# EmanueleCosenza/polyphemus

Measured on AMD Instinct MI355X. Metric: bar-graphs/sec VAE fwd+bwd (+loss +Adam), LMD2 4-track x 32-ts synthetic, higher is better.
Workload: dtype f32 (fp16-pair MFMA products)

## Files before the change

include/polyphemus_hip.h:

```cpp
#ifndef POLYPHEMUS_HIP_H
#define POLYPHEMUS_HIP_H

#include <stdint.h>

#ifdef __cplusplus
extern "C" {
#endif

typedef void* pm_stream_t;

enum {
  PM_OK = 0,
  PM_E_INVALID = -1,
  PM_E_LAUNCH = -2,
  PM_E_UNSUPPORTED = -3
};

enum { PM_N_REL = 6, PM_N_DIST = 32, PM_N_SLOTS = 15, PM_N_PITCH = 131, PM_N_DUR = 99, PM_N_TOK = 230 };

#define PM_ABI_VERSION 9
int pm_abi_version(void);
const char* pm_build_info(void);

int pm_set_deterministic(int32_t on);
// ... 98 lines not shown
int pm_edge_table_bwd(const float* dT , int32_t d, float* d_nn_weight ,
                      float* d_nn_bias , pm_stream_t stream);
int pm_segreduce_fwd(const float* x , const float* T , const int32_t* plan,
                     int32_t N, int32_t E, int32_t G, int32_t d, float dropout_p, uint32_t seed,
                     uint32_t layer_uid, int32_t compact, float* A , pm_stream_t stream);
int pm_segreduce_fwd_planes(const float* x, const float* T, const int32_t* plan, int32_t N, int32_t E, int32_t G,
                            int32_t d, float dropout_p, uint32_t seed, uint32_t layer_uid, int32_t compact,
                            uint16_t* planes, int64_t plane_stride, pm_stream_t stream);
int pm_gcl_forward_fused(const float* x , const float* T , const int32_t* plan, int32_t N,
                         int32_t E, int32_t G, int32_t d, float dropout_p, uint32_t seed, uint32_t layer_uid,
                         const uint16_t* w_frag, const float* bias , int32_t use_classes,
                         float* h , double* col_stats ,
                         uint16_t* planes , int64_t plane_stride, pm_stream_t stream);
int pm_gcl_input_grad_fused(const uint16_t* dh_planes , int64_t plane_stride, const int32_t* plan,
                            int32_t N, int32_t E, int32_t G, int32_t d, const uint16_t* w_frag_t, int32_t use_classes,
                            float* dA , pm_stream_t stream);
typedef struct PmBnBwd {
  const float* h;
  const float* du;
  const float* mean; const float* var; const float* gamma; const float* beta;
  const double* acc3;
  float* dgamma; float* dbeta; float* dbias_pre;
  float eps; int32_t relu;
  int32_t add_residual;
  int32_t reserved;
} PmBnBwd;
int pm_gcl_input_grad_bn(const PmBnBwd* norm, uint16_t* dh_planes , int64_t plane_stride,
                         const int32_t* plan, int32_t N, int32_t E, int32_t G, int32_t d, const uint16_t* w_frag_t,
                         int32_t use_classes, float* dA , pm_stream_t stream);
enum { PM_ABSMAX_SLOTS = 64 };
typedef struct PmH2 {
  const uint32_t* absmax_in; const uint32_t* absmax_aux; float* scale_out; float w_scale; int32_t reserved;
} PmH2;
int pm_absmax(const float* x, int64_t n, uint32_t* out, pm_stream_t stream);
int pm_split_planes_frag_h2(const float* W, int32_t rows, int32_t cols, int32_t kind, int32_t n_mats, int64_t src_stride,
                            int64_t dst_stride, float w_scale, uint16_t* out, pm_stream_t stream);
int pm_gcl_forward_fused_h2(const float* x, const float* T, const int32_t* plan, int32_t N, int32_t E, int32_t G, int32_t d,
                            float dropout_p, uint32_t seed, uint32_t layer_uid, const uint16_t* w_frag, const float* bias,
                            int32_t use_classes, float* h, double* col_stats, uint16_t* planes, int64_t plane_stride,
                            const PmH2* h2, pm_stream_t stream);
int pm_gcl_input_grad_bn_h2(const PmBnBwd* norm, uint16_t* dh_planes, int64_t plane_stride, const int32_t* plan, int32_t N,
                            int32_t E, int32_t G, int32_t d, const uint16_t* w_frag_t, int32_t use_classes, float* dA,
                            const PmH2* h2, pm_stream_t stream);
int pm_bn_bwd_fused_h2(const float* x, const float* dy, int32_t O, int32_t C, const float* mean, const float* var, float eps,
                       const float* gamma, const float* beta, int relu, float* dgamma, float* dbeta, float* dbias_pre,
                       double* acc3, uint16_t* dx_planes, int64_t plane_stride, int32_t sums_ready, const PmH2* h2,
                       pm_stream_t stream);
int pm_gcl_input_grad_fused_h2(const uint16_t* dh_planes, int64_t plane_stride, const int32_t* plan, int32_t N, int32_t E,
                               int32_t G, int32_t d, const uint16_t* w_frag_t, int32_t use_classes, float* dA,
                               const float* dh_scale, float w_scale, pm_stream_t stream);
int pm_gcl_weight_grad_fused_h2(const uint16_t* a_planes, int64_t a_plane_stride, const uint16_t* dh_planes,
                                int64_t dh_plane_stride, const int32_t* plan, int32_t N, int32_t E, int32_t G, int32_t d,
                                int32_t use_classes, float* dW, const float* a_scale, const float* dh_scale,
                                pm_stream_t stream);
int pm_gcl_weight_grad_fused(const uint16_t* a_planes , int64_t a_plane_stride,
                             const uint16_t* dh_planes , int64_t dh_plane_stride, const int32_t* plan,
                             int32_t N, int32_t E, int32_t G, int32_t d, int32_t use_classes, float* dW ,
                             pm_stream_t stream);
int pm_gcl_forward_from_planes(const uint16_t* a_planes , int64_t plane_stride, const int32_t* plan,
                               int32_t N, int32_t E, int32_t G, int32_t d, const uint16_t* w_frag,
                               const float* bias , int32_t use_classes, float* h ,
                               double* col_stats , pm_stream_t stream);
int pm_gcl_forward_from_planes_h2(const uint16_t* a_planes, int64_t plane_stride, const int32_t* plan, int32_t N, int32_t E,
                                  int32_t G, int32_t d, const uint16_t* w_frag, const float* bias, int32_t use_classes,
                                  float* h, double* col_stats, const float* a_scale, float w_scale, pm_stream_t stream);
int pm_rows_times_weight(const float* X, int32_t ldx, int32_t N, int32_t K, const uint16_t* w_frag, int32_t kind,
                         int32_t w_tiles, int32_t Nout, const float* bias , float* C, int32_t ldc,
                         pm_stream_t stream);
int pm_rows_times_weight_longk(const float* X, int32_t ldx, int32_t N, int32_t K, const uint16_t* w_frag, int32_t kind,
                               int32_t w_pitch, int32_t Nout, float* C, int32_t ldc, pm_stream_t stream);
int pm_rows_tn_weight_grad(const float* A, int32_t lda, int32_t M, const float* B, int32_t ldb, int32_t Nn, int32_t K,
                           float* C , int32_t ldc, float* colsum_a , pm_stream_t stream);
typedef struct PmNormSums {
  const float* h;
  const float* mean; const float* var; const float* gamma; const float* beta;
  float eps; int32_t relu;
  double* acc3;
  uint32_t* absmax_out;
} PmNormSums;
int pm_segreduce_bwd_norm(const float* x, const float* T, const float* dA, const float* dres, const int32_t* plan,
                          int32_t N, int32_t E, int32_t G, int32_t d, float dropout_p, uint32_t seed,
                          uint32_t layer_uid, int32_t compact, float* dx, float* dT, const PmNormSums* next_norm,
                          pm_stream_t stream);
int pm_segreduce_bwd(const float* x, const float* T, const float* dA ,
                     const float* dres ,
                     const int32_t* plan, int32_t N, int32_t E, int32_t G, int32_t d, float dropout_p,
                     uint32_t seed, uint32_t layer_uid, int32_t compact, float* dx ,
                     float* dT , pm_stream_t stream);

int pm_bar_aggregate_fwd(const float* x, const float* T, const int32_t* plan, int32_t N, int32_t E, int32_t G, int32_t d,
                         float dropout_p, uint32_t seed, uint32_t layer_uid, uint16_t* planes, int64_t plane_stride,
                         const PmH2* h2 , pm_stream_t stream);
int pm_bar_aggregate_bwd(const float* x, const float* T, const float* dA , const float* dres ,
                         const int32_t* plan, int32_t N, int32_t E, int32_t G, int32_t d, float dropout_p, uint32_t seed,
                         uint32_t layer_uid, float* dx , float* dT ,
                         const PmNormSums* next_norm , pm_stream_t stream);

enum { PM_GEMM_RELU = 1, PM_GEMM_ACCUM = 2,
       PM_GEMM_RELU_ADD = 16 ,
       PM_GEMM_ZEROED = 8 ,
       PM_GEMM_PARTITION = 4  };
int pm_gemm_config(int32_t transA, int32_t M, int32_t N, int32_t K);
int pm_gemm_force_config(int32_t cfg);
int pm_gemm_f32(int transA, int transB, int32_t M, int32_t N, int32_t K, const float* A, int32_t lda,
                const float* B, int32_t ldb, float* C, int32_t ldc, const float* bias, int flags,
                int split_k, const int32_t* rowmap, int32_t rows_per_entry, const int32_t* dyn_entries,
                pm_stream_t stream);
int pm_gemm_f32_grouped(int transA, int transB, int32_t M, int32_t N, int32_t K, const float* A, int32_t lda,
                        const float* B, int32_t ldb, float* C, int32_t ldc, const float* bias, int flags,
                        int split_k, const int32_t* rowmap, int32_t rows_per_entry, const int32_t* dyn_entries,
                        int32_t n_groups, int64_t a_group_stride, int64_t b_group_stride, int64_t c_group_stride,
                        int64_t bias_group_stride, int32_t map_group_stride, int32_t dyn_group_stride,
                        pm_stream_t stream);
int pm_split_planes(const float* src, int64_t n, uint16_t* planes, int64_t plane_stride ,
                    pm_stream_t stream);
typedef struct PmGemmDesc {
  int32_t transA, transB, M, N, K;
  const float* A; int32_t lda;
  const float* B; int32_t ldb;
  float* C; int32_t ldc;
  const float* bias;
  int32_t flags, split_k;
  const int32_t* rowmap; int32_t rows_per_entry;
  const int32_t* dyn_entries;
  int32_t n_groups;
  int64_t a_group_stride, b_group_stride, c_group_stride, bias_group_stride;
  int32_t map_group_stride, dyn_group_stride;
  int32_t b_split_rows; int64_t b_shared_off;
  int32_t c_split_rows; int64_t c_shared_off;
  double* col_stats;
  int32_t operand_planes;
  int64_t a_plane_stride, b_plane_stride;
  const int32_t* class_ptr;
  int32_t class_block;
  const void* b_frag;
  float* a_colsum;
} PmGemmDesc;
int pm_split_planes_frag(const float* W, int32_t rows, int32_t cols, int32_t kind, int32_t n_mats, int64_t src_stride,
                         int64_t dst_stride, uint16_t* out, pm_stream_t stream);
int pm_gemm_f32_desc(const PmGemmDesc* desc, pm_stream_t stream);

int pm_bn_stats(const float* x, int32_t O, int32_t C, int32_t I, float* mean ,
                float* var , float* running_mean ,
                float* running_var, float momentum, double* scratch , pm_stream_t stream);
int pm_bn_apply(const float* x, int32_t O, int32_t C, int32_t I, const float* mean, const float* var,
                float eps, const float* gamma, const float* beta, const float* residual ,
                int relu, float* y, pm_stream_t stream);
int pm_bn_bwd(const float* x, const float* dy, int32_t O, int32_t C, int32_t I, const float* mean,
              const float* var, float eps, const float* gamma, const float* beta, int relu,
              float* dgamma , float* dbeta , float* dbias_pre , float* dx,
              double* scratch , pm_stream_t stream);
#define PM_BN_SCRATCH(C) (256 * 3 * (C) + 4 * (C))
#define PM_BN_SMALL_MAX_ROWS 2048
int pm_bn_small_fwd(const float* x, int32_t O, int32_t C, float eps, const float* gamma, const float* beta,
                    const float* residual , int relu, float* y, float* mean ,
                    float* var , float* running_mean , float* running_var,
                    float momentum, pm_stream_t stream);
int pm_bn_small_bwd(const float* x, const float* dy, int32_t O, int32_t C, const float* mean, const float* var, float eps,
                    const float* gamma, const float* beta, int relu, float* dgamma , float* dbeta ,
                    float* dbias_pre , float* dx, pm_stream_t stream);
int pm_bn_partial_sums(const float* x, const float* dy , int32_t O, int32_t C, int32_t I, const float* mean,
                       const float* var, float eps, const float* gamma, const float* beta, int relu,
                       double* sums , double* scratch , pm_stream_t stream);
int pm_bn_stats_from_sums(const double* sums , double count, int32_t C, float* mean, float* var,
                          float* running_mean , float* running_var, float momentum, pm_stream_t stream);
int pm_bn_bwd_from_sums(const float* x, const float* dy, int32_t O, int32_t C, int32_t I, const float* mean,
// ... 19 lines not shown
                    int32_t sums_ready ,
                    pm_stream_t stream);
int pm_bn_bwd_sums(const float* x, const float* dy, int32_t O, int32_t C, const float* mean, const float* var, float eps,
                   const float* gamma, const float* beta, int relu, double* acc3, pm_stream_t stream);
int pm_bn_fold_weights(const float* W, int32_t rows, int32_t cols, const float* bias, const float* gamma, const float* beta,
                       const float* running_mean, const float* running_var, float eps, float* W_out, float* b_out,
                       pm_stream_t stream);
int pm_bn_counters_update(int64_t* counters , const int64_t* inc , const int64_t* sel ,
                          const int32_t* group_cnt , int32_t n, pm_stream_t stream);
int pm_relu_bwd(const float* dy, const float* y, int64_t n, float* dx, pm_stream_t stream);
int pm_relu_bwd_planes(const float* dy, const float* h, int64_t n, float* dh, uint16_t* planes, int64_t plane_stride,
                       pm_stream_t stream);
int pm_relu_residual_fwd(const float* x, const float* res, int64_t n, float* y, pm_stream_t stream);
int pm_dropout_rows(const float* x, int64_t rows, int32_t cols, float p, uint32_t seed, uint32_t site, float* y,
                    pm_stream_t stream);
int pm_add(const float* a, const float* b, int64_t n, float* out, pm_stream_t stream);
int pm_colsum_acc(const float* x, int32_t M, int32_t C, int32_t ld, float* out , pm_stream_t stream);
int pm_colsum_rows_acc(const float* x, int32_t C, int32_t ld, const int32_t* rowmap, int32_t rows_per_entry,
                       const int32_t* dyn_entries, int32_t max_entries, float* out , pm_stream_t stream);
int pm_reparam_fwd(const float* mu, const float* log_var, const float* eps, int64_t n, float* z, pm_stream_t stream);
int pm_reparam_bwd(const float* dz, const float* log_var, const float* eps, int64_t n, float* dmu ,
                   float* dlog_var , pm_stream_t stream);

int pm_embed_tables(const float* w_pitch_drum , const float* b_pitch_drum,
                    const float* w_pitch_nd, const float* b_pitch_nd, const float* w_dur ,
                    const float* b_dur, const float* bn_drum_g, const float* bn_drum_b,
                    const float* bn_nd_g, const float* bn_nd_b, const float* bn_dur_g, const float* bn_dur_b,
                    float* rm_drum, float* rv_drum, float* rm_nd, float* rv_nd, float* rm_dur, float* rv_dur,
                    const int32_t* tok_hist , int32_t d, int training, float eps, float momentum,
                    float* tables , float* stats ,
                    pm_stream_t stream);
int pm_embed_gather(const float* tables, const int32_t* tokens , const uint8_t* is_drum,
                    int32_t N, int32_t d, int32_t n_slots, float* X , pm_stream_t stream);
int pm_embed_bwd_scatter(const float* dX , const int32_t* tokens, const int32_t* plan, int32_t N,
                         int32_t E, int32_t G, int32_t d, int32_t n_slots,
                         float* S , pm_stream_t stream);
int pm_chord_pad_fwd(const float* tables, const float* chord_w , const float* chord_b,
                     const uint8_t* is_drum, int32_t N, int32_t d, int32_t n_slots, float* cvec ,
                     float* y , pm_stream_t stream);
int pm_chord_pad_bwd(const float* dy , const uint8_t* is_drum, int32_t N, int32_t d, int32_t n_slots,
                     const float* tables, const float* chord_w, float* gsum ,
                     float* d_chord_w , float* S , pm_stream_t stream);
int pm_chord_pad_vec(const float* tables, const float* chord_w, const float* chord_b, int32_t d, int32_t n_slots,
                     float* cvec , pm_stream_t stream);
int pm_chord_tables_fwd(const float* tables , const float* chord_w , int32_t d, int32_t n_slots,
                        float* PT, const float* chord_b , float* cvec ,
                        pm_stream_t stream);
int pm_chord_sum_fwd(const float* PT, const float* cvec, const int32_t* tokens , const uint8_t* is_drum, int32_t N,
                     int32_t d, int32_t n_slots, float* x0 , pm_stream_t stream);
int pm_chord_sum_bwd(const float* dy , const int32_t* tokens, const int32_t* plan, int32_t N, int32_t E, int32_t G,
                     int32_t d , int32_t n_slots, float* Gt, pm_stream_t stream);
int pm_chord_tables_bwd_w(const float* Gt, const float* tables, int32_t d, int32_t n_slots, float* d_chord_w ,
                          float* d_chord_b , pm_stream_t stream);
int pm_chord_tables_bwd_x(const float* Gt, const float* chord_w, int32_t d, int32_t n_slots, float* S , pm_stream_t stream);
int pm_embed_tables_bwd(const float* S, const float* w_pitch_drum, const float* b_pitch_drum,
                        const float* w_pitch_nd, const float* b_pitch_nd, const float* w_dur, const float* b_dur,
                        const float* bn_drum_g, const float* bn_nd_g, const float* bn_dur_g, const float* stats,
                        const int32_t* tok_hist, int32_t d, float eps, float* dw_pitch_drum, float* db_pitch_drum,
                        float* dw_pitch_nd, float* db_pitch_nd, float* dw_dur, float* db_dur, float* dg_drum,
                        float* dbeta_drum, float* dg_nd, float* dbeta_nd, float* dg_dur, float* dbeta_dur,
                        pm_stream_t stream);

int pm_embed_tables_bwd_sync(const float* S, const float* w_pitch_drum, const float* b_pitch_drum, const float* w_pitch_nd,
                             const float* b_pitch_nd, const float* w_dur, const float* b_dur, const float* bn_drum_g,
                             const float* bn_nd_g, const float* bn_dur_g, const float* stats, const int32_t* tok_hist,
                             int32_t d, float eps, float* dw_pitch_drum, float* db_pitch_drum, float* dw_pitch_nd,
                             float* db_pitch_nd, float* dw_dur, float* db_dur, float* dg_drum, float* dbeta_drum,
                             float* dg_nd, float* dbeta_nd, float* dg_dur, float* dbeta_dur, double* sums_out,
                             const double* sums_global, const int32_t* hist_global, pm_stream_t stream);

int pm_gate_fwd(const float* x , const float* w , const float* b , int32_t N,
                int32_t d, float* g , pm_stream_t stream);
int pm_attnpool_fwd(const float* x, const float* g, const float* g_mean, const float* g_var, float eps,
                    const float* bn_g, const float* bn_b, const int32_t* plan, int32_t N, int32_t E, int32_t G,
                    int32_t d, float* alpha , float* out , pm_stream_t stream);
int pm_attnpool_bwd(const float* x, const float* g, const float* g_mean, const float* g_var, float eps,
                    const float* bn_g, const float* alpha, const float* dout , const float* gate_w,
                    const int32_t* plan, int32_t N, int32_t E, int32_t G, int32_t d, float* dx ,
                    float* d_gate_w , float* d_gate_b , float* d_bn_g ,
                    float* d_bn_b , float* scratch ,
                    const float* x_gate ,
                    float* dx_gate ,
                    pm_stream_t stream);
int pm_attnpool_bwd_sums(const float* x, const float* g, const float* g_mean, const float* g_var, float eps,
                         const float* alpha, const float* dout, const int32_t* plan, int32_t N, int32_t E, int32_t G,
                         int32_t d, float* scratch , pm_stream_t stream);
int pm_attnpool_bwd_from_sums(const float* x, const float* g, const float* g_mean, const float* g_var, float eps,
                              const float* bn_g, const float* alpha, const float* dout, const float* gate_w,
                              const int32_t* plan, int32_t N, int32_t E, int32_t G, int32_t d, float* dx, float* d_gate_w,
                              float* d_gate_b, float* d_bn_g, float* d_bn_b, float* scratch, const float* x_gate,
                              float* dx_gate, const double* sums_global , double count_global,
                              pm_stream_t stream);
int pm_bar_broadcast_fwd(const float* bars , const int32_t* plan, int32_t N, int32_t E, int32_t G,
                         int32_t d, float* x , pm_stream_t stream);
int pm_bar_broadcast_bwd(const float* dx , const int32_t* plan, int32_t N, int32_t E, int32_t G,
                         int32_t d, float* dbars , pm_stream_t stream);

int pm_conv3x3_fwd(const float* x, const float* w, const float* b, int32_t G, int32_t Ci, int32_t Co, int32_t H,
                   int32_t W, int up4, float* y, pm_stream_t stream);
int pm_conv3x3_bwd_data(const float* dy, const float* w, int32_t G, int32_t Ci, int32_t Co, int32_t H, int32_t W,
                        int up4, float* dx, pm_stream_t stream);
int pm_conv3x3_bwd_weight(const float* x, const float* dy, int32_t G, int32_t Ci, int32_t Co, int32_t H, int32_t W,
                          int up4, float* dw , float* db , pm_stream_t stream);
int pm_maxpool4_fwd(const float* x, int64_t n_out, float* y, pm_stream_t stream);
int pm_maxpool4_bwd(const float* x, const float* dy, int64_t n_out, float* dx, pm_stream_t stream);
int pm_cnn_enc_fwd(const float* s, const float* w0 , const float* b0, const float* gamma1, const float* beta1,
                   const float* w4 , const float* b4, const float* gamma5, const float* beta5, int32_t G, float eps,
                   float momentum, float* c0, float* a0, float* p0, float* c1, float* a1, float* mean1, float* var1,
                   float* rmean1, float* rvar1, float* mean5, float* var5, float* rmean5, float* rvar5, double* scratch,
                   int64_t scratch_len, pm_stream_t stream);
int pm_cnn_dec_fwd(const float* u2, const float* w1 , const float* b1, const float* gamma2, const float* beta2,
                   const float* w4 , const float* b4, int32_t G, float eps, float momentum, float* c2, float* a2,
                   float* s_logits, float* mean2, float* var2, float* rmean2, float* rvar2, double* scratch, int64_t scratch_len,
                   pm_stream_t stream);
int pm_cnn_enc_bwd(const float* s, const float* c0, const float* a0, const float* p0, const float* c1, const float* da1,
                   const float* mean1, const float* var1, const float* gamma1, const float* beta1, const float* mean5,
                   const float* var5, const float* gamma5, const float* beta5, const float* w4, int32_t G, float eps, float* dw0,
                   float* db0, float* dgamma1, float* dbeta1, float* dw4, float* db4, float* dgamma5, float* dbeta5, float* dc1,
                   float* da0, float* dc0, double* scratch, int64_t scratch_len, pm_stream_t stream);

int pm_content_ce(const float* c_logits , const int32_t* tokens ,
                  const int32_t* tok_hist, const uint8_t* is_drum , int32_t N,
                  int32_t n_slots , float grad_scale,
                  float* d_logits , float* db_pitch_drum ,
                  float* db_pitch_nd , float* db_dur , double* out, pm_stream_t stream);
int pm_content_ce_scaled(const float* c_logits, const int32_t* tokens, const int32_t* tok_hist, const uint8_t* is_drum,
                         int32_t N, int32_t n_slots, float grad_scale, const float* dev_scale ,
                         float* d_logits, float* db_pitch_drum, float* db_pitch_nd, float* db_dur, double* out,
                         pm_stream_t stream);
int64_t pm_unembed_scratch_bytes(int32_t d);
int pm_unembed_ce(const float* H, const float* w_pitch_drum , const float* b_pitch_drum,
                  const float* w_pitch_nd, const float* b_pitch_nd, const float* w_dur , const float* b_dur,
                  const int32_t* tokens, const int32_t* plan, int32_t N, int32_t E, int32_t G, int32_t d, int32_t n_slots,
                  float grad_scale, const float* dev_scale, float* logits , float* d_logits,
                  float* db_pitch_drum, float* db_pitch_nd, float* db_dur, double* out, uint16_t* w_planes ,
                  pm_stream_t stream);
int64_t pm_unembed_dh_scratch_bytes(int32_t d);
int pm_unembed_dh(const float* d_logits, const float* w_pitch_drum , const float* w_pitch_nd,
                  const float* w_dur , const int32_t* plan, int32_t N, int32_t E, int32_t G, int32_t d,
                  int32_t n_slots, float* dH, uint16_t* w_planes, int32_t prepare, pm_stream_t stream);
int64_t pm_unembed_row_counts_len(int32_t N, int32_t n_slots);
int pm_unembed_row_lists(const int32_t* tokens, const int32_t* plan, int32_t N, int32_t E, int32_t G, int32_t d, int32_t n_slots,
                         int32_t* row_lists, int32_t* pad_lists, int32_t* row_counts, float* dH_zero, pm_stream_t stream);
int pm_unembed_ce_rows(const float* H, const float* w_pitch_drum, const float* b_pitch_drum, const float* w_pitch_nd,
                       const float* b_pitch_nd, const float* w_dur, const float* b_dur, const int32_t* tokens, const int32_t* plan,
                       int32_t N, int32_t E, int32_t G, int32_t d, int32_t n_slots, float grad_scale, const float* dev_scale,
                       float* logits, float* d_logits, float* db_pitch_drum, float* db_pitch_nd, float* db_dur, double* out,
                       uint16_t* w_planes, const int32_t* row_lists, const int32_t* row_counts, pm_stream_t stream);
int pm_unembed_dh_rows(const float* d_logits, const float* w_pitch_drum, const float* w_pitch_nd, const float* w_dur,
                       const int32_t* plan, int32_t N, int32_t E, int32_t G, int32_t d, int32_t n_slots, float* dH,
                       uint16_t* w_planes, const int32_t* row_lists, const int32_t* row_counts, pm_stream_t stream);
int pm_unembed_dw(const float* d_logits, const float* H, const int32_t* plan, int32_t N, int32_t E, int32_t G, int32_t d,
                  int32_t n_slots, float* dw_pitch_drum, float* dw_pitch_nd, float* dw_dur, const int32_t* row_lists,
                  const int32_t* row_counts, pm_stream_t stream);
int pm_unembed_bias_grads(const float* d_logits, const uint8_t* is_drum , int32_t N, int32_t S,
                          float* db_pitch_drums , float* db_pitch_non_drums , float* db_dur ,
                          pm_stream_t stream);
int pm_kld(const float* mu, const float* log_var, int32_t B, int32_t d, float beta, float* dmu ,
           float* dlog_var, double* out, pm_stream_t stream);
int pm_bce_logits(const float* logits, const float* target, int64_t n, float grad_scale, float* dlogits ,
                  double* out, pm_stream_t stream);

int pm_content_accuracy(const float* c_logits , const int32_t* tokens ,
                        const uint8_t* is_drum , int32_t N, int64_t* counts , pm_stream_t stream);
int pm_structure_metrics(const float* s_logits, const float* s_target, int64_t n, int64_t* counts ,
                         pm_stream_t stream);
// ... 151 lines not shown
```

polyphemus_amd/_lib.py:

```python
from __future__ import annotations

import ctypes as C
import os
from typing import Optional

import torch

_HERE = os.path.dirname(os.path.abspath(__file__))
LIB_PATH = os.environ.get("PM_LIB_PATH") or os.path.join(_HERE, "libpolyphemus_hip.so")

PROF_NCLASS = 40
PLAN_FIELDS = ["rowptr", "csr_src", "csr_dist", "csr_eid", "colptr", "csc_dst", "csc_reldist", "csc_eid",
               "csc_invcnt", "node_bar", "bar_ptr", "group_list", "group_cnt", "tok_hist", "row_list", "node_trel", "trk_list", "trk_cnt", "scratch"]

_SIGS = {
    "pm_plan_layout": "iiip",
    "pm_gcl_tile_order": "piipi",
    "pm_row_tile_order": "ipi",
    "pm_plan_build": "pppppppiiiiips",
    "pm_edge_attrs_to_ids": "pipps",
    "pm_tokens_from_onehot": "pips",
    "pm_batch_flags": "pppiipps",
    "pm_edge_table": "ppips",
    "pm_edge_table_bwd": "pipps",
# ... 67 lines not shown
    "pm_conv3x3_bwd_weight": "ppiiiiiipps",
    "pm_maxpool4_fwd": "plps",
    "pm_maxpool4_bwd": "pplps",
    "pm_cnn_enc_fwd": "pppppppppiffppppppppppppppls",
    "pm_cnn_dec_fwd": "pppppppiffppppppppls",
    "pm_cnn_enc_bwd": "pppppppppppppppifppppppppppppls",
    "pm_content_ce": "ppppiifppppps",
    "pm_content_ce_scaled": "ppppiifpppppps",
    "pm_unembed_ce": "pppppppppiiiiifpppppppps",
    "pm_unembed_dh": "pppppiiiiippis",
    "pm_unembed_dh_scratch_bytes": "i",
    "pm_unembed_row_counts_len": "ii",
    "pm_unembed_dw": "pppiiiiippppps",
    "pm_unembed_row_lists": "ppiiiiipppps",
    "pm_unembed_ce_rows": "pppppppppiiiiifpppppppppps",
    "pm_unembed_dh_rows": "pppppiiiiipppps",
    "pm_unembed_scratch_bytes": "i",
    "pm_kld": "ppiifppps",
    "pm_unembed_bias_grads": "ppiippps",
    "pm_bce_logits": "pplfpps",
    "pm_content_accuracy": "pppips",
    "pm_structure_metrics": "pplps",
    "pm_adam_step": "pppplffffifs",
    "pm_comm_unique_id": "p",
    "pm_comm_init": "piip",
    "pm_comm_destroy": "p",
    "pm_allreduce": "plps",
    "pm_prof_configure": "li",
    "pm_prof_begin": "i",
    "pm_prof_end": "ppp",
    "pm_vae_step_workspace_bytes": "piiiii",
    "pm_vae_step_forward": "pppppppfuufiplpps",
    "pm_vae_step_info": "pp",
    "pm_vae_step_outputs": "ppppps".replace(" ", ""),
    "pm_vae_step_set_output_grads": "ppppps",
    "pm_vae_step_saved": "piiipp",
    "pm_vae_step_output_views": "ppp",
    "pm_bn_relu_decisions": "pppppflips",
    "pm_vae_step_backward_decoder": "ps",
    "pm_vae_step_backward_encoder": "ps",
    "pm_vae_step_backward_encoder_tail": "ps",
    "pm_vae_step_join_decoder_grads": "ps",
    "pm_vae_step_backward_encoder_heads": "ps",
    "pm_vae_step_reload_switches": "",
    "pm_relu_bwd_planes": "pplppls",
    "pm_absmax": "plps",
    "pm_split_planes_frag_h2": "piiiillfps",
    "pm_gcl_forward_fused_h2": "pppiiiifuuppippplps",
    "pm_gcl_input_grad_bn_h2": "pplpiiiipipps",
    "pm_gcl_weight_grad_fused_h2": "plplpiiiiippps",
    "pm_bn_bwd_fused_h2": "ppiippfppippppplips",
    "pm_gcl_input_grad_fused_h2": "plpiiiipippfs",
    "pm_bn_apply_fused_absmax": "piipfpppipppppfps",
    "pm_bar_aggregate_fwd": "pppiiiifuuplps",
    "pm_bar_aggregate_bwd": "pppppiiiifuuppps",
    "pm_gcl_forward_from_planes_h2": "plpiiiippipppfs",
    "pm_set_deterministic": "i",
    "pm_get_deterministic": "",
    "pm_deterministic_faults": "",
    "pm_h2_clamp_events": "i",
    "pm_h2_clamp_init": "",
    "pm_overflow_snapshot": "ps",
    "pm_overflow_poison": "pps",
    "pm_grad_nonfinite_check": "plpppfffis",
    "pm_adam_step_guarded": "pppplffffps",
    "pm_adam_bias_scalars": "plfffps",
    "pm_vae_step_set_metrics": "pp",
    "pm_unembed_ce_metrics": "pppppppppiiiiifppppppppppps",
    "pm_unembed_ce_rows_metrics": "pppppppppiiiiifppppppppppppps",
    "pm_content_accuracy_slots": "pppiipps",
    "pm_train_metric_counts": "pppiipplps",
    "pm_grad_sumsq": "plps",
    "pm_grad_nonfinite_check_sumsq": "plpppfffips",
    "pm_grad_clip_finish": "pffps",
    "pm_adam_step_clipped": "pppplffffipps",
    "pm_adam_step_ema": "ppppplffffiffpps",
    "pm_buffer_swap": "ppls",
    "pm_sample_tokens": "plfifups",
    "pm_mtp_from_tokens": "ppilppps",
    "pm_sample_chords": "pplpupps",
    "pm_node_tracks": "pilppps",
    "pm_sample_structure": "pipuppps",
    "pm_notes_from_tokens": "ppiilppppplpps",
}
_CT = {"p": C.c_void_p, "i": C.c_int32, "l": C.c_int64, "f": C.c_float, "u": C.c_uint32, "s": C.c_void_p, "D": C.c_double}
_RET64 = {"pm_vae_step_workspace_bytes", "pm_vae_layout_bytes", "pm_vae_step_state_bytes", "pm_unembed_scratch_bytes",
          "pm_unembed_dh_scratch_bytes", "pm_unembed_row_counts_len"}
ABI_VERSION = 9
EXPORTED = sorted(list(_SIGS) + ["pm_abi_version", "pm_build_info", "pm_dropout_hash", "pm_sample_hash",
                                 "pm_vae_layout_bytes", "pm_vae_step_state_bytes"])



class PmChordRules(C.Structure):
    _fields_ = [("temperature", C.c_float * 2), ("top_k", C.c_int32), ("top_p", C.c_float), ("min_notes", C.c_int32 * 4),
                ("max_notes", C.c_int32 * 4), ("pitch_mask", (C.c_uint32 * 4) * 4)]


class PmStructureRules(C.Structure):
    _fields_ = [("temperature", C.c_float), ("bias", C.c_float * 4), ("min_active", C.c_int32 * 4),
                ("max_active", C.c_int32 * 4), ("step_mask", C.c_uint32 * 4)]


_lib: Optional[C.CDLL] = None


class HipExtensionError(RuntimeError):
    pass


def lib() -> C.CDLL:
    global _lib
    if _lib is None:
        if not os.path.exists(LIB_PATH):
            raise HipExtensionError(
                f"{LIB_PATH} is missing: build it with `python -m polyphemus_amd.build` "
                "(__graft_entry__.build()).  There is no CPU fallback for the HIP path.")
        L = C.CDLL(LIB_PATH)
        for name, sig in _SIGS.items():
            fn = getattr(L, name)
            fn.argtypes = [_CT[c] for c in sig]
            fn.restype = C.c_int64 if name in _RET64 else C.c_int
        L.pm_vae_layout_bytes.restype = C.c_int64
        L.pm_vae_step_state_bytes.restype = C.c_int64
        L.pm_abi_version.restype = C.c_int
        if L.pm_abi_version() != ABI_VERSION:
            raise HipExtensionError(f"{LIB_PATH} has ABI version {L.pm_abi_version()}, this binding expects {ABI_VERSION}: "
                                    "rebuild it (`python -m polyphemus_amd.build --force`)")
        L.pm_build_info.restype = C.c_char_p
        L.pm_dropout_hash.argtypes = [C.c_uint32] * 4
        L.pm_dropout_hash.restype = C.c_uint32
        L.pm_sample_hash.argtypes = [C.c_uint32] * 4
        L.pm_sample_hash.restype = C.c_uint32
        _lib = L
    return _lib


def ptr(t: Optional[torch.Tensor]):
    return None if t is None else t.data_ptr()


def stream() -> int:
    return torch.cuda.current_stream().cuda_stream


_ERR = {-1: "PM_E_INVALID (bad argument)", -2: "PM_E_LAUNCH (kernel launch failed)", -3: "PM_E_UNSUPPORTED"}


def call(name: str, *args) -> None:
    rc = getattr(lib(), name)(*args)
    if rc != 0:
        raise HipExtensionError(f"{name} failed: {_ERR.get(rc, rc)}")


def plan_layout(N: int, E: int, G: int):
    off = (C.c_int64 * (len(PLAN_FIELDS) + 1))()
    rc = lib().pm_plan_layout(N, E, G, C.cast(off, C.c_void_p))
    if rc != 0:
        raise HipExtensionError(f"pm_plan_layout({N},{E},{G}) failed: {_ERR.get(rc, rc)}")
    return list(off)


def gcl_tile_order(trk_cnt, use_classes: bool, N: int):
    tc = (C.c_int32 * 32)(*[int(v) for v in list(trk_cnt)[:32]])
    grid = lib().pm_gcl_tile_order(C.cast(tc, C.c_void_p), int(bool(use_classes)), int(N), None, 0)
    if grid < 0:
# ... 40 lines not shown
```

polyphemus_amd/csrc/common.h:

```cpp
#pragma once
#include <hip/hip_runtime.h>
#include <stdint.h>
#include "../../include/polyphemus_hip.h"

#define PM_WAVE 64

static inline int pm_check_launch() {
  hipError_t e = hipGetLastError();
  return e == hipSuccess ? PM_OK : PM_E_LAUNCH;
}

static inline int pm_device_slot() {
  int d = 0;
  if (hipGetDevice(&d) != hipSuccess || d < 0 || d >= 16) d = 0;
  return d;
}

static inline int64_t pm_cdiv(int64_t a, int64_t b) { return (a + b - 1) / b; }
static inline int64_t pm_align4(int64_t x) { return (x + 3) & ~int64_t(3); }

struct PmPlanView {
  const int32_t* rowptr; const int32_t* csr_src; const int32_t* csr_dist; const int32_t* csr_eid;
  const int32_t* colptr; const int32_t* csc_dst; const int32_t* csc_reldist; const int32_t* csc_eid;
  const float* csc_invcnt; const int32_t* node_bar; const int32_t* bar_ptr; const int32_t* group_list;
// ... 98 lines not shown
  return v;
}
__device__ static inline double pm_wave_sum_d(double v) {
#pragma unroll
  for (int o = 32; o > 0; o >>= 1) v += __shfl_xor(v, o, 64);
  return v;
}
typedef __bf16 pm_bf16x2 __attribute__((ext_vector_type(2)));
typedef float pm_f32x2 __attribute__((ext_vector_type(2)));
typedef unsigned int pm_u32x2 __attribute__((ext_vector_type(2)));
__device__ static inline unsigned pm_pk_bf16(float a, float b) {
  pm_f32x2 v = {a, b};
  return __builtin_bit_cast(unsigned, __builtin_convertvector(v, pm_bf16x2));
}
__device__ static inline void pm_split3_pair(float a, float b, unsigned& h1, unsigned& h2, unsigned& h3) {
  h1 = pm_pk_bf16(a, b);
  a -= __uint_as_float(h1 << 16); b -= __uint_as_float(h1 & 0xffff0000u);
  h2 = pm_pk_bf16(a, b);
  a -= __uint_as_float(h2 << 16); b -= __uint_as_float(h2 & 0xffff0000u);
  h3 = pm_pk_bf16(a, b);
}
typedef _Float16 pm_f16x2 __attribute__((ext_vector_type(2)));
__device__ static inline unsigned pm_pk_f16(float a, float b) {
  pm_f32x2 v = {a, b};
  return __builtin_bit_cast(unsigned, __builtin_convertvector(v, pm_f16x2));
}
__device__ static inline void pm_split2h_pair(float a, float b, unsigned& h1, unsigned& h2) {
  h1 = pm_pk_f16(a, b);
  const pm_f16x2 hv = __builtin_bit_cast(pm_f16x2, h1);
  a -= (float)hv.x; b -= (float)hv.y;
  h2 = pm_pk_f16(a, b);
}
__device__ static inline float pm_pow2_scale(float bound, int target) {
  if (!(bound > 0.f) || !(bound < 3.0e38f)) return 1.f;
  const int e = (int)((__float_as_uint(bound) >> 23) & 0xff) - 126;
  int k = target - e;
  k = k < -120 ? -120 : (k > 120 ? 120 : k);
  return __uint_as_float((unsigned)(k + 127) << 23);
}
__device__ static inline float pm_clamp_f16(float v) { return fminf(fmaxf(v, -65504.f), 65504.f); }
__device__ static inline float pm_clamp_f16(float v, bool& cut) {
  const float c = fminf(fmaxf(v, -65504.f), 65504.f);
  cut = cut || (c != v);
  return c;
}
__device__ static inline float pm_absmax_read(const unsigned* __restrict__ p) {
  static_assert(PM_ABSMAX_SLOTS == 64, "one slot per lane");
  float v = __uint_as_float(p[__lane_id()]);
#pragma unroll
  for (int o = 32; o > 0; o >>= 1) v = fmaxf(v, __shfl_xor(v, o, 64));
  return v;
}
__device__ static inline void pm_absmax_block(unsigned* __restrict__ out, float v, unsigned* sm) {
  v = fabsf(v);
#pragma unroll
  for (int o = 32; o > 0; o >>= 1) v = fmaxf(v, __shfl_xor(v, o, 64));
  if ((threadIdx.x & 63) == 0) atomicMax(sm, __float_as_uint(v));
  __syncthreads();
  if (threadIdx.x == 0) atomicMax(out + (blockIdx.x % PM_ABSMAX_SLOTS), *sm);
}
__device__ static inline void pm_store_planes4(uint16_t* __restrict__ planes, int64_t plane_stride, int64_t idx, float x0,
                                               float x1, float x2, float x3) {
  unsigned l1, l2, l3, u1, u2, u3;
  pm_split3_pair(x0, x1, l1, l2, l3);
  pm_split3_pair(x2, x3, u1, u2, u3);
  const pm_u32x2 p1 = {l1, u1}, p2 = {l2, u2}, p3 = {l3, u3};
  *reinterpret_cast<pm_u32x2*>(planes + idx) = p1;
  *reinterpret_cast<pm_u32x2*>(planes + plane_stride + idx) = p2;
  *reinterpret_cast<pm_u32x2*>(planes + 2 * plane_stride + idx) = p3;
}
__device__ static inline double pm_repl_sum(const double* __restrict__ acc, int nacc, int C, int a, int c) {
  double t = 0;
#pragma unroll
  for (int r = 0; r < PM_BN_REPL; ++r) t += acc[((int64_t)r * nacc + a) * C + c];
  return t;
}
__device__ static inline float pm_bn_bwd_elem(float x, float dy, float mean, float rstd, float ga, float be, float m0,
                                              float m1, int relu) {
  const float xh = (x - mean) * rstd;
  float du = dy;
  if (relu && !(xh * ga + be > 0.f)) du = 0.f;
  return ga * rstd * (du - m0 - xh * m1);
}
__device__ static inline float pm_wave_max(float v) {
#pragma unroll
  for (int o = 32; o > 0; o >>= 1) v = fmaxf(v, __shfl_xor(v, o, 64));
  return v;
}
#endif
```

polyphemus_amd/csrc/linear.hip:

```cpp
#include "gcl_tiles.h"
#include <type_traits>
#include <stdlib.h>
#include "prof.h"
#include "wide.h"

#ifndef ROWS_NMW
#define ROWS_NMW 4
#endif
template <int D> constexpr int rows_nmw() { return D == 256 ? ROWS_NMW : 4; }
template <int D> constexpr int rows_threads() { return (rows_nmw<D>() + 4) * 64; }
template <int D, int BKIND>
__global__ void __launch_bounds__(rows_threads<D>()) __attribute__((amdgpu_waves_per_eu((rows_nmw<D>() + 4) / 4, (rows_nmw<D>() + 4) / 4)))
k_rows_w(const float* __restrict__ X, int ldx, int N, const char* __restrict__ wfrag, int wtiles, int nblk,
         const float* __restrict__ bias, float* __restrict__ C, int ldc) {
  constexpr int NMW = rows_nmw<D>(), WC = D / NMW, TN = WC / 32, KS = D / 16, RB = D * 2, PL = BM * RB;
  extern __shared__ __attribute__((aligned(16))) char smem[];
  float* const sC = reinterpret_cast<float*>(smem + 3 * PL);
  int m0 = 0, rows = BM;
  if (!pm_row_tile(N, blockIdx.x, m0, rows)) return;
  const bool full = rows > BM / 2;
  N = min(N, m0 + rows);
  const int tid = threadIdx.x, lane = tid & 63, wave = tid >> 6, li = lane & 31, lh = lane >> 5;
  if (wave >= NMW) {
    constexpr int LPR = D / 4, RPW = 64 / LPR, NR = BM / (4 * RPW);
    const int st = tid - NMW * 64, c4 = st % LPR, r0 = st / LPR;
    const __amdgpu_buffer_rsrc_t crs = __builtin_amdgcn_make_buffer_rsrc(C, 0, GCL_OOB, 0x00020000);
    __syncthreads();
#pragma unroll 1
    for (int qb = 0; qb < nblk; ++qb) {
      __syncthreads();
      __syncthreads();
      float4 bv = make_float4(0.f, 0.f, 0.f, 0.f);
      if (bias) bv = *reinterpret_cast<const float4*>(bias + qb * D + c4 * 4);
#pragma unroll
      for (int k = 0; k < NR; ++k) {
        const int rr = r0 + k * 4 * RPW, row = m0 + rr;
        float4 v = *reinterpret_cast<const float4*>(sC + rr * D + c4 * 4);
        v.x += bv.x; v.y += bv.y; v.z += bv.z; v.w += bv.w;
        __builtin_amdgcn_raw_buffer_store_b128(__builtin_bit_cast(u32x4, v), crs,
            row < N ? (int)(((int64_t)row * ldc + qb * D + c4 * 4) * 4) : GCL_OOB, 0, 0);
      }
    }
    return;
  }
  {
    const __amdgpu_buffer_rsrc_t rs = __builtin_amdgcn_make_buffer_rsrc(const_cast<float*>(X), 0, GCL_OOB, 0x00020000);
    constexpr int CPR = D / 8, NST = NMW * 64, NCHK = BM * CPR / NST;
    u32x4 v[NCHK][2];
#pragma unroll
    for (int k = 0; k < NCHK; ++k) {
      const int ci = tid + k * NST, rr = ci / CPR, ch = ci % CPR, row = m0 + rr;
#pragma unroll
      for (int h = 0; h < 2; ++h)
        v[k][h] = __builtin_amdgcn_raw_buffer_load_b128(rs, row < N ? (int)(((int64_t)row * ldx + ch * 8 + h * 4) * 4) : GCL_OOB, 0, 0);
    }
#pragma unroll
    for (int k = 0; k < NCHK; ++k) {
      const int ci = tid + k * NST, rr = ci / CPR, ch = ci % CPR;
      unsigned p1[4], p2[4], p3[4];
#pragma unroll
      for (int h = 0; h < 2; ++h) {
        pm_split3_pair(__uint_as_float(v[k][h][0]), __uint_as_float(v[k][h][1]), p1[2 * h], p2[2 * h], p3[2 * h]);
        pm_split3_pair(__uint_as_float(v[k][h][2]), __uint_as_float(v[k][h][3]), p1[2 * h + 1], p2[2 * h + 1], p3[2 * h + 1]);
      }
      char* dst = smem + rr * RB + ((ch ^ (rr & 15)) << 4);
      *reinterpret_cast<u32x4*>(dst) = u32x4{p1[0], p1[1], p1[2], p1[3]};
      *reinterpret_cast<u32x4*>(dst + PL) = u32x4{p2[0], p2[1], p2[2], p2[3]};
      *reinterpret_cast<u32x4*>(dst + 2 * PL) = u32x4{p3[0], p3[1], p3[2], p3[3]};
    }
  }
  const __amdgpu_buffer_rsrc_t brs = __builtin_amdgcn_make_buffer_rsrc(const_cast<char*>(wfrag), 0, GCL_OOB, 0x00020000);
  auto bload = [&](bf16x8 (&dst)[3][TN], int gs) {
    const int qb = min(gs / KS, nblk - 1), ks = gs % KS;
    const int n0 = qb * D + wave * WC;
    const int soff = __builtin_amdgcn_readfirstlane(BKIND == 0 ? ((n0 >> 5) * KS + ks) * 3072 : (ks * wtiles + (n0 >> 5)) * 3072);
#pragma unroll
    for (int j = 0; j < TN; ++j)
#pragma unroll
      for (int p = 0; p < 3; ++p)
        dst[p][j] = __builtin_bit_cast(bf16x8, __builtin_amdgcn_raw_buffer_load_b128(brs, lane * 16, soff + j * (BKIND == 0 ? KS : 1) * 3072 + p * 1024, 0));
  };
  bf16x8 bq[GCL_BDEPTH][3][TN];
#pragma unroll
  for (int s2 = 0; s2 < GCL_BDEPTH; ++s2) bload(bq[s2], s2);
  __syncthreads();
// ... 2 lines not shown
    for (int p = 0; p < 3; ++p)
#pragma unroll
      for (int i = 0; i < 2; ++i) {
        const int rr = i * 32 + li;
        a[p][i] = *reinterpret_cast<const bf16x8*>(smem + p * PL + rr * RB + (((ks * 2 + lh) ^ (rr & 15)) << 4));
      }
  };
  bf16x8 af[2][3][2];
  aload(af[0], 0);
  auto blocks = [&](auto ni_tag) {
  constexpr int NI = decltype(ni_tag)::value;
#pragma unroll 1
  for (int qb = 0; qb < nblk; ++qb) {
    f32x16 acc[2][TN];
#pragma unroll
    for (int i = 0; i < 2; ++i)
#pragma unroll
      for (int j = 0; j < TN; ++j)
#pragma unroll
        for (int r = 0; r < 16; ++r) acc[i][j][r] = 0.f;
#pragma unroll
    for (int ks = 0; ks < KS; ++ks) {
      aload(af[(ks + 1) & 1], (ks + 1) % KS);
      constexpr int PA[6] = {2, 1, 0, 1, 0, 0}, PB[6] = {0, 1, 2, 0, 1, 0};
#pragma unroll
      for (int t6 = 0; t6 < 6; ++t6)
#pragma unroll
        for (int i = 0; i < NI; ++i)
#pragma unroll
          for (int j = 0; j < TN; ++j)
            acc[i][j] = __builtin_amdgcn_mfma_f32_32x32x16_bf16(af[ks & 1][PA[t6]][i], bq[ks % GCL_BDEPTH][PB[t6]][j], acc[i][j], 0, 0, 0);
      bload(bq[ks % GCL_BDEPTH], qb * KS + ks + GCL_BDEPTH);
      __builtin_amdgcn_sched_barrier(0);
    }
    __syncthreads();
#pragma unroll
    for (int i = 0; i < 2; ++i)
#pragma unroll
      for (int r = 0; r < 16; ++r)
#pragma unroll
        for (int j = 0; j < TN; ++j)
          sC[(i * 32 + (r & 3) + 8 * (r >> 2) + 4 * lh) * D + wave * WC + j * 32 + li] = acc[i][j][r];
    __syncthreads();
  }
  };
  if (full) blocks(std::integral_constant<int, 2>{});
  else blocks(std::integral_constant<int, 1>{});
}

extern "C" int pm_rows_times_weight(const float* X, int32_t ldx, int32_t N, int32_t K, const uint16_t* w_frag, int32_t kind,
                                    int32_t w_tiles, int32_t Nout, const float* bias, float* C, int32_t ldc,
                                    pm_stream_t stream) {
  if (!X || !w_frag || !C || N <= 0 || (K != 128 && K != 256 && K != 512) || Nout <= 0 || (Nout % K) || (kind != 0 && kind != 1) ||
      ldx < K || ldc < Nout || (ldx & 3) || (ldc & 3) || ((uintptr_t)X % 16) || ((uintptr_t)C % 16) ||
      ((uintptr_t)w_frag % 16) || (bias && ((uintptr_t)bias % 16)) || (int64_t)N * ldx * 4 >= 0x7fffffffLL ||
      (int64_t)N * ldc * 4 >= 0x7fffffffLL || (kind == 1 && w_tiles * 32 < Nout))
    return PM_E_INVALID;
  if (K == 512)
    return pm_wide_rows_times_weight(X, ldx, N, w_frag, kind, w_tiles, Nout, bias, C, ldc, (hipStream_t)stream);
  hipStream_t st = (hipStream_t)stream;
  const dim3 grid(pm_row_grid(N));
  const size_t lds = (size_t)3 * BM * K * 2 + (size_t)BM * K * 4;
  const int pe = pm_prof_open(st, PM_PROF_ROWS_W, 2.0 * N * (double)K * Nout);
#define LAUNCH(DD, KD)                                                                                                 \
  do {                                                                                                                 \
    static bool once_dev[16] = {}; bool& once = once_dev[pm_device_slot()];                                                                                          \
    if (!once) {                                                                                                       \
      hipFuncSetAttribute((const void*)k_rows_w<DD, KD>, hipFuncAttributeMaxDynamicSharedMemorySize, 160 * 1024);      \
      once = true;                                                                                                     \
    }                                                                                                                  \
    hipLaunchKernelGGL((k_rows_w<DD, KD>), grid, dim3(rows_threads<DD>()), lds, st, X, ldx, N, reinterpret_cast<const char*>(w_frag), \
                       w_tiles, Nout / K, bias, C, ldc);                                                               \
  } while (0)
  if (K == 256) { if (kind == 0) LAUNCH(256, 0); else LAUNCH(256, 1); }
  else { if (kind == 0) LAUNCH(128, 0); else LAUNCH(128, 1); }
#undef LAUNCH
  pm_prof_close(st, pe);
  return pm_check_launch();
}

template <int D, int BKIND>
__global__ void __launch_bounds__(rows_threads<D>()) __attribute__((amdgpu_waves_per_eu((rows_nmw<D>() + 4) / 4, (rows_nmw<D>() + 4) / 4)))
k_rows_wk(const float* __restrict__ X, int ldx, int N, int K, const char* __restrict__ wfrag, int wpitch,
          float* __restrict__ C, int ldc) {
  constexpr int NMW = rows_nmw<D>(), WC = D / NMW, TN = WC / 32, HS = D + 8, NTHR = rows_threads<D>();
  extern __shared__ __attribute__((aligned(16))) char smem[];
  float* const sH = reinterpret_cast<float*>(smem);
  const int nchunk = K / CH;
  int m0 = 0, rows = BM;
  if (!pm_row_tile(N, blockIdx.x, m0, rows)) return;
  const bool full = rows > BM / 2;
  N = min(N, m0 + rows);
  const int tid = threadIdx.x, lane = tid & 63, wave = tid >> 6;
  if (wave >= NMW) {
    const int pt = tid - NMW * 64, q = pt & 31, prow = pt >> 5;
    const __amdgpu_buffer_rsrc_t xrs = __builtin_amdgcn_make_buffer_rsrc(const_cast<float*>(X), 0, GCL_OOB, 0x00020000);
    auto issue = [&](float4 (&xs)[8], int c) {
#pragma unroll
      for (int ps = 0; ps < 8; ++ps) {
        const int row = m0 + ps * 8 + prow;
        xs[ps] = __builtin_bit_cast(float4, __builtin_amdgcn_raw_buffer_load_b128(
            xrs, (row < N && c < nchunk) ? (int)(((int64_t)row * ldx + c * CH + q * 4) * 4) : GCL_OOB, 0, 0));
      }
    };
    auto put = [&](const float4 (&xs)[8], int c) {
      char* img = smem + (c & 1) * IMG;
#pragma unroll
      for (int ps = 0; ps < 8; ++ps) {
        const int rr = ps * 8 + prow;
        unsigned l1, l2, l3, u1, u2, u3;
        pm_split3_pair(xs[ps].x, xs[ps].y, l1, l2, l3);
        pm_split3_pair(xs[ps].z, xs[ps].w, u1, u2, u3);
        const pm_u32x2 p1 = {l1, u1}, p2 = {l2, u2}, p3 = {l3, u3};
        char* dst = img + rr * ROWB + (((q >> 1) ^ (rr & 15)) << 4) + ((q & 1) << 3);
        *reinterpret_cast<pm_u32x2*>(dst) = p1;
        *reinterpret_cast<pm_u32x2*>(dst + PLANE) = p2;
        *reinterpret_cast<pm_u32x2*>(dst + 2 * PLANE) = p3;
      }
    };
    float4 xa[8], xb[8];
    issue(xa, 0);
    issue(xb, 1);
    __builtin_amdgcn_sched_barrier(0);
    put(xa, 0);
    __syncthreads();
#pragma unroll 1
    for (int c = 0; c < nchunk; c += 2) {
      issue(xa, c + 2);
      __builtin_amdgcn_sched_barrier(0);
      put(xb, c + 1);
      __syncthreads();
      if (c + 1 >= nchunk) break;
      issue(xb, c + 3);
      __builtin_amdgcn_sched_barrier(0);
      put(xa, c + 2);
      __syncthreads();
    }
  } else {
    const int li = lane & 31, lh = lane >> 5;
    f32x16 acc[2][TN];
#pragma unroll
    for (int i = 0; i < 2; ++i)
#pragma unroll
      for (int j = 0; j < TN; ++j)
#pragma unroll
        for (int r = 0; r < 16; ++r) acc[i][j][r] = 0.f;
    const __amdgpu_buffer_rsrc_t brs = __builtin_amdgcn_make_buffer_rsrc(const_cast<char*>(wfrag), 0, GCL_OOB, 0x00020000);
    const int n0 = wave * WC;
    auto bload = [&](bf16x8 (&dst)[3][TN], int gs) {
      const int kk = min(gs, nchunk * 8 - 1);
      const int soff = __builtin_amdgcn_readfirstlane(BKIND == 0 ? ((n0 >> 5) * wpitch + kk) * 3072 : (kk * (D / 32) + (n0 >> 5)) * 3072);
#pragma unroll
      for (int j = 0; j < TN; ++j)
#pragma unroll
        for (int p = 0; p < 3; ++p)
          dst[p][j] = __builtin_bit_cast(bf16x8, __builtin_amdgcn_raw_buffer_load_b128(brs, lane * 16, soff + j * (BKIND == 0 ? wpitch : 1) * 3072 + p * 1024, 0));
    };
    bf16x8 bq[GCL_BDEPTH][3][TN];
#pragma unroll
    for (int s2 = 0; s2 < GCL_BDEPTH; ++s2) bload(bq[s2], s2);
    __syncthreads();
    auto chunks = [&](auto ni_tag) {
      constexpr int NI = decltype(ni_tag)::value;
#pragma unroll 1
      for (int c = 0; c < nchunk; ++c) {
        const char* img = smem + (c & 1) * IMG;
#pragma unroll
        for (int ks = 0; ks < 8; ++ks) {
          bf16x8 a[3][NI];
#pragma unroll
          for (int p = 0; p < 3; ++p)
#pragma unroll
            for (int i = 0; i < NI; ++i) {
              const int rr = i * 32 + li;
              a[p][i] = *reinterpret_cast<const bf16x8*>(img + p * PLANE + rr * ROWB + (((ks * 2 + lh) ^ (rr & 15)) << 4));
            }
          constexpr int PA[6] = {2, 1, 0, 1, 0, 0}, PB[6] = {0, 1, 2, 0, 1, 0};
#pragma unroll
          for (int t6 = 0; t6 < 6; ++t6)
#pragma unroll
            for (int i = 0; i < NI; ++i)
#pragma unroll
              for (int j = 0; j < TN; ++j)
                acc[i][j] = __builtin_amdgcn_mfma_f32_32x32x16_bf16(a[PA[t6]][i], bq[ks % GCL_BDEPTH][PB[t6]][j], acc[i][j], 0, 0, 0);
          bload(bq[ks % GCL_BDEPTH], c * 8 + ks + GCL_BDEPTH);
          __builtin_amdgcn_sched_barrier(0);
        }
        __syncthreads();
      }
    };
    if (full) chunks(std::integral_constant<int, 2>{});
    else chunks(std::integral_constant<int, 1>{});
#pragma unroll
    for (int j = 0; j < TN; ++j)
#pragma unroll
      for (int i = 0; i < 2; ++i)
#pragma unroll
        for (int r = 0; r < 16; ++r)
          sH[(i * 32 + (r & 3) + 8 * (r >> 2) + 4 * lh) * HS + n0 + j * 32 + li] = acc[i][j][r];
  }
  __syncthreads();
  constexpr int NG = 512 / D, RG = BM / NG;
  static_assert(NTHR >= 512, "row groups");
  const int col = tid % D, rg = tid / D;
  const __amdgpu_buffer_rsrc_t crs = __builtin_amdgcn_make_buffer_rsrc(C, 0, GCL_OOB, 0x00020000);
  if (tid >= 512) return;
#pragma unroll 8
  for (int k = 0; k < RG; ++k) {
    const int rr = rg * RG + k, row = m0 + rr;
    __builtin_amdgcn_raw_buffer_store_b32(__float_as_uint(sH[rr * HS + col]), crs, row < N ? (int)(((int64_t)row * ldc + col) * 4) : GCL_OOB, 0, 0);
  }
}

extern "C" int pm_rows_times_weight_longk(const float* X, int32_t ldx, int32_t N, int32_t K, const uint16_t* w_frag,
                                          int32_t kind, int32_t w_pitch, int32_t Nout, float* C, int32_t ldc,
                                          pm_stream_t stream) {
  if (!X || !w_frag || !C || N <= 0 || K <= 0 || (K % CH) || (Nout != 128 && Nout != 256 && Nout != 512) || (kind != 0 && kind != 1) ||
      ldx < K || ldc < Nout || (ldx & 3) || ((uintptr_t)X % 16) || ((uintptr_t)w_frag % 16) ||
      (int64_t)N * ldx * 4 >= 0x7fffffffLL || (int64_t)N * ldc * 4 >= 0x7fffffffLL || (kind == 0 && w_pitch * 16 < K))
    return PM_E_INVALID;
  if (Nout == 512)
    return pm_wide_rows_times_weight_longk(X, ldx, N, K, w_frag, kind, w_pitch, C, ldc, (hipStream_t)stream);
  hipStream_t st = (hipStream_t)stream;
  const dim3 grid(pm_row_grid(N));
  const size_t lds = 2 * IMG;
  const int pe = pm_prof_open(st, PM_PROF_ROWS_W, 2.0 * N * (double)K * Nout);
#define LAUNCH(DD, KD)                                                                                                 \
  do {                                                                                                                 \
    static bool once_dev[16] = {}; bool& once = once_dev[pm_device_slot()];                                                                                          \
    if (!once) {                                                                                                       \
      hipFuncSetAttribute((const void*)k_rows_wk<DD, KD>, hipFuncAttributeMaxDynamicSharedMemorySize, 160 * 1024);     \
      once = true;                                                                                                     \
    }                                                                                                                  \
    hipLaunchKernelGGL((k_rows_wk<DD, KD>), grid, dim3(rows_threads<DD>()), lds, st, X, ldx, N, K, reinterpret_cast<const char*>(w_frag), \
                       w_pitch, C, ldc);                                                                               \
  } while (0)
  if (Nout == 256) { if (kind == 0) LAUNCH(256, 0); else LAUNCH(256, 1); }
  else { if (kind == 0) LAUNCH(128, 0); else LAUNCH(128, 1); }
#undef LAUNCH
  pm_prof_close(st, pe);
  return pm_check_launch();
}


__global__ void __launch_bounds__(512) __attribute__((amdgpu_waves_per_eu(2, 2)))
k_rows_tn(const float* __restrict__ A, int lda, const float* __restrict__ B, int ldb, int K, int ntn, int nsplit,
          float* __restrict__ C, int ldc, float* __restrict__ colsum_a, unsigned* gate) {
  extern __shared__ __attribute__((aligned(16))) char smem[];
  const int ntile = gridDim.x / nsplit;
  int L = blockIdx.x;
  {
    const int total = gridDim.x, q = total >> 3, r = total & 7, xcd = L & 7, idx = L >> 3;
    L = (xcd < r ? xcd * (q + 1) : r * (q + 1) + (xcd - r) * q) + idx;
  }
  const int zs = L / ntile, within = L % ntile, ft = within / ntn, ct = within % ntn;
  const int kper = (((K + nsplit - 1) / nsplit + DW_KT - 1) / DW_KT) * DW_KT;
  const int kbeg = zs * kper, kend = min(kbeg + kper, K);
  if (kbeg >= kend) { pm_turn_skip_block(gate, 8); return; }
  const int nt = (kend - kbeg + DW_KT - 1) / DW_KT;
  const int tid = threadIdx.x, lane = tid & 63, wave = tid >> 6;
  const unsigned my_turn = blockIdx.x * 8 + wave;
  if (wave >= 4) {
    const int lt = tid - 256, c4 = lt & 31, r0 = lt >> 5;
    const __amdgpu_buffer_rsrc_t ars = __builtin_amdgcn_make_buffer_rsrc(const_cast<float*>(A), 0, GCL_OOB, 0x00020000);
    const __amdgpu_buffer_rsrc_t brs = __builtin_amdgcn_make_buffer_rsrc(const_cast<float*>(B), 0, GCL_OOB, 0x00020000);
    const int acol = (ft * DW_T + c4 * 4) * 4, bcol = (ct * DW_T + c4 * 4) * 4;
    float4 cs = make_float4(0.f, 0.f, 0.f, 0.f);
    const bool want_cs = colsum_a != nullptr && ct == 0;
    auto issue = [&](float4 (&v)[4][2], int t) {
#pragma unroll
      for (int j = 0; j < 4; ++j) {
        const int row = kbeg + t * DW_KT + r0 + j * 8;
        const bool ok = t < nt && row < kend;
        v[j][0] = __builtin_bit_cast(float4, __builtin_amdgcn_raw_buffer_load_b128(ars, ok ? (int)((int64_t)row * lda * 4) + acol : GCL_OOB, 0, 0));
        v[j][1] = __builtin_bit_cast(float4, __builtin_amdgcn_raw_buffer_load_b128(brs, ok ? (int)((int64_t)row * ldb * 4) + bcol : GCL_OOB, 0, 0));
      }
    };
    auto put = [&](const float4 (&v)[4][2], int t) {
      char* st = smem + (t & 1) * DW_STAGE;
#pragma unroll
      for (int j = 0; j < 4; ++j) {
        if (want_cs) { cs.x += v[j][0].x; cs.y += v[j][0].y; cs.z += v[j][0].z; cs.w += v[j][0].w; }
#pragma unroll
        for (int o = 0; o < 2; ++o) {
          unsigned l1, l2, l3, u1, u2, u3;
          pm_split3_pair(v[j][o].x, v[j][o].y, l1, l2, l3);
          pm_split3_pair(v[j][o].z, v[j][o].w, u1, u2, u3);
          const pm_u32x2 p1 = {l1, u1}, p2 = {l2, u2}, p3 = {l3, u3};
          char* dst = st + o * 3 * DW_PLANE + (r0 + j * 8) * DW_PITCH + c4 * 8;
          *reinterpret_cast<pm_u32x2*>(dst) = p1;
          *reinterpret_cast<pm_u32x2*>(dst + DW_PLANE) = p2;
          *reinterpret_cast<pm_u32x2*>(dst + 2 * DW_PLANE) = p3;
        }
      }
    };
    float4 va[4][2], vb[4][2];
    issue(va, 0);
    issue(vb, 1);
    __builtin_amdgcn_sched_barrier(0);
    put(va, 0);
    __syncthreads();
#pragma unroll 1
    for (int t = 0; t < nt; t += 2) {
      issue(va, t + 2);
      __builtin_amdgcn_sched_barrier(0);
      put(vb, t + 1);
      __syncthreads();
      if (t + 1 >= nt) break;
      issue(vb, t + 3);
      __builtin_amdgcn_sched_barrier(0);
      put(va, t + 2);
      __syncthreads();
    }
    pm_turn_enter(gate, my_turn);
    if (want_cs) {
      cs.x += __shfl_xor(cs.x, 32, 64); cs.y += __shfl_xor(cs.y, 32, 64);
      cs.z += __shfl_xor(cs.z, 32, 64); cs.w += __shfl_xor(cs.w, 32, 64);
      float* dst = colsum_a + ft * DW_T + c4 * 4;
      if (lane < 32) { atomicAdd(dst, cs.x); atomicAdd(dst + 1, cs.y); atomicAdd(dst + 2, cs.z); atomicAdd(dst + 3, cs.w); }
    }
    pm_turn_leave(gate, my_turn);
    return;
  }
  const int li = lane & 31, lh = lane >> 5, wr = wave >> 1, wc = wave & 1;
// ... 70 lines not shown
```

polyphemus_amd/csrc/norm.hip:

```cpp
#include "common.h"
#include <stdlib.h>

#define BN_MAX_CHUNKS 256
#define BN_NACC 3

struct BnCtx {
  const float* mean; const float* var; const float* gamma; const float* beta; float eps; int relu;
};
template <int MODE>
__device__ static inline void bn_acc(float xv, float dyv, float m, float rstd, float ga, float be, int relu,
                                     double& a, double& b, double& c) {
  if (MODE == 0) { a += (double)xv; b += (double)xv * (double)xv; }
  else {
    const float xh = (xv - m) * rstd;
    float du = dyv;
    if (relu && !(xh * ga + be > 0.f)) du = 0.f;
    a += (double)du; b += (double)du * (double)xh; c += (double)xh;
  }
}

template <int MODE>
__global__ void __launch_bounds__(256) k_colreduce_rows(const float* __restrict__ x, const float* __restrict__ dy,
                                                        int O, int C, BnCtx ctx, int rows_per_chunk,
                                                        double* __restrict__ partial) {
  __shared__ double sh[4][64][12];
  const int lane = threadIdx.x & 63, wave = threadIdx.x >> 6;
  const int c = (blockIdx.x * 64 + lane) * 4;
  const bool ok = c < C;
  double acc[12] = {0, 0, 0, 0, 0, 0, 0, 0, 0, 0, 0, 0};
  float m[4] = {0, 0, 0, 0}, rs[4] = {1, 1, 1, 1}, ga[4] = {1, 1, 1, 1}, be[4] = {0, 0, 0, 0};
  if (MODE == 1 && ok) {
#pragma unroll
    for (int j = 0; j < 4; ++j) {
      m[j] = ctx.mean[c + j]; rs[j] = rsqrtf(ctx.var[c + j] + ctx.eps);
      ga[j] = ctx.gamma[c + j]; be[j] = ctx.beta[c + j];
    }
  }
  const int r0 = blockIdx.y * rows_per_chunk;
  int r1 = r0 + rows_per_chunk;
  if (r1 > O) r1 = O;
  if (ok) {
    for (int r = r0 + wave; r < r1; r += 4) {
      const float4 xv = *reinterpret_cast<const float4*>(x + (int64_t)r * C + c);
      float4 dv = make_float4(0.f, 0.f, 0.f, 0.f);
      if (MODE == 1) dv = *reinterpret_cast<const float4*>(dy + (int64_t)r * C + c);
      bn_acc<MODE>(xv.x, dv.x, m[0], rs[0], ga[0], be[0], ctx.relu, acc[0], acc[4], acc[8]);
      bn_acc<MODE>(xv.y, dv.y, m[1], rs[1], ga[1], be[1], ctx.relu, acc[1], acc[5], acc[9]);
      bn_acc<MODE>(xv.z, dv.z, m[2], rs[2], ga[2], be[2], ctx.relu, acc[2], acc[6], acc[10]);
      bn_acc<MODE>(xv.w, dv.w, m[3], rs[3], ga[3], be[3], ctx.relu, acc[3], acc[7], acc[11]);
    }
  }
  constexpr int NA = MODE == 0 ? 8 : 12;
#pragma unroll
  for (int j = 0; j < NA; ++j) sh[wave][lane][j] = acc[j];
  __syncthreads();
  if (wave == 0 && ok) {
#pragma unroll
    for (int j = 0; j < NA; ++j) {
      const double s = sh[0][lane][j] + sh[1][lane][j] + sh[2][lane][j] + sh[3][lane][j];
      partial[((int64_t)blockIdx.y * BN_NACC + (j >> 2)) * C + c + (j & 3)] = s;
    }
  }
}

template <int MODE>
__global__ void __launch_bounds__(256) k_colreduce_chan(const float* __restrict__ x, const float* __restrict__ dy,
                                                        int O, int C, int I, BnCtx ctx, int64_t per_chunk,
                                                        double* __restrict__ partial) {
  __shared__ double sh[3][4];
  const int c = blockIdx.x;
  float m = 0.f, rs = 1.f, ga = 1.f, be = 0.f;
  if (MODE == 1) { m = ctx.mean[c]; rs = rsqrtf(ctx.var[c] + ctx.eps); ga = ctx.gamma[c]; be = ctx.beta[c]; }
  double a = 0, b = 0, cc = 0;
  const int64_t total = (int64_t)O * I;
  const int64_t j0 = (int64_t)blockIdx.y * per_chunk;
  int64_t j1 = j0 + per_chunk;
  if (j1 > total) j1 = total;
  for (int64_t j = j0 + threadIdx.x; j < j1; j += blockDim.x) {
    const int64_t idx = ((j / I) * C + c) * I + (j % I);
    bn_acc<MODE>(x[idx], MODE == 1 ? dy[idx] : 0.f, m, rs, ga, be, ctx.relu, a, b, cc);
  }
  a = pm_wave_sum_d(a); b = pm_wave_sum_d(b); cc = pm_wave_sum_d(cc);
  if ((threadIdx.x & 63) == 0) { sh[0][threadIdx.x >> 6] = a; sh[1][threadIdx.x >> 6] = b; sh[2][threadIdx.x >> 6] = cc; }
  __syncthreads();
  if (threadIdx.x < 3)
    partial[((int64_t)blockIdx.y * BN_NACC + threadIdx.x) * C + c] =
        sh[threadIdx.x][0] + sh[threadIdx.x][1] + sh[threadIdx.x][2] + sh[threadIdx.x][3];
}

#define BN_FIN_WAVES 16
__device__ static inline void sum_chunks(const double* __restrict__ partial, int nchunk, int C, int c, int nacc,
                                         double (*sh)[64][BN_NACC], double* out) {
  const int lane = threadIdx.x & 63, wave = threadIdx.x >> 6;
  double s[BN_NACC] = {0, 0, 0};
  if (c < C)
    for (int k = wave; k < nchunk; k += BN_FIN_WAVES)
      for (int a = 0; a < nacc; ++a) s[a] += partial[((int64_t)k * BN_NACC + a) * C + c];
  for (int a = 0; a < BN_NACC; ++a) sh[wave][lane][a] = s[a];
  __syncthreads();
  for (int a = 0; a < BN_NACC; ++a) {
    double t = 0;
// ... 791 lines not shown
```

polyphemus_amd/csrc/pool.hip:

```cpp
#include "common.h"

__global__ void __launch_bounds__(256) k_gate_fwd(const float* __restrict__ x, const float* __restrict__ w,
                                                  const float* __restrict__ b, int N, int d, float* __restrict__ g) {
  const int n = blockIdx.x * 4 + (threadIdx.x >> 6);
  if (n >= N) return;
  const int lane = threadIdx.x & 63;
  float s = 0.f;
  for (int c = lane * 4; c < d; c += 256) {
    const float4 xv = *reinterpret_cast<const float4*>(x + (int64_t)n * d + c);
    const float4 wv = *reinterpret_cast<const float4*>(w + c);
    s += xv.x * wv.x + xv.y * wv.y + xv.z * wv.z + xv.w * wv.w;
  }
  s = pm_wave_sum(s);
  if (lane == 0) g[n] = s + b[0];
}
extern "C" int pm_gate_fwd(const float* x, const float* w, const float* b, int32_t N, int32_t d, float* g,
                           pm_stream_t stream) {
  if (!x || !w || !b || !g || N <= 0 || d <= 0 || (d & 3)) return PM_E_INVALID;
  hipLaunchKernelGGL(k_gate_fwd, dim3(pm_cdiv(N, 4)), dim3(256), 0, (hipStream_t)stream, x, w, b, N, d, g);
  return pm_check_launch();
}

__device__ static inline float block_max(float v, float* sh) {
  v = pm_wave_max(v);
  if ((threadIdx.x & 63) == 0) sh[threadIdx.x >> 6] = v;
  __syncthreads();
  const float r = fmaxf(fmaxf(sh[0], sh[1]), fmaxf(sh[2], sh[3]));
  __syncthreads();
  return r;
}
__device__ static inline float block_sum(float v, float* sh) {
  v = pm_wave_sum(v);
  if ((threadIdx.x & 63) == 0) sh[threadIdx.x >> 6] = v;
  __syncthreads();
  const float r = sh[0] + sh[1] + sh[2] + sh[3];
  __syncthreads();
  return r;
}

__global__ void __launch_bounds__(256) k_attnpool_fwd(const float* __restrict__ x, const float* __restrict__ g,
                                                      const float* __restrict__ gm, const float* __restrict__ gv,
                                                      float eps, const float* __restrict__ bg,
                                                      const float* __restrict__ bb, const int* __restrict__ bar_ptr,
                                                      int d, float* __restrict__ alpha, float* __restrict__ out) {
  __shared__ float sh[4];
  const int b = blockIdx.x;
  const int beg = bar_ptr[b], end = bar_ptr[b + 1];
  const float mean = gm[0], rstd = rsqrtf(gv[0] + eps), ga = bg[0], be = bb[0];
  float mx = -INFINITY;
  for (int i = beg + threadIdx.x; i < end; i += blockDim.x) mx = fmaxf(mx, (g[i] - mean) * rstd * ga + be);
  mx = block_max(mx, sh);
  float s = 0.f;
  for (int i = beg + threadIdx.x; i < end; i += blockDim.x) s += expf(((g[i] - mean) * rstd * ga + be) - mx);
  s = block_sum(s, sh);
  const float inv = 1.0f / (s + 1e-16f);
  for (int i = beg + threadIdx.x; i < end; i += blockDim.x)
    alpha[i] = expf(((g[i] - mean) * rstd * ga + be) - mx) * inv;
  __syncthreads();
  for (int c = threadIdx.x; c < d; c += blockDim.x) {
    float acc = 0.f;
    for (int i = beg; i < end; ++i) acc += alpha[i] * x[(int64_t)i * d + c];
    out[(int64_t)b * d + c] = acc;
  }
}
extern "C" int pm_attnpool_fwd(const float* x, const float* g, const float* g_mean, const float* g_var, float eps,
                               const float* bn_g, const float* bn_b, const int32_t* plan, int32_t N, int32_t E,
                               int32_t G, int32_t d, float* alpha, float* out, pm_stream_t stream) {
  if (!x || !g || !g_mean || !g_var || !bn_g || !bn_b || !plan || !alpha || !out || N <= 0 || G <= 0 || d <= 0)
    return PM_E_INVALID;
  PmPlanView pv = pm_plan_view(plan, N, E, G);
  hipLaunchKernelGGL(k_attnpool_fwd, dim3(G), dim3(256), 0, (hipStream_t)stream, x, g, g_mean, g_var, eps, bn_g, bn_b,
                     pv.bar_ptr, d, alpha, out);
  return pm_check_launch();
}

__global__ void __launch_bounds__(256) k_attnpool_bwd1(const float* __restrict__ x, const float* __restrict__ g,
                                                       const float* __restrict__ gm, const float* __restrict__ gv,
                                                       float eps, const float* __restrict__ alpha,
                                                       const float* __restrict__ dout, const int* __restrict__ bar_ptr,
                                                       int d, float* __restrict__ dgn, double* __restrict__ sums,
                                                       unsigned* gate) {
  __shared__ float sh[4];
  const int b = blockIdx.x;
  const int beg = bar_ptr[b], end = bar_ptr[b + 1];
  const int lane = threadIdx.x & 63, wave = threadIdx.x >> 6;
  for (int i = beg + wave; i < end; i += 4) {
    float s = 0.f;
    for (int c = lane * 4; c < d; c += 256) {
      const float4 xv = *reinterpret_cast<const float4*>(x + (int64_t)i * d + c);
      const float4 dv = *reinterpret_cast<const float4*>(dout + (int64_t)b * d + c);
      s += xv.x * dv.x + xv.y * dv.y + xv.z * dv.z + xv.w * dv.w;
    }
    s = pm_wave_sum(s);
    if (lane == 0) dgn[i] = s;
  }
  __syncthreads();
  float t = 0.f;
  for (int i = beg + threadIdx.x; i < end; i += blockDim.x) t += alpha[i] * dgn[i];
  t = block_sum(t, sh);
  const float mean = gm[0], rstd = rsqrtf(gv[0] + eps);
  float s0 = 0.f, s1 = 0.f;
  for (int i = beg + threadIdx.x; i < end; i += blockDim.x) {
    const float v = alpha[i] * (dgn[i] - t);
    dgn[i] = v;
    s0 += v;
    s1 += v * ((g[i] - mean) * rstd);
  }
  s0 = block_sum(s0, sh);
  s1 = block_sum(s1, sh);
  pm_turn_enter_block(gate);
  if (threadIdx.x == 0) { atomicAdd(&sums[0], (double)s0); atomicAdd(&sums[1], (double)s1); }
  pm_turn_leave_block(gate);
}
__global__ void __launch_bounds__(256) k_attnpool_bwd2(const float* __restrict__ x, const float* __restrict__ g,
                                                       const float* __restrict__ gm, const float* __restrict__ gv,
                                                       float eps, const float* __restrict__ bg,
                                                       const float* __restrict__ alpha, const float* __restrict__ dout,
                                                       const float* __restrict__ w, const int* __restrict__ node_bar,
                                                       const float* __restrict__ dgn, const double* __restrict__ sums,
                                                       int N, int d, float* __restrict__ dx, float* dW, float* db,
                                                       float* dbn_g, float* dbn_b, const float* __restrict__ xg,
                                                       float* __restrict__ dxg, const double* __restrict__ gsums,
                                                       double gcount, unsigned* gate) {
  extern __shared__ __attribute__((aligned(16))) float sW[];
  for (int i = threadIdx.x; i <= d; i += blockDim.x) sW[i] = 0.f;
  __syncthreads();
  const int lane = threadIdx.x & 63, wave = threadIdx.x >> 6;
  const float mean = gm[0], rstd = rsqrtf(gv[0] + eps), ga = bg[0];
  const float m0 = gsums ? (float)(gsums[0] / gcount) : (float)(sums[0] / N);
  const float m1 = gsums ? (float)(gsums[1] / gcount) : (float)(sums[1] / N);
  if (blockIdx.x == 0 && threadIdx.x == 0) { dbn_b[0] += (float)sums[0]; dbn_g[0] += (float)sums[1]; }
  float4 wacc[4];
#pragma unroll
  for (int k = 0; k < 4; ++k) wacc[k] = make_float4(0.f, 0.f, 0.f, 0.f);
  float bacc = 0.f;
  for (int n = blockIdx.x * 4 + wave; n < N; n += gridDim.x * 4) {
    const float gh = (g[n] - mean) * rstd;
    const float dg = ga * rstd * (dgn[n] - m0 - gh * m1);
    const float a = alpha[n];
    const int b = node_bar[n];
#pragma unroll
    for (int k = 0; k < 4; ++k) {
      const int c = lane * 4 + k * 256;
      if (c >= d) continue;
      const float4 xv = *reinterpret_cast<const float4*>(xg + (int64_t)n * d + c);
      const float4 dv = *reinterpret_cast<const float4*>(dout + (int64_t)b * d + c);
      const float4 wv = *reinterpret_cast<const float4*>(w + c);
      if (dxg) {
        *reinterpret_cast<float4*>(dx + (int64_t)n * d + c) = make_float4(a * dv.x, a * dv.y, a * dv.z, a * dv.w);
        *reinterpret_cast<float4*>(dxg + (int64_t)n * d + c) = make_float4(dg * wv.x, dg * wv.y, dg * wv.z, dg * wv.w);
      } else
      *reinterpret_cast<float4*>(dx + (int64_t)n * d + c) =
          make_float4(a * dv.x + dg * wv.x, a * dv.y + dg * wv.y, a * dv.z + dg * wv.z, a * dv.w + dg * wv.w);
      wacc[k].x += dg * xv.x; wacc[k].y += dg * xv.y; wacc[k].z += dg * xv.z; wacc[k].w += dg * xv.w;
    }
    bacc += dg;
  }
  for (int w = 0; w < (gate ? 4 : 1); ++w) {
    if (!gate || wave == w) {
#pragma unroll
      for (int k = 0; k < 4; ++k) {
        const int c = lane * 4 + k * 256;
        if (c >= d) continue;
        atomicAdd(&sW[c + 0], wacc[k].x); atomicAdd(&sW[c + 1], wacc[k].y);
        atomicAdd(&sW[c + 2], wacc[k].z); atomicAdd(&sW[c + 3], wacc[k].w);
      }
      if (lane == 0) atomicAdd(&sW[d], bacc);
    }
    if (gate) __syncthreads();
  }
  __syncthreads();
  pm_turn_enter_block(gate);
  for (int i = threadIdx.x; i < d; i += blockDim.x) atomicAdd(&dW[i], sW[i]);
  if (threadIdx.x == 0) atomicAdd(&db[0], sW[d]);
  pm_turn_leave_block(gate);
}
static int attnpool_bwd_impl(const float* x, const float* g, const float* g_mean, const float* g_var, float eps,
                             const float* bn_g, const float* alpha, const float* dout, const float* gate_w,
                             const int32_t* plan, int32_t N, int32_t E, int32_t G, int32_t d, float* dx, float* d_gate_w,
                             float* d_gate_b, float* d_bn_g, float* d_bn_b, float* scratch, const float* x_gate,
                             float* dx_gate, int phase, const double* gsums, double gcount, pm_stream_t stream) {
  if ((x_gate == nullptr) != (dx_gate == nullptr)) return PM_E_INVALID;
  if (!x || !g || !g_mean || !g_var || !alpha || !dout || !plan || !scratch || N <= 0 || G <= 0 || d <= 0 || (d & 3) ||
      d > 1024 || ((uintptr_t)scratch & 7))
    return PM_E_INVALID;
  if (phase != 1 && (!bn_g || !gate_w || !dx || !d_gate_w || !d_gate_b || !d_bn_g || !d_bn_b)) return PM_E_INVALID;
  hipStream_t st = (hipStream_t)stream;
  PmPlanView pv = pm_plan_view(plan, N, E, G);
  double* sums = reinterpret_cast<double*>(scratch);
  float* dgn = scratch + 4;
  if (phase != 2) {
    hipMemsetAsync(sums, 0, 2 * sizeof(double), st);
    hipLaunchKernelGGL(k_attnpool_bwd1, dim3(G), dim3(256), 0, st, x, g, g_mean, g_var, eps, alpha, dout, pv.bar_ptr, d,
                       dgn, sums, pm_det_gate(st));
  }
  if (phase != 1) {
    int nb = (int)pm_cdiv(N, 4);
    if (nb > 256) nb = 256;
    hipLaunchKernelGGL(k_attnpool_bwd2, dim3(nb), dim3(256), sizeof(float) * (d + 1), st, x, g, g_mean, g_var, eps, bn_g,
                       alpha, dout, gate_w, pv.node_bar, dgn, sums, N, d, dx, d_gate_w, d_gate_b, d_bn_g, d_bn_b,
                       x_gate ? x_gate : x, dx_gate, gsums, gcount, pm_det_gate(st));
  }
  return pm_check_launch();
}
extern "C" int pm_attnpool_bwd(const float* x, const float* g, const float* g_mean, const float* g_var, float eps,
                               const float* bn_g, const float* alpha, const float* dout, const float* gate_w,
                               const int32_t* plan, int32_t N, int32_t E, int32_t G, int32_t d, float* dx,
                               float* d_gate_w, float* d_gate_b, float* d_bn_g, float* d_bn_b, float* scratch,
                               const float* x_gate, float* dx_gate, pm_stream_t stream) {
  return attnpool_bwd_impl(x, g, g_mean, g_var, eps, bn_g, alpha, dout, gate_w, plan, N, E, G, d, dx, d_gate_w, d_gate_b,
                           d_bn_g, d_bn_b, scratch, x_gate, dx_gate, 0, nullptr, 0.0, stream);
}
extern "C" int pm_attnpool_bwd_sums(const float* x, const float* g, const float* g_mean, const float* g_var, float eps,
                                    const float* alpha, const float* dout, const int32_t* plan, int32_t N, int32_t E,
                                    int32_t G, int32_t d, float* scratch, pm_stream_t stream) {
  return attnpool_bwd_impl(x, g, g_mean, g_var, eps, nullptr, alpha, dout, nullptr, plan, N, E, G, d, nullptr, nullptr,
                           nullptr, nullptr, nullptr, scratch, nullptr, nullptr, 1, nullptr, 0.0, stream);
}
extern "C" int pm_attnpool_bwd_from_sums(const float* x, const float* g, const float* g_mean, const float* g_var, float eps,
                                         const float* bn_g, const float* alpha, const float* dout, const float* gate_w,
                                         const int32_t* plan, int32_t N, int32_t E, int32_t G, int32_t d, float* dx,
                                         float* d_gate_w, float* d_gate_b, float* d_bn_g, float* d_bn_b, float* scratch,
                                         const float* x_gate, float* dx_gate, const double* sums_global,
                                         double count_global, pm_stream_t stream) {
  if (!sums_global || !(count_global > 0)) return PM_E_INVALID;
  return attnpool_bwd_impl(x, g, g_mean, g_var, eps, bn_g, alpha, dout, gate_w, plan, N, E, G, d, dx, d_gate_w, d_gate_b,
                           d_bn_g, d_bn_b, scratch, x_gate, dx_gate, 2, sums_global, count_global, stream);
}

__global__ void __launch_bounds__(256) k_bar_bcast_fwd(const float* __restrict__ bars, const int* __restrict__ node_bar,
                                                       int N, int d, float* __restrict__ x) {
  const int n = blockIdx.x * 4 + (threadIdx.x >> 6);
  if (n >= N) return;
  const int b = node_bar[n];
  for (int c = (threadIdx.x & 63) * 4; c < d; c += 256)
    *reinterpret_cast<float4*>(x + (int64_t)n * d + c) = *reinterpret_cast<const float4*>(bars + (int64_t)b * d + c);
}
__global__ void __launch_bounds__(256) k_bar_bcast_bwd(const float* __restrict__ dx, const int* __restrict__ bar_ptr,
                                                       int d, float* __restrict__ dbars) {
  const int b = blockIdx.x;
  const int beg = bar_ptr[b], end = bar_ptr[b + 1];
  for (int c = threadIdx.x; c < d; c += blockDim.x) {
    float acc = 0.f;
    for (int i = beg; i < end; ++i) acc += dx[(int64_t)i * d + c];
    dbars[(int64_t)b * d + c] = acc;
  }
}
extern "C" int pm_bar_broadcast_fwd(const float* bars, const int32_t* plan, int32_t N, int32_t E, int32_t G, int32_t d,
                                    float* x, pm_stream_t stream) {
  if (!bars || !plan || !x || N <= 0 || G <= 0 || d <= 0 || (d & 3)) return PM_E_INVALID;
  PmPlanView pv = pm_plan_view(plan, N, E, G);
  hipLaunchKernelGGL(k_bar_bcast_fwd, dim3(pm_cdiv(N, 4)), dim3(256), 0, (hipStream_t)stream, bars, pv.node_bar, N, d, x);
  return pm_check_launch();
}
extern "C" int pm_bar_broadcast_bwd(const float* dx, const int32_t* plan, int32_t N, int32_t E, int32_t G, int32_t d,
                                    float* dbars, pm_stream_t stream) {
  if (!dx || !plan || !dbars || N <= 0 || G <= 0 || d <= 0) return PM_E_INVALID;
  PmPlanView pv = pm_plan_view(plan, N, E, G);
  hipLaunchKernelGGL(k_bar_bcast_bwd, dim3(G), dim3(256), 0, (hipStream_t)stream, dx, pv.bar_ptr, d, dbars);
  return pm_check_launch();
}
```

polyphemus_amd/csrc/segreduce.hip:

```cpp
#include "common.h"
#include <string.h>
#include <stdlib.h>
#include "prof.h"

extern "C" uint32_t pm_dropout_hash(uint32_t seed, uint32_t layer_uid, uint32_t eid, uint32_t channel) {
  return pm_elem_hash(pm_edge_key(seed, layer_uid, eid), channel) >> 8;
}

__global__ void k_edge_table(const float* __restrict__ w, const float* __restrict__ b, int d, float* T) {
  const int i = blockIdx.x * blockDim.x + threadIdx.x;
  if (i >= PM_N_DIST * d) return;
  const int dist = i / d, c = i % d;
  T[i] = w[c * PM_N_DIST + dist] + b[c];
}
__global__ void k_edge_table_bwd(const float* __restrict__ dT, int d, float* dw, float* db) {
  const int c = blockIdx.x * blockDim.x + threadIdx.x;
  if (c >= d) return;
  float s = 0.f;
  for (int dist = 0; dist < PM_N_DIST; ++dist) {
    const float g = dT[dist * d + c];
    dw[c * PM_N_DIST + dist] += g;
    s += g;
  }
  db[c] += s;
// ... 65 lines not shown
    const float inv = 1.0f / (float)(cnt > 1 ? cnt : 1);
#pragma unroll
    for (int v = 0; v < NV; ++v) {
      if (!ok[v]) continue;
      float4 o = make_float4(acc[v].x * inv, acc[v].y * inv, acc[v].z * inv, acc[v].w * inv);
      if (planes) pm_store_planes4(planes, plane_stride, arow + (int64_t)blk * d + c[v], o.x, o.y, o.z, o.w);
      else *reinterpret_cast<float4*>(A + arow + (int64_t)blk * d + c[v]) = o;
    }
    beg = end;
  }
#pragma unroll
  for (int v = 0; v < NV; ++v) {
    if (!ok[v]) continue;
    const float4 xs = *reinterpret_cast<const float4*>(x + (int64_t)n * d + c[v]);
    if (planes) pm_store_planes4(planes, plane_stride, arow + (int64_t)(nblk - 1) * d + c[v], xs.x, xs.y, xs.z, xs.w);
    else *reinterpret_cast<float4*>(A + arow + (int64_t)(nblk - 1) * d + c[v]) = xs;
  }
}

static bool seg_xcd_aware() {
  constexpr bool on = true;
  return on;
}

static int segreduce_fwd_impl(const float* x, const float* T, const int32_t* plan, int32_t N, int32_t E, int32_t G,
                              int32_t d, float dropout_p, uint32_t seed, uint32_t layer_uid, int32_t compact, float* A,
                              uint16_t* planes, int64_t plane_stride, pm_stream_t stream) {
  if (!x || !T || !plan || (!A && !planes) || N <= 0 || d <= 0 || (d & 3) || d > 1024 || dropout_p < 0.f ||
      dropout_p >= 1.f)
    return PM_E_INVALID;
  if (planes && (plane_stride < (int64_t)N * (compact ? 4 : 7) * d || (plane_stride & 3) || ((uintptr_t)planes % 8)))
    return PM_E_INVALID;
  PmPlanView pv = pm_plan_view(plan, N, E, G);
  const int* trel = compact ? pv.node_trel : nullptr;
  hipStream_t st = (hipStream_t)stream;
  int nwg = (int)pm_cdiv(N, 4), xcd_chunk = 0;
  if (seg_xcd_aware() && nwg >= 64) { xcd_chunk = (int)pm_cdiv(nwg, 8); nwg = xcd_chunk * 8; }
  const dim3 grid(nwg), block(256);
  const bool drop = dropout_p > 0.f;
  const uint32_t thresh = pm_keep_threshold(dropout_p);
  const float scale = drop ? 1.0f / (1.0f - dropout_p) : 1.0f;
#define LAUNCH(NV, DR)                                                                                              \
  hipLaunchKernelGGL((k_segreduce_fwd<NV, DR>), grid, block, 0, st, x, T, pv.rowptr, pv.csr_src, pv.csr_dist,       \
                     pv.csr_eid, N, d, seed, layer_uid, thresh, scale, trel, A, planes, plane_stride, xcd_chunk)
  const int nv = (int)pm_cdiv(d, 256);
  const double bytes_out = (planes ? 6.0 : 4.0) * d * (double)N * (compact ? 4 : 7);
  const int pe = pm_prof_open(st, PM_PROF_SEGREDUCE_FWD, 4.0 * d * (double)N + bytes_out + 12.0 * E);
  if (nv == 1) { if (drop) LAUNCH(1, true); else LAUNCH(1, false); }
  else if (nv == 2) { if (drop) LAUNCH(2, true); else LAUNCH(2, false); }
  else { if (drop) LAUNCH(4, true); else LAUNCH(4, false); }
#undef LAUNCH
  pm_prof_close(st, pe);
  return pm_check_launch();
}
extern "C" int pm_segreduce_fwd(const float* x, const float* T, const int32_t* plan, int32_t N, int32_t E, int32_t G,
                                int32_t d, float dropout_p, uint32_t seed, uint32_t layer_uid, int32_t compact, float* A,
                                pm_stream_t stream) {
  if (!A) return PM_E_INVALID;
  return segreduce_fwd_impl(x, T, plan, N, E, G, d, dropout_p, seed, layer_uid, compact, A, nullptr, 0, stream);
}
extern "C" int pm_segreduce_fwd_planes(const float* x, const float* T, const int32_t* plan, int32_t N, int32_t E,
                                       int32_t G, int32_t d, float dropout_p, uint32_t seed, uint32_t layer_uid,
                                       int32_t compact, uint16_t* planes, int64_t plane_stride, pm_stream_t stream) {
  if (!planes) return PM_E_INVALID;
  return segreduce_fwd_impl(x, T, plan, N, E, G, d, dropout_p, seed, layer_uid, compact, nullptr, planes, plane_stride,
                            stream);
}

#ifndef SEG_KEEP
#define SEG_KEEP 1
#endif
#ifndef SEG_EPT
#define SEG_EPT 4
#endif
template <int NV, bool DROP, bool FUSE, bool RL>
__global__ void __launch_bounds__(1024) k_segreduce_bwd(const float* __restrict__ x, const float* __restrict__ T,
                                                       const float* __restrict__ dA, const float* __restrict__ dres,
                                                       const int* __restrict__ colptr, const int* __restrict__ csc_dst,
                                                       const int* __restrict__ csc_reldist,
                                                       const int* __restrict__ csc_eid,
                                                       const float* __restrict__ csc_invcnt, int N, int d,
                                                       uint32_t seed, uint32_t layer_uid, uint32_t thresh, float scale,
                                                       int compact, float* __restrict__ dx, float* __restrict__ dT,
                                                       PmNormSums nn, int xcd_nodes, int pr, unsigned* gate) {
  constexpr int EPT = NV == 1 ? SEG_EPT : 2;
  extern __shared__ __attribute__((aligned(16))) float sT[];
  const int nwv0 = blockDim.x >> 6;
  for (int i = threadIdx.x; i < (PM_N_DIST + nwv0 * pr) * d + 1; i += blockDim.x) sT[i] = 0.f;
  __syncthreads();
  const int lane = threadIdx.x & 63;
  const int wave = threadIdx.x >> 6;
  float* const sP = sT + PM_N_DIST * d + wave * pr * d;
  const int nblk = compact ? 4 : 7;
  const int dq = d >> 2;
  int c[NV];
  bool ok[NV];
#pragma unroll
  for (int v = 0; v < NV; ++v) { c[v] = (lane + v * 64) * 4; ok[v] = c[v] < d; }
  const int nwv = blockDim.x >> 6;
  constexpr bool KEEP = NV == 1 && SEG_KEEP;
  float nm[NV][4], nrs[NV][4], nga[NV][4], nbe[NV][4];
  double ns0[NV][4], ns1[NV][4], ns2[NV][4];
  if (FUSE) {
#pragma unroll
    for (int v = 0; v < NV; ++v)
#pragma unroll
      for (int j = 0; j < 4; ++j) {
        const int col = ok[v] ? c[v] + j : 0;
        if (KEEP) {
          nm[v][j] = nn.mean[col]; nrs[v][j] = rsqrtf(nn.var[col] + nn.eps); nga[v][j] = nn.gamma[col]; nbe[v][j] = nn.beta[col];
        }
        ns0[v][j] = 0; ns1[v][j] = 0; ns2[v][j] = 0;
      }
  }
  float z0[NV][4];
#pragma unroll
  for (int v = 0; v < NV; ++v)
#pragma unroll
    for (int j = 0; j < 4; ++j) z0[v][j] = 0.f;
  float amax = 0.f;
  unsigned* const sMax = reinterpret_cast<unsigned*>(sT + (PM_N_DIST + nwv0 * pr) * d);
  int n_lo = blockIdx.x * nwv, n_hi = N, n_step = gridDim.x * nwv;
  if (xcd_nodes > 0) {
    n_lo = (blockIdx.x & 7) * xcd_nodes + (blockIdx.x >> 3) * nwv;
    n_hi = min(N, ((int)(blockIdx.x & 7) + 1) * xcd_nodes);
    n_step = (gridDim.x >> 3) * nwv;
  }
  float run[NV][4];
#pragma unroll
  for (int v = 0; v < NV; ++v)
#pragma unroll
    for (int j = 0; j < 4; ++j) run[v][j] = 0.f;
  int cur = -1;
  auto flush_run = [&](int v, int dist_r) {
    if (dist_r < 0) return;
    {
      if (dist_r == 0) {
#pragma unroll
        for (int j = 0; j < 4; ++j) z0[v][j] += run[v][j];
      } else if (dist_r <= pr) {
        float4* pp = reinterpret_cast<float4*>(sP + (dist_r - 1) * d + c[v]);
        float4 t = *pp;
        t.x += run[v][0]; t.y += run[v][1]; t.z += run[v][2]; t.w += run[v][3];
        *pp = t;
      } else {
        float* row = sT + dist_r * d + (c[v] >> 2);
#pragma unroll
        for (int j = 0; j < 4; ++j)
          if (run[v][j] != 0.f) atomicAdd(row + j * dq, run[v][j]);
      }
#pragma unroll
      for (int j = 0; j < 4; ++j) run[v][j] = 0.f;
    }
  };
  for (int n0 = n_lo; n0 < n_hi; n0 += n_step) {
    const int n = __builtin_amdgcn_readfirstlane(n0 + wave);
    if (n >= n_hi) continue;
    float4 xv[NV], acc[NV];
    int beg, end;
    {
#pragma unroll
    for (int v = 0; v < NV; ++v) {
      if (!ok[v]) continue;
      xv[v] = *reinterpret_cast<const float4*>(x + (int64_t)n * d + c[v]);
      acc[v] = *reinterpret_cast<const float4*>(dA + ((int64_t)n * nblk + (nblk - 1)) * d + c[v]);
      if (dres) {
        const float4 rv = *reinterpret_cast<const float4*>(dres + (int64_t)n * d + c[v]);
        acc[v].x += rv.x; acc[v].y += rv.y; acc[v].z += rv.z; acc[v].w += rv.w;
      }
    }
    beg = colptr[n]; end = colptr[n + 1];
    }
    struct Meta { int dst[EPT], dist[EPT], blk[EPT]; float w[EPT]; uint32_t key[EPT]; };
    auto load_meta = [&](Meta& m, int p) __attribute__((always_inline)) {
#pragma unroll
      for (int u = 0; u < EPT; ++u) {
        const bool live = p + u < end;
        const int q = live ? p + u : end - 1;
        m.dst[u] = csc_dst[q];
        const int rd = csc_reldist[q];
        const int r = rd & 0xff;
        m.dist[u] = rd >> 8;
        m.blk[u] = compact ? (r < 4 ? 0 : r - 3) : r;
        m.w[u] = live ? csc_invcnt[q] * scale : 0.f;
        m.key[u] = DROP ? pm_edge_key(seed, layer_uid, (uint32_t)csc_eid[q]) : 0u;
      }
    };
    Meta mt;
    for (int p = beg; p < end; p += EPT) {
      load_meta(mt, p);
      const int (&dst)[EPT] = mt.dst, (&dist)[EPT] = mt.dist, (&blk)[EPT] = mt.blk;
      const float (&w)[EPT] = mt.w;
      const uint32_t (&key)[EPT] = mt.key;
      int prev[EPT];
      prev[0] = cur;
#pragma unroll
      for (int u = 1; u < EPT; ++u) prev[u] = dist[u - 1];
#pragma unroll
      for (int v = 0; v < NV; ++v) {
        if (!ok[v]) continue;
        float4 g4[EPT], tv[EPT];
#pragma unroll
        for (int u = 0; u < EPT; ++u) {
          g4[u] = *reinterpret_cast<const float4*>(dA + ((int64_t)dst[u] * nblk + blk[u]) * d + c[v]);
          tv[u] = *reinterpret_cast<const float4*>(T + dist[u] * d + c[v]);
        }
        const float xs[4] = {xv[v].x, xv[v].y, xv[v].z, xv[v].w};
        float* ap = reinterpret_cast<float*>(&acc[v]);
#pragma unroll
        for (int u = 0; u < EPT; ++u) {
          const float g[4] = {g4[u].x * w[u], g4[u].y * w[u], g4[u].z * w[u], g4[u].w * w[u]};
          const float ts[4] = {tv[u].x, tv[u].y, tv[u].z, tv[u].w};
          float gt[4];
          const uint32_t gh = DROP ? pm_group_hash(key[u], c[v] >> 2) : 0u;
#pragma unroll
          for (int j = 0; j < 4; ++j) {
            bool on = xs[j] * ts[j] > 0.f;
            if (DROP) on = on && ((pm_lane_hash(gh, j) >> 8) >= thresh);
            const float gg = on ? g[j] : 0.f;
            ap[j] += gg * ts[j];
            gt[j] = gg * xs[j];
          }
          if (RL) {
            if (dist[u] != prev[u]) flush_run(v, prev[u]);
#pragma unroll
            for (int j = 0; j < 4; ++j) run[v][j] += gt[j];
          } else {
#pragma unroll
            for (int j = 0; j < 4; ++j) run[v][j] = gt[j];
            flush_run(v, dist[u]);
          }
        }
      }
      cur = dist[EPT - 1];
    }
    if (RL) {
#pragma unroll
      for (int v = 0; v < NV; ++v)
        if (ok[v]) flush_run(v, cur);
    }
    cur = -1;
#pragma unroll
    for (int v = 0; v < NV; ++v) {
      if (!ok[v]) continue;
      *reinterpret_cast<float4*>(dx + (int64_t)n * d + c[v]) = acc[v];
      if (FUSE) {
        if constexpr (NV == 1)
          amax = fmaxf(fmaxf(amax, fmaxf(fabsf(acc[v].x), fabsf(acc[v].y))), fmaxf(fabsf(acc[v].z), fabsf(acc[v].w)));
        const float4 hv = *reinterpret_cast<const float4*>(nn.h + (int64_t)n * d + c[v]);
        const float hs[4] = {hv.x, hv.y, hv.z, hv.w};
        const float ds[4] = {acc[v].x, acc[v].y, acc[v].z, acc[v].w};
        float m4[4], r4[4], g4n[4], b4[4];
        if (KEEP) {
#pragma unroll
          for (int j = 0; j < 4; ++j) { m4[j] = nm[v][j]; r4[j] = nrs[v][j]; g4n[j] = nga[v][j]; b4[j] = nbe[v][j]; }
        } else {
          const float4 mv = *reinterpret_cast<const float4*>(nn.mean + c[v]), vv = *reinterpret_cast<const float4*>(nn.var + c[v]);
          const float4 gv = *reinterpret_cast<const float4*>(nn.gamma + c[v]), bv = *reinterpret_cast<const float4*>(nn.beta + c[v]);
          m4[0] = mv.x; m4[1] = mv.y; m4[2] = mv.z; m4[3] = mv.w;
          r4[0] = rsqrtf(vv.x + nn.eps); r4[1] = rsqrtf(vv.y + nn.eps); r4[2] = rsqrtf(vv.z + nn.eps); r4[3] = rsqrtf(vv.w + nn.eps);
          g4n[0] = gv.x; g4n[1] = gv.y; g4n[2] = gv.z; g4n[3] = gv.w;
          b4[0] = bv.x; b4[1] = bv.y; b4[2] = bv.z; b4[3] = bv.w;
        }
#pragma unroll
        for (int j = 0; j < 4; ++j) {
          const float xh = (hs[j] - m4[j]) * r4[j];
          float du = ds[j];
          if (nn.relu && !(xh * g4n[j] + b4[j] > 0.f)) du = 0.f;
          ns0[v][j] += (double)du; ns1[v][j] += (double)du * (double)xh; ns2[v][j] += (double)xh;
        }
      }
    }
  }
#pragma unroll
  for (int v = 0; v < NV; ++v) {
    if (!ok[v]) continue;
#pragma unroll
    for (int j = 0; j < 4; ++j)
      if (z0[v][j] != 0.f) atomicAdd(&sT[j * dq + (c[v] >> 2)], z0[v][j]);
  }
  if (FUSE && NV == 1 && nn.absmax_out) {
    amax = pm_wave_max(amax);
    if (lane == 0) atomicMax(sMax, __float_as_uint(amax));
  }
  __syncthreads();
  if (FUSE && NV == 1 && nn.absmax_out && threadIdx.x == 0) atomicMax(nn.absmax_out + (blockIdx.x % PM_ABSMAX_SLOTS), *sMax);
  for (int i = threadIdx.x; i < pr * d; i += blockDim.x) {
    const int r = i / d, col = i - r * d;
    float t = 0.f;
    for (int w = 0; w < nwv0; ++w) t += sT[PM_N_DIST * d + (w * pr + r) * d + col];
    sT[(r + 1) * d + (col & 3) * dq + (col >> 2)] += t;
  }
  __syncthreads();
  pm_turn_enter_block(gate);
  for (int i = threadIdx.x; i < PM_N_DIST * d; i += blockDim.x) {
    const int col = i % d;
    const float v = sT[i - col + (col & 3) * dq + (col >> 2)];
    if (v != 0.f) atomicAdd(&dT[i], v);
  }
  if (FUSE) {
    __syncthreads();
    double* sd = reinterpret_cast<double*>(sT);
    for (int r = 0; r * 4 < nwv; ++r) {
      if ((wave >> 2) == r) {
        double* slot = sd + (int64_t)(wave & 3) * 3 * d;
#pragma unroll
        for (int v = 0; v < NV; ++v) {
          if (!ok[v]) continue;
#pragma unroll
          for (int j = 0; j < 4; ++j) {
            const int col = c[v] + j;
            if (r == 0) { slot[col] = ns0[v][j]; slot[d + col] = ns1[v][j]; slot[2 * d + col] = ns2[v][j]; }
            else { slot[col] += ns0[v][j]; slot[d + col] += ns1[v][j]; slot[2 * d + col] += ns2[v][j]; }
          }
        }
      }
      __syncthreads();
    }
    const int nslot = nwv < 4 ? nwv : 4;
    double* dst = nn.acc3 + (int64_t)(blockIdx.x % PM_BN_REPL) * 3 * d;
    for (int i = threadIdx.x; i < 3 * d; i += blockDim.x) {
      double t = 0;
      for (int q = 0; q < nslot; ++q) t += sd[(int64_t)q * 3 * d + i];
      atomicAdd(&dst[i], t);
    }
  }
  pm_turn_leave_block(gate);
}

template <int NV, bool DR, bool FU, bool RL>
static void seg_bwd_lds_attr(size_t lds) {
  static size_t granted_dev[16] = {};
  size_t& granted = granted_dev[pm_device_slot()];
  if (granted == 0) granted = 64 * 1024;
  if (lds > granted) {
    hipFuncSetAttribute(reinterpret_cast<const void*>(&k_segreduce_bwd<NV, DR, FU, RL>),
                        hipFuncAttributeMaxDynamicSharedMemorySize, (int)lds);
    granted = lds;
  }
}

static int segreduce_bwd_impl(const float* x, const float* T, const float* dA, const float* dres, const int32_t* plan,
                              int32_t N, int32_t E, int32_t G, int32_t d, float dropout_p, uint32_t seed,
                              uint32_t layer_uid, int32_t compact, float* dx, float* dT, const PmNormSums* nn,
                              pm_stream_t stream) {
  if (!x || !T || !dA || !plan || !dx || !dT || N <= 0 || d <= 0 || (d & 3) || d > 1024 || dropout_p < 0.f ||
      dropout_p >= 1.f)
    return PM_E_INVALID;
  if (nn && (!nn->h || !nn->mean || !nn->var || !nn->gamma || !nn->beta || !nn->acc3)) return PM_E_INVALID;
  PmPlanView pv = pm_plan_view(plan, N, E, G);
  hipStream_t st = (hipStream_t)stream;
  unsigned* const gate = pm_det_gate(st);
  constexpr int dev_waves = 0;
  constexpr int dev_blocks = 0;
  const int threads = gate ? 64 : (N >= 4096 ? (dev_waves > 0 && dev_waves <= 16 ? dev_waves * 64 : 1024) : 256);
  int nblk = (int)pm_cdiv(N, threads / 64);
  const int cap = gate ? 512 : (dev_blocks > 0 ? dev_blocks : 256);
  if (nblk > cap) nblk = cap;
  const dim3 grid(nblk), block(threads);
  int xcd_nodes = 0;
  if (seg_xcd_aware() && nblk >= 16 && (nblk & 7) == 0) xcd_nodes = (int)pm_cdiv(pm_cdiv(N, 8), threads / 64) * (threads / 64);
  constexpr int pr_cap = 4;
  int pr = (int)((144 * 1024 / sizeof(float) / d - PM_N_DIST) / (threads / 64));
  if (pr > pr_cap) pr = pr_cap;
  if (pr < 0) pr = 0;
  const size_t lds = sizeof(float) * ((PM_N_DIST + (size_t)(threads / 64) * pr) * d + 4);
  const bool drop = dropout_p > 0.f;
  const uint32_t thresh = pm_keep_threshold(dropout_p);
  const float scale = drop ? 1.0f / (1.0f - dropout_p) : 1.0f;
  PmNormSums none;
  memset(&none, 0, sizeof(none));
  const PmNormSums nv_ = nn ? *nn : none;
#define LAUNCH(NV, DR, FU, RL)                                                                                       \
  do { seg_bwd_lds_attr<NV, DR, FU, RL>(lds);                                                                     \
  hipLaunchKernelGGL((k_segreduce_bwd<NV, DR, FU, RL>), grid, block, lds, st, x, T, dA, dres, pv.colptr, pv.csc_dst,  \
                     pv.csc_reldist, pv.csc_eid, pv.csc_invcnt, N, d, seed, layer_uid, thresh, scale, compact, dx, dT, nv_, xcd_nodes, pr, gate); } while (0)
  const bool rl = d <= 256 || (int64_t)E >= 16 * (int64_t)N;
#define LAUNCH2(NV, DR) do { if (nn) { if (rl) LAUNCH(NV, DR, true, true); else LAUNCH(NV, DR, true, false); }       \
                             else { if (rl) LAUNCH(NV, DR, false, true); else LAUNCH(NV, DR, false, false); } } while (0)
  const int nv = (int)pm_cdiv(d, 256);
  const int pe = pm_prof_open(st, PM_PROF_SEGREDUCE_BWD, 4.0 * d * (double)N * ((compact ? 4 : PM_N_REL + 1) + 1 + (dres ? 1 : 0) + (nn ? 1 : 0)) + 12.0 * E + 128.0 * d);
  if (nv == 1) { if (drop) LAUNCH2(1, true); else LAUNCH2(1, false); }
  else if (nv == 2) { if (drop) LAUNCH2(2, true); else LAUNCH2(2, false); }
  else { if (drop) LAUNCH2(4, true); else LAUNCH2(4, false); }
#undef LAUNCH2
#undef LAUNCH
  pm_prof_close(st, pe);
  return pm_check_launch();
}
extern "C" int pm_segreduce_bwd(const float* x, const float* T, const float* dA, const float* dres, const int32_t* plan,
                                int32_t N, int32_t E, int32_t G, int32_t d, float dropout_p, uint32_t seed,
                                uint32_t layer_uid, int32_t compact, float* dx, float* dT, pm_stream_t stream) {
  return segreduce_bwd_impl(x, T, dA, dres, plan, N, E, G, d, dropout_p, seed, layer_uid, compact, dx, dT, nullptr, stream);
}
extern "C" int pm_segreduce_bwd_norm(const float* x, const float* T, const float* dA, const float* dres,
                                     const int32_t* plan, int32_t N, int32_t E, int32_t G, int32_t d, float dropout_p,
                                     uint32_t seed, uint32_t layer_uid, int32_t compact, float* dx, float* dT,
                                     const PmNormSums* next_norm, pm_stream_t stream) {
  if (!next_norm) return PM_E_INVALID;
  return segreduce_bwd_impl(x, T, dA, dres, plan, N, E, G, d, dropout_p, seed, layer_uid, compact, dx, dT, next_norm, stream);
}
```

polyphemus_amd/csrc/vae_step.hip:

```cpp
#include "common.h"
#include <stdio.h>
#include <string.h>
#include <mutex>

int pm_plan_build_marked(const int64_t* edge_index, const int32_t* edge_type, const int32_t* edge_dist, const int64_t* bars,
                         const int64_t* batch, const uint8_t* is_drum, const int32_t* tokens, int32_t n_bars, int32_t n_slots,
                         int32_t N, int32_t E, int32_t G, int32_t* plan, hipStream_t stream, hipEvent_t after_count);
extern "C" int pm_kld_acc(const float* mu, const float* log_var, int32_t B, int32_t d, float beta, float* dmu, float* dlog_var,
                          double* out, pm_stream_t stream);
extern "C" int pm_chord_sum_fwd_absmax(const float* PT, const float* cvec, const int32_t* tokens, const uint8_t* is_drum, int32_t N, int32_t d,
                                       int32_t n_slots, float* x0, uint32_t* absmax, pm_stream_t stream);
extern "C" int pm_bn_bwd_sums_absmax(const float* x, const float* dy, int32_t O, int32_t C, const float* mean, const float* var, float eps,
                                     const float* gamma, const float* beta, int relu, double* acc3, uint32_t* absmax_dy,
                                     pm_stream_t stream);
extern "C" int pm_bce_logits_acc(const float* logits, const float* target, int64_t n, float grad_scale, float* dlogits, double* out,
                                 pm_stream_t stream);
namespace {

struct StepCfg {
  bool gcl_fused, no_dw, no_rows_w, no_classes, fused_ce, debug;
  int side_stream;
  int side_delay_us;
  bool dagg_bn;
  bool dagg_res;
  bool chord_tables;
  bool plan_side;
  bool h2;
  bool senc_first;
  bool unembed_dw;
  bool pad_skip;
  bool cnn_fused;
  bool bar_route;
  int64_t offset_limit;
};
static StepCfg read_cfg() {
  auto flag = [](const char* n, bool dflt) { const char* v = getenv(n); return v ? atoi(v) != 0 : dflt; };
  StepCfg k;
  k.gcl_fused = flag("PM_GCL_FUSED", true);
  k.no_dw = flag("PM_GCL_NO_DW", false);
  k.no_rows_w = flag("PM_NO_ROWS_W", false);
  k.no_classes = getenv("PM_GCL_NO_CLASSES") != nullptr;
  k.fused_ce = flag("PM_FUSED_CE", true);
  k.debug = getenv("PM_DEBUG") != nullptr;
  k.side_stream = getenv("PM_SIDE_STREAM") ? atoi(getenv("PM_SIDE_STREAM")) : 0xffff;
  k.dagg_bn = flag("PM_DAGG_BN", true);
  k.plan_side = flag("PM_PLAN_SIDE", true);
  k.chord_tables = flag("PM_CHORD_TABLES", true);
  k.dagg_res = flag("PM_DAGG_RES", true);
  k.h2 = flag("PM_H2", true);
  k.side_delay_us = getenv("PM_SIDE_DELAY_US") ? atoi(getenv("PM_SIDE_DELAY_US")) : 0;
  k.bar_route = flag("PM_BAR_ROUTE", true);
  k.pad_skip = flag("PM_PAD_SKIP", true);
  k.unembed_dw = flag("PM_UNEMBED_DW", true);
  k.senc_first = flag("PM_SENC_FIRST", true);
  k.cnn_fused = flag("PM_CNN_FUSED", true);
  k.offset_limit = getenv("PM_GCL_OFFSET_LIMIT") ? atoll(getenv("PM_GCL_OFFSET_LIMIT")) : 0x7fffffffLL;
  return k;
}
static StepCfg g_cfg = read_cfg();
static const StepCfg& cfg() { return g_cfg; }

struct Arena {
  char* base; size_t cap, used; bool overflow;
  size_t zcap, zused;
  void* take(size_t bytes) {
    const size_t a = (used + 255) & ~size_t(255);
    used = a + bytes;
    if (!base) return nullptr;
    if (zcap + used > cap) { overflow = true; return base + zcap; }
    return base + zcap + a;
  }
  void* z(size_t bytes) {
    const size_t a = (zused + 255) & ~size_t(255);
    zused = a + bytes;
    if (!base) return nullptr;
    if (zused > zcap) { overflow = true; return base; }
    return base + a;
  }
  bool zeroed(const void* p) const { return base && (const char*)p >= base && (const char*)p < base + zcap; }
  float* f(size_t n) { return (float*)take(n * sizeof(float)); }
  double* dbl(size_t n) { return (double*)take(n * sizeof(double)); }
  float* zf(size_t n) { return (float*)z(n * sizeof(float)); }
  double* zdbl(size_t n) { return (double*)z(n * sizeof(double)); }
};

constexpr int kDenseDeg = 16;
struct GcnRoute {
  enum Agg { AGG_IN_PRODUCT, AGG_BAR, AGG_SEG_PLANES, AGG_SEG_F32 } agg;
  enum Mul { MUL_FUSED, MUL_FROM_PLANES, MUL_GROUPED, MUL_SEVEN } mul;
  bool h2;
  bool x_tracked;
  bool plain_w_planes;
  enum Norm { NORM_IN_DAGG, NORM_PASS, NORM_NONE } norm;
  bool res_in_dagg;
  enum Dagg { DAGG_BN, DAGG_TILES, DAGG_GROUPED, DAGG_SEVEN } dagg;
  enum Dw { DW_TILES, DW_GROUPED, DW_SEVEN } dw;
  enum Bagg { BAGG_SEG_DROPPED, BAGG_BAR, BAGG_SEG } bagg;
  bool bagg_sums;
  bool bagg_absmax;
  bool frag;
  int classes;
};
struct HeadRoute {
  enum Chord { CHORD_TABLES, CHORD_FULL, CHORD_FRAG, CHORD_TILES } chord;
  bool chord_dw_tn;
  bool dec_rows;
  bool dec_dw_tn;
  enum Ue { UE_KERNEL, UE_PRODUCTS } ue_fwd, ue_dh, ue_dw;
  bool ue_rows;
  bool keep_logits;
  bool logits_only;
  bool cnn_fused;
  bool metrics;
  bool plan_side, prep_main, senc_first;
  bool sw_fused_ce, sw_gcl_fused, sw_dagg_bn; int side_mask;
};

struct GcnSaved {
  GcnRoute rt;
  float* T; float* x[PM_MAX_LAYERS + 1]; float* A[PM_MAX_LAYERS]; float* h[PM_MAX_LAYERS];
  const float* xin[PM_MAX_LAYERS];
  uint32_t site0;
  float* mean[PM_MAX_LAYERS]; float* var[PM_MAX_LAYERS];
  uint16_t* Ap[PM_MAX_LAYERS];
  uint16_t* Wp; int64_t wp_stride; int64_t wp_base;
  uint16_t* Wfn; uint16_t* Wft; int64_t wf_stride;
  double* pool;
  uint32_t seed, uid0; float p;
  uint32_t* mx; uint32_t* mdu; float* sA; float* sdh;
  bool x0_maxed;
  const float* x0_src; int64_t x0_src_n;
};
constexpr float kH2WScale = 16.f;

struct StepState {
  uint64_t magic;
  PmVaeLayout lay;
  const float* P; float* Bf; float* G;
  PmBatch bt; const int32_t* plan; const float* eps;
  Arena ar;
  double* bn_scratch; double* bn_scratch_side; double* losses;
  float beta; int fix_structure;
  float *c0, *a0, *m0, *v0, *p0, *c1, *a1, *m1, *v1, *h1, *h2, *zcat;
  float *emb_stats, *X, *x0, *tables, *cvec; GcnSaved eg; float *g, *gm, *gv, *alpha, *pooled;
  float *m, *mm, *mv, *zg, *mu, *lv, *z;
  float *zd, *dm, *dv, *zr, *sb, *u1, *u2, *c2, *a2, *m2, *v2, *s_logits, *cb; GcnSaved dg; float *H, *c_logits;
  float *dc_logits, *ds_logits, *dmu, *dlv, *dz;
  HeadRoute head;
  int32_t* ue_lists; int32_t* ue_counts; float* dH;
  float* dc_logits_own;
  float* PT;
  uint16_t *wf_enc, *wf_enc_t, *wf_dec, *wf_dec_t, *w_unembed_dh;
  const float *a1d, *h1d, *x0d, *xLg, *zcat_d, *zg_d, *zr_d, *sbd, *u1d, *H_d;
  struct { float *a1, *h1, *x0, *xLg, *zcat, *zg, *zr, *sb, *u1; } dbuf;
  uint32_t seed_enc, seed_dec;
  float *bk_dx0, *bk_dzcat;
  float *bk_dxL;
  int rc;
  unsigned br_open;
  int ext_loss;
  int64_t* metrics;
  uint8_t* verdict;
};
constexpr uint64_t kMagic = 0x504d5354455031ULL;

struct Ctx {
  StepState* s; hipStream_t st; int rc;
  double* bn_scratch;
  int N, E, Gn, B, d, nb, L, S;
  bool bn;
  float pdrop;
  int compact;
  int planes;
  const float* P; float* G; float* Bf;
  void chk(int r, int line = __builtin_LINE()) {
    if (r != PM_OK && rc == PM_OK) {
      rc = r;
      if (cfg().debug) fprintf(stderr, "[polyphemus_hip] vae_step.hip:%d returned %d\n", line, r);
    }
  }
};

// ... 90 lines not shown
  w.a_colsum = want_bias ? c.G + l.b : nullptr;
  if (defer && defer->n < 8) defer->q[defer->n++] = w;
  else RUN(pm_gemm_f32_desc(&w, c.st));
  if (dx) RUN(pm_gemm_f32(0, 0, M, Kin, Nout, dy, lddy, c.P + l.w, Kin, dx, lddx ? lddx : Kin, nullptr,
                            c.s->ar.zeroed(dx) ? PM_GEMM_ZEROED : 0, 1, nullptr, 0, nullptr, c.st));
}
void bn_fwd(Ctx& c, const float* x, int O, int C, int I, PmBn bn, bool relu, const float* res, float* y, float* mean,
            float* var) {
  if (I == 1 && O <= PM_BN_SMALL_MAX_ROWS) {
    RUN(pm_bn_small_fwd(x, O, C, 1e-5f, c.P + bn.w, c.P + bn.b, res, relu ? 1 : 0, y, mean, var, c.Bf + bn.rm, c.Bf + bn.rv,
                          0.1f, c.st));
    return;
  }
  RUN(pm_bn_stats(x, O, C, I, mean, var, c.Bf + bn.rm, c.Bf + bn.rv, 0.1f, c.bn_scratch, c.st));
  RUN(pm_bn_apply(x, O, C, I, mean, var, 1e-5f, c.P + bn.w, c.P + bn.b, res, relu ? 1 : 0, y, c.st));
}
void bn_bwd(Ctx& c, const float* x, const float* dy, int O, int C, int I, PmBn bn, const float* mean, const float* var,
            bool relu, float* dx, float* dbias_pre = nullptr) {
  if (I == 1 && O <= PM_BN_SMALL_MAX_ROWS) {
    RUN(pm_bn_small_bwd(x, dy, O, C, mean, var, 1e-5f, c.P + bn.w, c.P + bn.b, relu ? 1 : 0, c.G + bn.w, c.G + bn.b,
                          dbias_pre, dx, c.st));
    return;
  }
  RUN(pm_bn_bwd(x, dy, O, C, I, mean, var, 1e-5f, c.P + bn.w, c.P + bn.b, relu ? 1 : 0, c.G + bn.w, c.G + bn.b,
                  dbias_pre, dx, c.bn_scratch, c.st));
}

enum { SITE_ENC_CNN_IN = 2001, SITE_ENC_CNN_MID, SITE_ENC_CHORD, SITE_ENC_GATE, SITE_ENC_MERGE_IN, SITE_ENC_MERGE_OUT, SITE_DEC_IN,
       SITE_DEC_CNN_IN, SITE_DEC_CNN_MID, SITE_DEC_CHORD, SITE_ENC_GCN = 2100, SITE_DEC_GCN = 2200 };
const float* drop(Ctx& c, const float* x, int64_t rows, int cols, uint32_t site, uint32_t seed, float* y) {
  if (!(c.pdrop > 0.f)) return x;
  RUN(pm_dropout_rows(x, rows, cols, c.pdrop, seed, site, y, c.st));
  return y;
}
static bool rows_tn_pays(int d) { return d >= 512 && d % 128 == 0; }
static bool gcl_width(int d) { return d == 128 || d == 256 || d == 512; }
static bool gcl_fits(int N, int d, int S) {
  const int64_t lim = cfg().offset_limit;
  return (int64_t)N * 4 * d * 6 < lim && (int64_t)N * 4 * d * 4 < lim && (int64_t)N * S * d * 4 < lim;
}
static bool rows_w_ok(const Ctx& c) { return gcl_width(c.d) && cfg().gcl_fused && gcl_fits(c.N, c.d, c.S) && !cfg().no_rows_w; }
static bool chord_tab_ok(const Ctx& c) { return cfg().chord_tables && c.d % 32 == 0 && c.d <= 512 && (int64_t)c.N * c.d * 4 < 0x7fffffffLL; }
static bool enc_frag_ok(const Ctx& c) { return rows_w_ok(c) && c.S < PM_N_SLOTS && !chord_tab_ok(c); }
static bool fused_ce_on() { return cfg().fused_ce; }
static bool unembed_dh_ok(const Ctx& c) {
  const int dh = c.d / 2;
  return cfg().fused_ce && (dh == 64 || dh == 128 || dh == 256) && (int64_t)c.N * c.S * (c.d > PM_N_TOK ? c.d : PM_N_TOK) * 4 < ((int64_t)1 << 31);
}
PmGemmDesc gcl_desc(const PmPlanView& pv, int N, int d, int classes) {
  PmGemmDesc q;
  memset(&q, 0, sizeof(q));
  q.flags = PM_GEMM_PARTITION; q.split_k = 1; q.rowmap = pv.trk_list; q.rows_per_entry = 1; q.dyn_entries = pv.trk_cnt;
  if (classes) { q.class_ptr = pv.trk_cnt + 8; q.class_block = d; }
  q.n_groups = 4; q.map_group_stride = N; q.dyn_group_stride = 1;
  return q;
}

GcnRoute gcn_route(const Ctx& c, const GcnSaved& sv) {
  const StepCfg& k = cfg();
  const int d = c.d;
  const bool dropping = c.pdrop > 0.f;
  GcnRoute r;
  r.frag = sv.Wfn && sv.Wft;
  r.classes = k.no_classes ? 0 : 1;
  const bool tiles = c.planes && c.compact && k.gcl_fused && gcl_fits(c.N, d, 1);
  const bool gcl_kernels = tiles && r.frag && gcl_width(d);
  const bool dense = (int64_t)c.E >= (int64_t)kDenseDeg * c.N;
  const bool bar = dense && c.compact && c.planes && (d % 128) == 0 && k.bar_route && !pm_det_on();
  const bool fused = gcl_kernels && !dense;
  const bool from_planes = gcl_kernels && dense && d == 512;
  r.agg = fused ? GcnRoute::AGG_IN_PRODUCT : bar ? GcnRoute::AGG_BAR : c.planes ? GcnRoute::AGG_SEG_PLANES : GcnRoute::AGG_SEG_F32;
  r.mul = fused ? GcnRoute::MUL_FUSED : from_planes ? GcnRoute::MUL_FROM_PLANES : c.compact ? GcnRoute::MUL_GROUPED : GcnRoute::MUL_SEVEN;
  r.plain_w_planes = c.planes && r.mul == GcnRoute::MUL_GROUPED;
  r.h2 = k.h2 && gcl_kernels && (!dense || (bar && d == 512)) && c.bn && (((d == 128 || d == 256) && k.dagg_bn) || d == 512) && !k.no_dw;
  r.x_tracked = r.h2 && !dropping;
  const bool in_dagg = c.bn && tiles && r.frag && (d == 128 || d == 256) && k.dagg_bn;
  r.norm = in_dagg ? GcnRoute::NORM_IN_DAGG : c.bn ? GcnRoute::NORM_PASS : GcnRoute::NORM_NONE;
  r.res_in_dagg = in_dagg && !dropping && k.dagg_res;
  r.dagg = !c.compact ? GcnRoute::DAGG_SEVEN : in_dagg ? GcnRoute::DAGG_BN : gcl_kernels ? GcnRoute::DAGG_TILES : GcnRoute::DAGG_GROUPED;
  r.dw = !c.compact ? GcnRoute::DW_SEVEN : (tiles && gcl_width(d) && !k.no_dw) ? GcnRoute::DW_TILES : GcnRoute::DW_GROUPED;
  r.bagg = dropping ? GcnRoute::BAGG_SEG_DROPPED : bar ? GcnRoute::BAGG_BAR : GcnRoute::BAGG_SEG;
  r.bagg_sums = d <= 512 && c.bn && !dropping;
  r.bagg_absmax = r.h2 && (d <= 256 || bar);
  return r;
}
HeadRoute head_route(const Ctx& c) {
  const StepCfg& k = cfg();
  const StepState& s = *c.s;
  const int d = c.d, dh = d / 2;
  const int64_t R = (int64_t)c.N * c.S;
  HeadRoute r;
  r.chord = chord_tab_ok(c) ? HeadRoute::CHORD_TABLES : c.S == PM_N_SLOTS ? HeadRoute::CHORD_FULL
          : enc_frag_ok(c) ? HeadRoute::CHORD_FRAG : HeadRoute::CHORD_TILES;
  r.chord_dw_tn = r.chord == HeadRoute::CHORD_FRAG && rows_tn_pays(d);
  r.dec_rows = rows_w_ok(c);
  r.dec_dw_tn = r.dec_rows && rows_tn_pays(d);
  r.keep_logits = (s.bt.flags & 4) != 0;
  r.logits_only = (s.bt.flags & 8) != 0;
  r.metrics = !r.logits_only && s.metrics != nullptr;
  r.plan_side = k.plan_side;
  r.prep_main = r.chord == HeadRoute::CHORD_TABLES && r.plan_side;
  r.senc_first = k.senc_first;
  r.cnn_fused = k.cnn_fused && c.bn;
  r.ue_fwd = (fused_ce_on() && !r.logits_only) ? HeadRoute::UE_KERNEL : HeadRoute::UE_PRODUCTS;
  r.ue_dh = unembed_dh_ok(c) ? HeadRoute::UE_KERNEL : HeadRoute::UE_PRODUCTS;
  r.ue_rows = k.pad_skip && fused_ce_on() && r.plan_side && unembed_dh_ok(c) && !r.logits_only;
  r.ue_dw = (k.unembed_dw && dh % 128 == 0 && !pm_det_on() && R * PM_N_TOK * 4 < ((int64_t)1 << 31) && R * (int64_t)d * 4 < ((int64_t)1 << 31))
                ? HeadRoute::UE_KERNEL : HeadRoute::UE_PRODUCTS;
  r.sw_fused_ce = k.fused_ce; r.sw_gcl_fused = k.gcl_fused; r.sw_dagg_bn = k.dagg_bn;
  r.side_mask = k.side_stream;
  return r;
}
void head_route_gradient_in_any_row(HeadRoute& r) { r.ue_rows = false; }
void gcn_prepare(Ctx& c, const PmGcn& g, GcnSaved& sv) {
  Arena& ar = c.s->ar;
  const int d = c.d;
  const int64_t dd = (int64_t)d * d;
  sv.T = ar.f((size_t)PM_N_DIST * d);
  if (ar.base) RUN(pm_edge_table(c.P + g.nn_w, c.P + g.nn_b, d, sv.T, c.st));
  sv.pool = ar.zdbl((size_t)c.L * 5 * d * PM_BN_REPL);
  {
    constexpr int SL = PM_ABSMAX_SLOTS;
    uint32_t* w = (uint32_t*)ar.z(sizeof(uint32_t) * (size_t)((2 * c.L + 1) * SL + 2 * c.L));
    sv.mx = w; sv.mdu = w ? w + (c.L + 1) * SL : nullptr; sv.sA = w ? (float*)(w + (2 * c.L + 1) * SL) : nullptr;
    sv.sdh = w ? sv.sA + c.L : nullptr;
  }
  const int64_t lstride = c.L > 2 ? g.weight[2] - g.weight[1] : 7 * dd;
  sv.Wfn = sv.Wft = nullptr; sv.wf_stride = 7 * dd * 3;
  if (c.planes) {
    sv.wp_base = g.weight[0];
    sv.wp_stride = (g.weight[c.L - 1] + 7 * dd - g.weight[0] + 7) & ~(int64_t)7;
    for (int i = 0; i < c.L; ++i)
      if (g.weight[i] < sv.wp_base || ((g.weight[i] - sv.wp_base) & 7)) RUN(PM_E_INVALID);
    sv.Wp = (uint16_t*)ar.take((size_t)sv.wp_stride * 6);
    bool even = (d % 32) == 0 && c.compact && (lstride % 4) == 0;
    for (int i = 2; i < c.L; ++i) even = even && (g.weight[i] - g.weight[i - 1] == lstride);
    if (even) {
      sv.Wfn = (uint16_t*)ar.take((size_t)sv.wf_stride * 2 * c.L);
      sv.Wft = (uint16_t*)ar.take((size_t)sv.wf_stride * 2 * c.L);
    }
  }
  const GcnRoute& r = sv.rt = gcn_route(c, sv);
  if (r.frag) {
    auto split = [&](const float* W, int n_mats, int64_t src_stride, int kind, uint16_t* dst) {
      if (r.h2) RUN(pm_split_planes_frag_h2(W, 7 * d, d, kind, n_mats, src_stride, sv.wf_stride, kH2WScale, dst, c.st));
      else RUN(pm_split_planes_frag(W, 7 * d, d, kind, n_mats, src_stride, sv.wf_stride, dst, c.st));
    };
    for (int kind = 0; kind < 2; ++kind) {
      uint16_t* dst = kind ? sv.Wfn : sv.Wft;
      split(c.P + g.weight[0], 1, 7 * dd, kind, dst);
      if (c.L > 1) split(c.P + g.weight[1], c.L - 1, lstride, kind, dst + sv.wf_stride);
    }
    if (r.h2) RUN(pm_absmax(sv.T, (int64_t)PM_N_DIST * d, sv.mx + c.L * PM_ABSMAX_SLOTS, c.st));
  }
  if (r.plain_w_planes)
    RUN(pm_split_planes(c.P + sv.wp_base, sv.wp_stride & ~(int64_t)3, sv.Wp, sv.wp_stride, c.st));
}

float* gcn_forward(Ctx& c, float* x0, const PmGcn& g, GcnSaved& sv, uint32_t seed, uint32_t uid0, float p) {
  Arena& ar = c.s->ar;
  const int N = c.N, d = c.d, nb = c.compact ? 4 : 7;
  const int64_t dd = (int64_t)d * d;
  sv.seed = seed; sv.uid0 = uid0; sv.p = p;
  PmPlanView pv;
  if (ar.base) pv = pm_plan_view(c.s->plan, N, c.E, c.Gn);
  sv.x[0] = x0;
// ... 2 lines not shown
  const bool dropping = c.pdrop > 0.f;
  sv.site0 = uid0 == 0 ? SITE_ENC_GCN : SITE_DEC_GCN;
  for (int i = 0; i < c.L; ++i) {
    if (c.planes) { sv.Ap[i] = (uint16_t*)ar.take((size_t)aps * 6); sv.A[i] = nullptr; }
    else sv.A[i] = ar.f((size_t)N * nb * d);
    sv.h[i] = ar.f((size_t)N * d); sv.x[i + 1] = ar.f((size_t)N * d);
    sv.mean[i] = ar.f(d); sv.var[i] = ar.f(d);
    float* xdrop = dropping ? ar.f((size_t)N * d) : nullptr;
    if (!ar.base) continue;
    sv.xin[i] = drop(c, sv.x[i], N, d, sv.site0 + i, seed, xdrop);
    const float* W = c.P + g.weight[i];
    const float* bias = c.P + g.bias[i];
    const uint16_t* Wf = r.frag ? sv.Wfn + (int64_t)i * sv.wf_stride : nullptr;
    double* sums = c.bn ? sv.pool + (size_t)i * 5 * d * PM_BN_REPL : nullptr;
    PmH2 h2;
    if (r.h2) {
      if (!(r.x_tracked && i > 0)) {
        if (i == 0 && sv.x0_maxed && !dropping) {}
        else if (i == 0 && sv.x0_src && !dropping) RUN(pm_absmax(sv.x0_src, sv.x0_src_n, sv.mx, c.st));
        else RUN(pm_absmax(sv.xin[i], (int64_t)N * d, sv.mx + i * PM_ABSMAX_SLOTS, c.st));
      }
      h2.absmax_in = sv.mx + i * PM_ABSMAX_SLOTS; h2.absmax_aux = sv.mx + c.L * PM_ABSMAX_SLOTS; h2.scale_out = sv.sA + i;
      h2.w_scale = kH2WScale; h2.reserved = 0;
    }
    switch (r.agg) {
      case GcnRoute::AGG_IN_PRODUCT:
        if (r.h2)
          RUN(pm_gcl_forward_fused_h2(sv.xin[i], sv.T, c.s->plan, N, c.E, c.Gn, d, p, seed, uid0 + i, Wf, bias, r.classes,
                                        sv.h[i], sums, sv.Ap[i], aps, &h2, c.st));
        else
          RUN(pm_gcl_forward_fused(sv.xin[i], sv.T, c.s->plan, N, c.E, c.Gn, d, p, seed, uid0 + i, Wf, bias, r.classes,
                                     sv.h[i], sums, sv.Ap[i], aps, c.st));
        break;
      case GcnRoute::AGG_BAR:
        RUN(pm_bar_aggregate_fwd(sv.xin[i], sv.T, c.s->plan, N, c.E, c.Gn, d, p, seed, uid0 + i, sv.Ap[i], aps, r.h2 ? &h2 : nullptr, c.st)); break;
      case GcnRoute::AGG_SEG_PLANES:
        RUN(pm_segreduce_fwd_planes(sv.xin[i], sv.T, c.s->plan, N, c.E, c.Gn, d, p, seed, uid0 + i, 1, sv.Ap[i], aps, c.st)); break;
      case GcnRoute::AGG_SEG_F32:
        RUN(pm_segreduce_fwd(sv.xin[i], sv.T, c.s->plan, N, c.E, c.Gn, d, p, seed, uid0 + i, c.compact, sv.A[i], c.st)); break;
    }
    switch (r.mul) {
      case GcnRoute::MUL_FUSED: break;
      case GcnRoute::MUL_FROM_PLANES:
        if (r.h2)
          RUN(pm_gcl_forward_from_planes_h2(sv.Ap[i], aps, c.s->plan, N, c.E, c.Gn, d, Wf, bias, r.classes, sv.h[i], sums,
                                              sv.sA + i, kH2WScale, c.st));
        else
          RUN(pm_gcl_forward_from_planes(sv.Ap[i], aps, c.s->plan, N, c.E, c.Gn, d, Wf, bias, r.classes, sv.h[i], sums, c.st));
        break;
      case GcnRoute::MUL_SEVEN: {
        PmGemmDesc q;
        memset(&q, 0, sizeof(q));
        q.M = N; q.N = d; q.K = 7 * d; q.split_k = 1; q.n_groups = 1;
        q.A = sv.A[i]; q.lda = 7 * d; q.B = W; q.ldb = d; q.C = sv.h[i]; q.ldc = d; q.bias = bias;
        q.col_stats = sums;
        RUN(pm_gemm_f32_desc(&q, c.st));
        break;
      }
      case GcnRoute::MUL_GROUPED: {
        PmGemmDesc q = gcl_desc(pv, N, d, r.classes);
        q.M = N; q.N = d; q.K = 4 * d;
        q.A = sv.A[i]; q.lda = 4 * d; q.B = W; q.ldb = d; q.C = sv.h[i]; q.ldc = d; q.bias = bias;
        q.b_group_stride = dd; q.b_split_rows = d; q.b_shared_off = 3 * dd;
        q.col_stats = sums;
        if (c.planes) {
          q.operand_planes = 1; q.A = (const float*)sv.Ap[i]; q.a_plane_stride = aps;
          q.B = (const float*)(sv.Wp + (g.weight[i] - sv.wp_base)); q.b_plane_stride = sv.wp_stride;
          q.b_frag = Wf;
        }
        RUN(pm_gemm_f32_desc(&q, c.st));
        break;
      }
    }
    const PmBn& bn = g.norm[i];
    if (c.bn)
      RUN(pm_bn_apply_fused_absmax(sv.h[i], N, d, sums, 1e-5f, c.P + bn.w, c.P + bn.b, sv.x[i], 1, sv.x[i + 1], sv.mean[i],
                                     sv.var[i], c.Bf + bn.rm, c.Bf + bn.rv, 0.1f,
                                     (r.x_tracked && i + 1 < c.L) ? sv.mx + (i + 1) * PM_ABSMAX_SLOTS : nullptr, c.st));
    else
      RUN(pm_relu_residual_fwd(sv.h[i], sv.x[i], (int64_t)N * d, sv.x[i + 1], c.st));
  }
  return sv.x[c.L];
}
float* gcn_backward(Ctx& c, float* dx, const PmGcn& g, GcnSaved& sv) {
  Arena& ar = c.s->ar;
  const int N = c.N, d = c.d, nb = c.compact ? 4 : 7;
  const int64_t dd = (int64_t)d * d;
  float* dT = ar.zf((size_t)PM_N_DIST * d);
  float* dh = ar.f((size_t)N * d);
  float* dA = ar.f((size_t)N * nb * d);
  const int64_t aps = (int64_t)N * nb * d, dps = (int64_t)N * d;
  uint16_t* const dhp = c.planes ? (uint16_t*)ar.take((size_t)dps * 6) : nullptr;
  float* dxa = ar.f((size_t)N * d);
  float* dxb = ar.f((size_t)N * d);
  PmPlanView pv = pm_plan_view(c.s->plan, N, c.E, c.Gn);
  float* dxin = c.pdrop > 0.f ? ar.f((size_t)N * d) : nullptr;
  const GcnRoute& r = sv.rt;
  for (int i = c.L - 1; i >= 0; --i) {
    const float* W = c.P + g.weight[i];
    float* dW = c.G + g.weight[i];
    const PmBn& bn = g.norm[i];
    const uint16_t* Wf = r.frag ? sv.Wft + (int64_t)i * sv.wf_stride : nullptr;
    double* const acc3 = sv.pool + ((size_t)i * 5 + 2) * d * PM_BN_REPL;
    const bool sums_ready = i < c.L - 1 && r.bagg_sums;
    const bool du_tracked = sums_ready && r.bagg_absmax, du_from_sums = r.norm == GcnRoute::NORM_IN_DAGG && !sums_ready;
    PmH2 h2 = {};
    if (r.h2) { h2.absmax_in = sv.mdu + i * PM_ABSMAX_SLOTS; h2.scale_out = sv.sdh + i; h2.w_scale = kH2WScale; }
    switch (r.norm) {
      case GcnRoute::NORM_IN_DAGG:
        if (!sums_ready)
          RUN(pm_bn_bwd_sums_absmax(sv.h[i], dx, N, d, sv.mean[i], sv.var[i], 1e-5f, c.P + bn.w, c.P + bn.b, 1, acc3,
                                      (r.h2 && du_from_sums) ? sv.mdu + i * PM_ABSMAX_SLOTS : nullptr, c.st));
        break;
      case GcnRoute::NORM_PASS:
        if (r.h2) {
          if (!du_tracked) RUN(pm_absmax(dx, (int64_t)N * d, sv.mdu + i * PM_ABSMAX_SLOTS, c.st));
          RUN(pm_bn_bwd_fused_h2(sv.h[i], dx, N, d, sv.mean[i], sv.var[i], 1e-5f, c.P + bn.w, c.P + bn.b, 1, c.G + bn.w, c.G + bn.b,
                                   c.G + g.bias[i], acc3, dhp, dps, sums_ready ? 1 : 0, &h2, c.st));
        } else
          RUN(pm_bn_bwd_fused(sv.h[i], dx, N, d, sv.mean[i], sv.var[i], 1e-5f, c.P + bn.w, c.P + bn.b, 1, c.G + bn.w,
                                c.G + bn.b, c.G + g.bias[i], c.planes ? nullptr : dh, acc3, dhp, dps, sums_ready ? 1 : 0, c.st));
        break;
      case GcnRoute::NORM_NONE:
        RUN(pm_relu_bwd_planes(dx, sv.h[i], (int64_t)N * d, dh, c.planes ? dhp : nullptr, dps, c.st));
        RUN(pm_colsum_acc(dh, N, d, d, c.G + g.bias[i], c.st));
        break;
    }
    switch (r.dagg) {
      case GcnRoute::DAGG_SEVEN:
        RUN(pm_gemm_f32(0, 1, N, 7 * d, d, dh, d, W, d, dA, 7 * d, nullptr, 0, 1, nullptr, 0, nullptr, c.st)); break;
      case GcnRoute::DAGG_BN: {
        PmBnBwd nb;
        nb.h = sv.h[i]; nb.du = dx; nb.mean = sv.mean[i]; nb.var = sv.var[i]; nb.gamma = c.P + bn.w; nb.beta = c.P + bn.b;
        nb.acc3 = acc3; nb.dgamma = c.G + bn.w; nb.dbeta = c.G + bn.b; nb.dbias_pre = c.G + g.bias[i]; nb.eps = 1e-5f; nb.relu = 1;
        nb.add_residual = r.res_in_dagg ? 1 : 0; nb.reserved = 0;
        if (r.h2) {
          if (!du_tracked && !du_from_sums) RUN(pm_absmax(dx, (int64_t)N * d, sv.mdu + i * PM_ABSMAX_SLOTS, c.st));
          RUN(pm_gcl_input_grad_bn_h2(&nb, dhp, dps, c.s->plan, N, c.E, c.Gn, d, Wf, r.classes, dA, &h2, c.st));
        } else
          RUN(pm_gcl_input_grad_bn(&nb, dhp, dps, c.s->plan, N, c.E, c.Gn, d, Wf, r.classes, dA, c.st));
        break;
      }
      case GcnRoute::DAGG_TILES:
        if (r.h2)
          RUN(pm_gcl_input_grad_fused_h2(dhp, dps, c.s->plan, N, c.E, c.Gn, d, Wf, r.classes, dA, sv.sdh + i, kH2WScale, c.st));
        else
          RUN(pm_gcl_input_grad_fused(dhp, dps, c.s->plan, N, c.E, c.Gn, d, Wf, r.classes, dA, c.st));
        break;
      case GcnRoute::DAGG_GROUPED: {
        PmGemmDesc q = gcl_desc(pv, N, d, r.classes);
        q.transB = 1; q.M = N; q.N = 4 * d; q.K = d;
        q.A = dh; q.lda = d; q.B = W; q.ldb = d; q.C = dA; q.ldc = 4 * d;
        q.b_group_stride = dd; q.b_split_rows = d; q.b_shared_off = 3 * dd;
        if (c.planes) {
          q.operand_planes = 1; q.A = (const float*)dhp; q.a_plane_stride = dps;
          q.B = (const float*)(sv.Wp + (g.weight[i] - sv.wp_base)); q.b_plane_stride = sv.wp_stride;
          q.b_frag = Wf;
        }
        RUN(pm_gemm_f32_desc(&q, c.st));
        break;
      }
    }
    switch (r.dw) {
      case GcnRoute::DW_SEVEN:
        RUN(pm_gemm_f32(1, 0, 7 * d, d, N, sv.A[i], 7 * d, dh, d, dW, d, nullptr, PM_GEMM_ACCUM, 0, nullptr, 0, nullptr, c.st)); break;
      case GcnRoute::DW_TILES:
        if (r.h2)
          RUN(pm_gcl_weight_grad_fused_h2(sv.Ap[i], aps, dhp, dps, c.s->plan, N, c.E, c.Gn, d, r.classes, dW, sv.sA + i, sv.sdh + i, c.st));
        else
          RUN(pm_gcl_weight_grad_fused(sv.Ap[i], aps, dhp, dps, c.s->plan, N, c.E, c.Gn, d, r.classes, dW, c.st));
        break;
      case GcnRoute::DW_GROUPED: {
        PmGemmDesc w = gcl_desc(pv, N, d, r.classes);
        w.transA = 1; w.M = 4 * d; w.N = d; w.K = N; w.flags = PM_GEMM_ACCUM | PM_GEMM_PARTITION; w.split_k = 0;
        w.A = sv.A[i]; w.lda = 4 * d; w.B = dh; w.ldb = d; w.C = dW; w.ldc = d;
        w.c_group_stride = dd; w.c_split_rows = d; w.c_shared_off = 3 * dd;
        if (c.planes) {
          w.operand_planes = 1; w.A = (const float*)sv.Ap[i]; w.a_plane_stride = aps;
          w.B = (const float*)dhp; w.b_plane_stride = dps;
        }
        RUN(pm_gemm_f32_desc(&w, c.st));
        break;
      }
    }
    float* out = (dx == dxa) ? dxb : dxa;
    const float* res = r.res_in_dagg ? nullptr : dx;
    PmNormSums nn;
    const bool carry = i > 0 && r.bagg_sums;
    if (carry) {
      const PmBn& pb = g.norm[i - 1];
      nn.h = sv.h[i - 1]; nn.mean = sv.mean[i - 1]; nn.var = sv.var[i - 1]; nn.gamma = c.P + pb.w; nn.beta = c.P + pb.b;
      nn.eps = 1e-5f; nn.relu = 1; nn.acc3 = sv.pool + ((size_t)(i - 1) * 5 + 2) * d * PM_BN_REPL;
      nn.absmax_out = r.bagg_absmax ? sv.mdu + (i - 1) * PM_ABSMAX_SLOTS : nullptr;
    }
    switch (r.bagg) {
      case GcnRoute::BAGG_SEG_DROPPED:
        RUN(pm_segreduce_bwd(sv.xin[i], sv.T, dA, nullptr, c.s->plan, N, c.E, c.Gn, d, sv.p, sv.seed, sv.uid0 + i, c.compact, dxin,
                               dT, c.st));
        drop(c, dxin, N, d, sv.site0 + i, sv.seed, dxin);
        RUN(pm_add(dx, dxin, (int64_t)N * d, out, c.st));
        break;
      case GcnRoute::BAGG_BAR:
        RUN(pm_bar_aggregate_bwd(sv.x[i], sv.T, dA, res, c.s->plan, N, c.E, c.Gn, d, sv.p, sv.seed, sv.uid0 + i, out, dT,
                                   carry ? &nn : nullptr, c.st));
        break;
      case GcnRoute::BAGG_SEG:
        if (carry)
          RUN(pm_segreduce_bwd_norm(sv.x[i], sv.T, dA, res, c.s->plan, N, c.E, c.Gn, d, sv.p, sv.seed, sv.uid0 + i, c.compact, out,
                                      dT, &nn, c.st));
        else
          RUN(pm_segreduce_bwd(sv.x[i], sv.T, dA, res, c.s->plan, N, c.E, c.Gn, d, sv.p, sv.seed, sv.uid0 + i, c.compact, out, dT, c.st));
        break;
    }
    dx = out;
  }
  RUN(pm_edge_table_bwd(dT, d, c.G + g.nn_w, c.G + g.nn_b, c.st));
  return dx;
}

Ctx make_ctx(StepState* s, hipStream_t st) {
  Ctx c;
  c.s = s; c.st = st; c.rc = PM_OK; c.bn_scratch = s->bn_scratch;
  c.N = s->bt.N; c.E = s->bt.E; c.Gn = s->bt.G; c.B = s->bt.B;
  c.d = s->lay.d; c.nb = s->lay.n_bars; c.L = s->lay.n_layers;
  c.S = s->bt.n_slots;
  c.compact = (s->bt.flags & 1) ? 1 : 0;
  c.planes = (c.compact && (s->bt.flags & 2) && (s->lay.d % 8) == 0) ? 1 : 0;
  c.P = s->P; c.G = s->G; c.Bf = s->Bf;
  c.bn = !(s->lay.flags & 1); c.pdrop = s->lay.dropout;
  return c;
}


void cnn_act_fwd(Ctx& c, const float* x, int O, int C, int I, PmBn bn, float* y, float* mean, float* var) {
  if (c.bn) bn_fwd(c, x, O, C, I, bn, true, nullptr, y, mean, var);
  else RUN(pm_relu_residual_fwd(x, nullptr, (int64_t)O * C * I, y, c.st));
}
int64_t bn_scratch_len(const Ctx& c) { return (int64_t)PM_BN_SCRATCH(2 * c.d > 16 ? 2 * c.d : 16); }
void cnn_act_bwd(Ctx& c, const float* x, const float* dy, int O, int C, int I, PmBn bn, const float* mean, const float* var, float* dx) {
  if (c.bn) bn_bwd(c, x, dy, O, C, I, bn, mean, var, true, dx);
  else RUN(pm_relu_bwd(dy, x, (int64_t)O * C * I, dx, c.st));
}
#define EMB_PARAMS(base)                                                                                                       \
  base + Y.enc_pitch_d.w, base + Y.enc_pitch_d.b, base + Y.enc_pitch_nd.w, base + Y.enc_pitch_nd.b, base + Y.enc_dur.w,        \
  base + Y.enc_dur.b, base + Y.enc_bn_d.w, base + Y.enc_bn_d.b, base + Y.enc_bn_nd.w, base + Y.enc_bn_nd.b,                    \
  base + Y.enc_bn_dur.w, base + Y.enc_bn_dur.b
enum UeDir { UE_LOGITS, UE_DH, UE_DW };
void unembed_products(Ctx& c, UeDir dir, bool lists, float* dH) {
  StepState& s = *c.s;
  if (!s.ar.base) return;
  const PmVaeLayout& Y = s.lay;
  const int N = c.N, d = c.d, dh = d / 2;
  const int64_t R = (int64_t)N * c.S;
  const PmPlanView pv = pm_plan_view(s.plan, N, c.E, c.Gn);
  const PmLin head[3] = {Y.dec_dur, Y.dec_pitch_d, Y.dec_pitch_nd};
  for (int g = 0; g < 3; ++g) {
    const int n_out = g ? PM_N_PITCH : PM_N_DUR, col = g ? 0 : PM_N_PITCH, hoff = g ? 0 : dh;
    const int32_t* lst = g ? pv.row_list + (g == 2 ? (int64_t)N * PM_N_SLOTS : 0) : nullptr;
    const int32_t* cnt = g ? pv.group_cnt + 1 + g : nullptr;
    if (lists) { lst = s.ue_lists + (g + 2) % 3 * R; cnt = s.ue_counts + (g + 2) % 3; }
    const PmLin& w = head[g];
    switch (dir) {
      case UE_LOGITS:
        RUN(pm_gemm_f32(0, 1, (int)R, n_out, dh, s.H + hoff, d, c.P + w.w, dh, s.c_logits + col, PM_N_TOK, c.P + w.b, 0, 1, lst,
                          lst ? 1 : 0, cnt, c.st));
        break;
      case UE_DH:
        RUN(pm_gemm_f32(0, 0, (int)R, dh, n_out, s.dc_logits + col, PM_N_TOK, c.P + w.w, dh, dH + hoff, d, nullptr, 0, 1, lst,
                          lst ? 1 : 0, cnt, c.st));
        break;
      case UE_DW:
        RUN(pm_gemm_f32(1, 0, n_out, dh, (int)R, s.dc_logits + col, PM_N_TOK, s.H + hoff, d, c.G + w.w, dh, nullptr, PM_GEMM_ACCUM, 0,
                          lst, lst ? 1 : 0, cnt, c.st));
        break;
    }
  }
}

void carve_structure_encoder(Ctx& c) {
  StepState& s = *c.s; Arena& ar = s.ar;
  const int Gn = c.Gn, d = c.d;
  const bool dropping = c.pdrop > 0.f;
  s.zcat = ar.zf((size_t)c.B * 2 * d);
  s.c0 = ar.f((size_t)Gn * 8 * 128); s.a0 = ar.f((size_t)Gn * 8 * 128); s.m0 = ar.f(8); s.v0 = ar.f(8);
  s.p0 = ar.f((size_t)Gn * 8 * 32); s.c1 = ar.f((size_t)Gn * 16 * 32); s.a1 = ar.f((size_t)Gn * 512);
  s.m1 = ar.f(16); s.v1 = ar.f(16); s.h1 = ar.f((size_t)Gn * d); s.h2 = ar.zf((size_t)Gn * d);
  s.dbuf.a1 = dropping ? ar.f((size_t)Gn * 512) : nullptr;
  s.dbuf.h1 = dropping ? ar.f((size_t)Gn * d) : nullptr;
}
void chord_encoder_planes(Ctx& c, int kind) {
  StepState& s = *c.s;
  const int d = c.d;
// ... 272 lines not shown
  float* xd0 = decoder_trunk(c);
  if (run) branch_join(c, BR_WPREP_DEC);
  if (run) branch_join(c, BR_ENC_FWD);
  s.dg.x0_src = s.cb; s.dg.x0_src_n = (int64_t)c.Gn * c.d;
  float* xdL = gcn_forward(c, xd0, Y.dec_gcn, s.dg, seed_dec, 1000, msg_p);
  structure_decoder(c);
  decoder_head(c, xdL);
}

void structure_decoder_backward(Ctx& c, float* dzr) {
  StepState& s = *c.s; Arena& ar = s.ar; const PmVaeLayout& Y = s.lay;
  const int Gn = c.Gn, d = c.d;
  BranchScope br(c, BR_DEC_BWD);
  float* da2 = ar.f((size_t)Gn * 8 * 128); float* dc2 = ar.f((size_t)Gn * 8 * 128);
  float* du2 = ar.f((size_t)Gn * 512); float* du1 = ar.zf((size_t)Gn * d); float* dsb = ar.zf((size_t)Gn * d);
  RUN(pm_conv3x3_bwd_weight(s.a2, s.ds_logits, Gn, 8, 1, 4, 32, 0, c.G + Y.dec_conv4.w, c.G + Y.dec_conv4.b, c.st));
  RUN(pm_conv3x3_bwd_data(s.ds_logits, c.P + Y.dec_conv4.w, Gn, 8, 1, 4, 32, 0, da2, c.st));
  cnn_act_bwd(c, s.c2, da2, Gn, 8, 128, Y.dec_bn2, s.m2, s.v2, dc2);
  RUN(pm_conv3x3_bwd_weight(s.u2, dc2, Gn, 16, 8, 4, 32, 1, c.G + Y.dec_conv1.w, c.G + Y.dec_conv1.b, c.st));
  RUN(pm_conv3x3_bwd_data(dc2, c.P + Y.dec_conv1.w, Gn, 16, 8, 4, 32, 1, du2, c.st));
  RUN(pm_relu_bwd(du2, s.u2, (int64_t)Gn * 512, du2, c.st));
  lin_bwd(c, du2, s.u1d, Y.dec_s_lin4, Gn, 512, d, du1);
  drop(c, du1, Gn, d, SITE_DEC_CNN_MID, s.seed_dec, du1);
  RUN(pm_relu_bwd(du1, s.u1, (int64_t)Gn * d, du1, c.st));
  lin_bwd(c, du1, s.sbd, Y.dec_s_lin1, Gn, d, d, dsb);
  drop(c, dsb, Gn, d, SITE_DEC_CNN_IN, s.seed_dec, dsb);
  lin_bwd(c, dsb, s.zr_d, Y.dec_s_bars, c.B, c.nb * d, d, dzr, 0, 2 * d, 2 * d);
}
void unembed_input_grad(Ctx& c) {
  StepState& s = *c.s; const PmVaeLayout& Y = s.lay;
  const HeadRoute& rt = s.head;
  const int N = c.N, d = c.d, S = c.S;
  if (rt.ue_dh == HeadRoute::UE_PRODUCTS) unembed_products(c, UE_DH, false, s.dH);
  else if (rt.ue_rows)
    RUN(pm_unembed_dh_rows(s.dc_logits, c.P + Y.dec_pitch_d.w, c.P + Y.dec_pitch_nd.w, c.P + Y.dec_dur.w, s.plan, N, c.E, c.Gn, d, S,
                             s.dH, s.w_unembed_dh, s.ue_lists, s.ue_counts, c.st));
  else
    RUN(pm_unembed_dh(s.dc_logits, c.P + Y.dec_pitch_d.w, c.P + Y.dec_pitch_nd.w, c.P + Y.dec_dur.w, s.plan, N, c.E, c.Gn, d, S,
                        s.dH, s.w_unembed_dh, 0, c.st));
  drop(c, s.dH, N, S * d, SITE_DEC_CHORD, s.seed_dec, s.dH);
}
void decoder_weight_grads(Ctx& c) {
  StepState& s = *c.s; const PmVaeLayout& Y = s.lay;
  const HeadRoute& rt = s.head;
  const int N = c.N, d = c.d, S = c.S;
  BranchScope br(c, BR_DEC_WGRAD);
  if (rt.ue_dw == HeadRoute::UE_KERNEL)
    RUN(pm_unembed_dw(s.dc_logits, s.H, s.plan, N, c.E, c.Gn, d, S, c.G + Y.dec_pitch_d.w, c.G + Y.dec_pitch_nd.w, c.G + Y.dec_dur.w,
                        rt.ue_rows ? s.ue_lists : nullptr, rt.ue_rows ? s.ue_counts : nullptr, c.st));
  else unembed_products(c, UE_DW, rt.ue_rows, nullptr);
  if (s.ext_loss) {
    RUN(pm_unembed_bias_grads(s.dc_logits, s.bt.is_drum, N, S, c.G + Y.dec_pitch_d.b, c.G + Y.dec_pitch_nd.b, c.G + Y.dec_dur.b, c.st));
  }
  if (rt.dec_dw_tn)
    RUN(pm_rows_tn_weight_grad(s.dH, S * d, S * d, s.dg.x[c.L], d, d, N, c.G + Y.dec_chord.w, d, c.G + Y.dec_chord.b, c.st));
  else if (rt.dec_rows) lin_bwd(c, s.dH, s.dg.x[c.L], Y.dec_chord, N, S * d, d, nullptr);
}
void decoder_trunk_backward(Ctx& c, float* dx0, float* dzr) {
  StepState& s = *c.s; Arena& ar = s.ar; const PmVaeLayout& Y = s.lay;
  const int N = c.N, Gn = c.Gn, B = c.B, d = c.d;
  float* dcb = ar.f((size_t)Gn * d);
  RUN(pm_bar_broadcast_bwd(dx0, s.plan, N, c.E, Gn, d, dcb, c.st));
  Deferred df;
  float* dzd = ar.zf((size_t)B * 2 * d);
  s.dz = ar.zf((size_t)B * d);
  lin_bwd(c, dcb, s.zr_d + d, Y.dec_c_bars, B, c.nb * d, d, dzr + d, 0, 2 * d, 2 * d, true, &df);
  branch_join(c, BR_DEC_BWD);
  drop(c, dzr, B, 2 * d, SITE_DEC_IN, s.seed_dec, dzr);
  bn_bwd(c, s.zd, dzr, B, 2 * d, 1, Y.dec_bn, s.dm, s.dv, true, dzd);
  lin_bwd(c, dzd, s.z, Y.dec_lin, B, 2 * d, d, s.dz, 0, 0, 0, true, &df);
  RUN(pm_reparam_bwd(s.dz, s.lv, s.eps, (int64_t)B * d, s.dmu, s.dlv, c.st));
  if (df.n) {
    BranchScope br(c, BR_DEC_WGRAD);
    flush_deferred(c, df);
  }
}
void backward_decoder(Ctx& c) {
  StepState& s = *c.s; const PmVaeLayout& Y = s.lay;
  const int N = c.N, d = c.d, S = c.S;
  float* dzr = s.ar.zf((size_t)c.B * 2 * d);
  if (s.fix_structure) structure_decoder_backward(c, dzr);
  unembed_input_grad(c);
  float* dxL = s.ar.f((size_t)N * d);
  if (s.head.dec_rows)
    RUN(pm_rows_times_weight_longk(s.dH, S * d, N, S * d, s.wf_dec_t, 1, 0, d, dxL, d, c.st));
  else
    lin_bwd(c, s.dH, s.dg.x[c.L], Y.dec_chord, N, S * d, d, dxL);
  float* dx0 = gcn_backward(c, dxL, Y.dec_gcn, s.dg);
  decoder_weight_grads(c);
  decoder_trunk_backward(c, dx0, dzr);
}

void backward_encoder_heads(Ctx& c) {
  StepState& s = *c.s;
  Arena& ar = s.ar;
  const PmVaeLayout& Y = s.lay;
  const int N = c.N, Gn = c.Gn, B = c.B, d = c.d, nb = c.nb, dh = d / 2;
  float* dzg = ar.zf((size_t)B * d); float* dzg2 = ar.zf((size_t)B * d);
  Deferred df;
  float* dm = ar.f((size_t)B * d);
  float* dzcat = ar.zf((size_t)B * 2 * d);
  float* dpooled = ar.zf((size_t)Gn * d);
  if (d % 64 == 0 && d >= 128) {
    lin_bwd(c, s.dmu, s.zg_d, Y.enc_mu, B, d, d, nullptr, 0, 0, 0, true, &df);
    lin_bwd(c, s.dlv, s.zg_d, Y.enc_lv, B, d, d, nullptr, 0, 0, 0, true, &df);
    RUN(pm_gemm_f32_grouped(0, 0, B, d, d, s.dmu, d, c.P + Y.enc_mu.w, d, dzg, d, nullptr, PM_GEMM_ACCUM | PM_GEMM_ZEROED,
                              d / 64 < 8 ? d / 64 : 8, nullptr, 0, nullptr, 2, s.dlv - s.dmu, (int64_t)Y.enc_lv.w - (int64_t)Y.enc_mu.w, 0, 0, 0, 0,
                              c.st));
  } else {
    lin_bwd(c, s.dmu, s.zg_d, Y.enc_mu, B, d, d, dzg, 0, 0, 0, true, &df);
    lin_bwd(c, s.dlv, s.zg_d, Y.enc_lv, B, d, d, dzg2, 0, 0, 0, true, &df);
    RUN(pm_add(dzg, dzg2, (int64_t)B * d, dzg, c.st));
  }
  drop(c, dzg, B, d, SITE_ENC_MERGE_OUT, s.seed_enc, dzg);
  bn_bwd(c, s.m, dzg, B, d, 1, Y.enc_bn_merge, s.mm, s.mv, true, dm);
  lin_bwd(c, dm, s.zcat_d, Y.enc_merge, B, d, 2 * d, dzcat, 0, 0, 0, true, &df);
  drop(c, dzcat, B, 2 * d, SITE_ENC_MERGE_IN, s.seed_enc, dzcat);
  {
    BranchScope br(c, BR_ENC_BWD);
    float* dh2 = ar.zf((size_t)Gn * d); float* dh1 = ar.zf((size_t)Gn * d); float* da1 = ar.zf((size_t)Gn * 512);
    float* dc1 = ar.f((size_t)Gn * 512); float* dp0 = ar.f((size_t)Gn * 8 * 32); float* da0 = ar.f((size_t)Gn * 8 * 128);
    float* dc0 = ar.f((size_t)Gn * 8 * 128);
    lin_bwd(c, dzcat + d, s.h2, Y.enc_s_bars, B, d, nb * d, dh2, 2 * d, nb * d, nb * d);
    lin_bwd(c, dh2, s.h1d, Y.enc_lin4, Gn, d, d, dh1);
    drop(c, dh1, Gn, d, SITE_ENC_CNN_MID, s.seed_enc, dh1);
    RUN(pm_relu_bwd(dh1, s.h1, (int64_t)Gn * d, dh1, c.st));
    lin_bwd(c, dh1, s.a1d, Y.enc_lin1, Gn, d, 512, da1);
    drop(c, da1, Gn, 512, SITE_ENC_CNN_IN, s.seed_enc, da1);
    if (s.head.cnn_fused) {
      RUN(pm_cnn_enc_bwd(s.bt.s_tensor, s.c0, s.a0, s.p0, s.c1, da1, s.m0, s.v0, c.P + Y.enc_bn1.w, c.P + Y.enc_bn1.b, s.m1, s.v1,
                           c.P + Y.enc_bn5.w, c.P + Y.enc_bn5.b, c.P + Y.enc_conv4.w, Gn, 1e-5f, c.G + Y.enc_conv0.w, c.G + Y.enc_conv0.b,
                           c.G + Y.enc_bn1.w, c.G + Y.enc_bn1.b, c.G + Y.enc_conv4.w, c.G + Y.enc_conv4.b, c.G + Y.enc_bn5.w,
                           c.G + Y.enc_bn5.b, nullptr, da0, nullptr, c.bn_scratch, bn_scratch_len(c), c.st));
    } else {
      cnn_act_bwd(c, s.c1, da1, Gn, 16, 32, Y.enc_bn5, s.m1, s.v1, dc1);
      RUN(pm_conv3x3_bwd_weight(s.p0, dc1, Gn, 8, 16, 4, 8, 0, c.G + Y.enc_conv4.w, c.G + Y.enc_conv4.b, c.st));
      RUN(pm_conv3x3_bwd_data(dc1, c.P + Y.enc_conv4.w, Gn, 8, 16, 4, 8, 0, dp0, c.st));
      RUN(pm_maxpool4_bwd(s.a0, dp0, (int64_t)Gn * 8 * 32, da0, c.st));
      cnn_act_bwd(c, s.c0, da0, Gn, 8, 128, Y.enc_bn1, s.m0, s.v0, dc0);
      RUN(pm_conv3x3_bwd_weight(s.bt.s_tensor, dc0, Gn, 1, 8, 4, 32, 0, c.G + Y.enc_conv0.w, c.G + Y.enc_conv0.b, c.st));
    }
  }
  lin_bwd(c, dzcat, s.pooled, Y.enc_c_bars, B, d, nb * d, dpooled, 2 * d, nb * d, nb * d, true, &df);
  if (df.n) {
    BranchScope br(c, BR_ENC_HEAD_WGRAD);
    flush_deferred(c, df);
  }
  float* dxL = ar.f((size_t)N * d);
  float* pscr = ar.f((size_t)3 * N + 8);
  const bool dropping = c.pdrop > 0.f;
  float* dxg = dropping ? ar.f((size_t)N * d) : nullptr;
  RUN(pm_attnpool_bwd(s.eg.x[c.L], s.g, s.gm, s.gv, 1e-5f, c.P + Y.enc_gate_bn.w, s.alpha, dpooled, c.P + Y.enc_gate.w,
                        s.plan, N, c.E, Gn, d, dxL, c.G + Y.enc_gate.w, c.G + Y.enc_gate.b, c.G + Y.enc_gate_bn.w,
                        c.G + Y.enc_gate_bn.b, pscr, dropping ? s.xLg : nullptr, dxg, c.st));
  if (dropping) {
    drop(c, dxg, N, d, SITE_ENC_GATE, s.seed_enc, dxg);
    RUN(pm_add(dxL, dxg, (int64_t)N * d, dxL, c.st));
  }
  branch_join(c, BR_DEC_WGRAD);
  s.bk_dxL = dxL; s.bk_dzcat = dzcat;
}
void backward_encoder(Ctx& c) {
  StepState& s = *c.s;
  const PmVaeLayout& Y = s.lay;
  const int N = c.N, d = c.d;
  if (!s.bk_dxL) backward_encoder_heads(c);
  float* dxL = s.bk_dxL;
  float* dzcat = s.bk_dzcat;
  s.bk_dxL = nullptr;
  float* dx0 = gcn_backward(c, dxL, Y.enc_gcn, s.eg);
  drop(c, dx0, N, d, SITE_ENC_CHORD, s.seed_enc, dx0);
  RUN(pm_relu_bwd(dx0, s.x0, (int64_t)N * d, dx0, c.st));
  branch_join(c, BR_ENC_HEAD_WGRAD);
  s.bk_dx0 = dx0; s.bk_dzcat = dzcat;
}
void backward_encoder_tail(Ctx& c) {
  StepState& s = *c.s;
  Arena& ar = s.ar;
  const PmVaeLayout& Y = s.lay;
  const int N = c.N, Gn = c.Gn, B = c.B, d = c.d, nb = c.nb, dh = d / 2;
  float* dx0 = s.bk_dx0;
  float* dzcat = s.bk_dzcat;
  const int S = c.S;
  const HeadRoute& rt = s.head;
  const bool chord_tab = chord_tab_ok(c);
  float* dX = chord_tab ? nullptr : ar.f((size_t)N * S * d);
  float* Stab = chord_tab ? ar.zf((size_t)4 * PM_N_PITCH * dh) : ar.f((size_t)4 * PM_N_PITCH * dh);
  float* gsum = ar.f((size_t)2 * d);
  float* Gt = chord_tab ? ar.zf((size_t)2 * S * 2 * PM_N_PITCH * d) : nullptr;
  if (rt.chord == HeadRoute::CHORD_TABLES) {
    {
      BranchScope br(c, BR_ENC_WGRAD);
      RUN(pm_chord_pad_bwd(dx0, s.bt.is_drum, N, d, S, s.tables, c.P + Y.enc_chord.w, gsum, c.G + Y.enc_chord.w, Stab, c.st));
      br.pause();
      RUN(pm_chord_sum_bwd(dx0, s.bt.tokens, s.plan, N, c.E, Gn, d, S, Gt, c.st));
      br.wait_main();
      br.resume();
      RUN(pm_chord_tables_bwd_x(Gt, c.P + Y.enc_chord.w, d, S, Stab, c.st));
      br.pause();
      RUN(pm_chord_tables_bwd_w(Gt, s.tables, d, S, c.G + Y.enc_chord.w, c.G + Y.enc_chord.b, c.st));
    }
    branch_join(c, BR_ENC_WGRAD);
  } else if (rt.chord == HeadRoute::CHORD_FULL) lin_bwd(c, dx0, s.X, Y.enc_chord, N, d, PM_N_SLOTS * d, dX);
  else {
    {
      BranchScope br(c, BR_ENC_WGRAD);
      if (rt.chord_dw_tn)
        RUN(pm_rows_tn_weight_grad(dx0, d, d, s.X, S * d, S * d, N, c.G + Y.enc_chord.w, PM_N_SLOTS * d, c.G + Y.enc_chord.b, c.st));
      else {
        PmGemmDesc w;
        memset(&w, 0, sizeof(w));
        w.transA = 1; w.M = d; w.N = S * d; w.K = N; w.A = dx0; w.lda = d; w.B = s.X; w.ldb = S * d;
        w.C = c.G + Y.enc_chord.w; w.ldc = PM_N_SLOTS * d; w.flags = PM_GEMM_ACCUM; w.split_k = 0; w.n_groups = 1;
        w.a_colsum = c.G + Y.enc_chord.b;
        RUN(pm_gemm_f32_desc(&w, c.st));
      }
    }
    if (rt.chord == HeadRoute::CHORD_FRAG)
      RUN(pm_rows_times_weight(dx0, d, N, d, s.wf_enc_t, 1, PM_N_SLOTS * d / 32, S * d, nullptr, dX, S * d, c.st));
    else
      RUN(pm_gemm_f32(0, 0, N, S * d, d, dx0, d, c.P + Y.enc_chord.w, PM_N_SLOTS * d, dX, S * d, nullptr, 0, 1, nullptr, 0,
                        nullptr, c.st));
  }
  if (rt.chord != HeadRoute::CHORD_TABLES) {
    RUN(pm_embed_bwd_scatter(dX, s.bt.tokens, s.plan, N, c.E, Gn, d, S, Stab, c.st));
    RUN(pm_chord_pad_bwd(dx0, s.bt.is_drum, N, d, S, s.tables, c.P + Y.enc_chord.w, gsum, c.G + Y.enc_chord.w, Stab, c.st));
  }
  PmPlanView pv = pm_plan_view(s.plan, N, c.E, Gn);
  RUN(pm_embed_tables_bwd(Stab, c.P + Y.enc_pitch_d.w, c.P + Y.enc_pitch_d.b, c.P + Y.enc_pitch_nd.w, c.P + Y.enc_pitch_nd.b,
                            c.P + Y.enc_dur.w, c.P + Y.enc_dur.b, c.P + Y.enc_bn_d.w, c.P + Y.enc_bn_nd.w,
                            c.P + Y.enc_bn_dur.w, s.emb_stats, pv.tok_hist, d, 1e-5f, EMB_PARAMS(c.G), c.st));
  branch_join(c, BR_ENC_WGRAD);
  branch_join(c, BR_ENC_BWD);
}

void measure_backward(Ctx& c) {
  c.s->fix_structure = 1;
  backward_decoder(c);
  backward_encoder(c);
  backward_encoder_tail(c);
}

}

extern "C" int64_t pm_vae_layout_bytes(void) { return (int64_t)sizeof(PmVaeLayout); }
extern "C" int pm_vae_step_reload_switches(void) {
  g_cfg = read_cfg();
  return PM_OK;
}
extern "C" int64_t pm_vae_step_state_bytes(void) { return (int64_t)sizeof(StepState); }

static void measure_step(const PmVaeLayout* lay, const PmBatch& bt, size_t* zero_bytes, size_t* main_bytes) {
  StepState s;
  memset(&s, 0, sizeof(s));
  s.lay = *lay; s.bt = bt;
// ... 220 lines not shown
```

Before: 131,900.

## Fold top-layer BN backward sums and input ReLU backward into producer kernels

Adds norm-sum epilogues to the decoder long-K rows GEMM and the encoder attention-pool backward, so the top GCN layer's batch-norm backward statistics and absmax are accumulated while the gradient is written. This removes the separate pm_bn_bwd_sums_absmax pass over the gradient. It also adds a ReLU-masking variant of the segment-reduce backward for layer 0, which drops the standalone pm_relu_bwd pass in the encoder. In exchange the epilogues do extra reads of h, double-precision atomics and larger LDS use, and the folds are turned off in deterministic mode.

```diff
diff --git a/include/polyphemus_hip.h b/include/polyphemus_hip.h
--- a/include/polyphemus_hip.h
+++ b/include/polyphemus_hip.h
@@ -204,6 +204,12 @@
                           int32_t N, int32_t E, int32_t G, int32_t d, float dropout_p, uint32_t seed,
                           uint32_t layer_uid, int32_t compact, float* dx, float* dT, const PmNormSums* next_norm,
                           pm_stream_t stream);
+int pm_rows_times_weight_longk_norm(const float* X, int32_t ldx, int32_t N, int32_t K, const uint16_t* w_frag, int32_t kind,
+                                    int32_t w_pitch, int32_t Nout, float* C, int32_t ldc, const PmNormSums* top_norm,
+                                    pm_stream_t stream);
+int pm_segreduce_bwd_relu(const float* x, const float* T, const float* dA, const float* dres, const int32_t* plan,
+                          int32_t N, int32_t E, int32_t G, int32_t d, float dropout_p, uint32_t seed,
+                          uint32_t layer_uid, int32_t compact, float* dx, float* dT, pm_stream_t stream);
 int pm_segreduce_bwd(const float* x, const float* T, const float* dA ,
                      const float* dres ,
                      const int32_t* plan, int32_t N, int32_t E, int32_t G, int32_t d, float dropout_p,
@@ -389,6 +395,11 @@
                     const float* x_gate ,
                     float* dx_gate ,
                     pm_stream_t stream);
+int pm_attnpool_bwd_norm(const float* x, const float* g, const float* g_mean, const float* g_var, float eps,
+                         const float* bn_g, const float* alpha, const float* dout, const float* gate_w,
+                         const int32_t* plan, int32_t N, int32_t E, int32_t G, int32_t d, float* dx, float* d_gate_w,
+                         float* d_gate_b, float* d_bn_g, float* d_bn_b, float* scratch, const PmNormSums* top_norm,
+                         pm_stream_t stream);
 int pm_attnpool_bwd_sums(const float* x, const float* g, const float* g_mean, const float* g_var, float eps,
                          const float* alpha, const float* dout, const int32_t* plan, int32_t N, int32_t E, int32_t G,
                          int32_t d, float* scratch , pm_stream_t stream);
diff --git a/polyphemus_amd/_lib.py b/polyphemus_amd/_lib.py
--- a/polyphemus_amd/_lib.py
+++ b/polyphemus_amd/_lib.py
@@ -173,6 +173,9 @@
     "pm_node_tracks": "pilppps",
     "pm_sample_structure": "pipuppps",
     "pm_notes_from_tokens": "ppiilppppplpps",
+    "pm_rows_times_weight_longk_norm": "piiipiiipips",
+    "pm_segreduce_bwd_relu": "pppppiiiifuuipps",
+    "pm_attnpool_bwd_norm": "ppppfpppppiiiippppppps",
 }
 _CT = {"p": C.c_void_p, "i": C.c_int32, "l": C.c_int64, "f": C.c_float, "u": C.c_uint32, "s": C.c_void_p, "D": C.c_double}
 _RET64 = {"pm_vae_step_workspace_bytes", "pm_vae_layout_bytes", "pm_vae_step_state_bytes", "pm_unembed_scratch_bytes",
diff --git a/polyphemus_amd/csrc/common.h b/polyphemus_amd/csrc/common.h
--- a/polyphemus_amd/csrc/common.h
+++ b/polyphemus_amd/csrc/common.h
@@ -204,6 +204,13 @@
   if (relu && !(xh * ga + be > 0.f)) du = 0.f;
   return ga * rstd * (du - m0 - xh * m1);
 }
+__device__ static inline void pm_bn_bwd_acc(float x, float dy, float mean, float rstd, float ga, float be, int relu, double& a,
+                                            double& b, double& c) {
+  const float xh = (x - mean) * rstd;
+  float du = dy;
+  if (relu && !(xh * ga + be > 0.f)) du = 0.f;
+  a += (double)du; b += (double)du * (double)xh; c += (double)xh;
+}
 __device__ static inline float pm_wave_max(float v) {
 #pragma unroll
   for (int o = 32; o > 0; o >>= 1) v = fmaxf(v, __shfl_xor(v, o, 64));
diff --git a/polyphemus_amd/csrc/linear.hip b/polyphemus_amd/csrc/linear.hip
--- a/polyphemus_amd/csrc/linear.hip
+++ b/polyphemus_amd/csrc/linear.hip
@@ -1,6 +1,7 @@
 #include "gcl_tiles.h"
 #include <type_traits>
 #include <stdlib.h>
+#include <string.h>
 #include "prof.h"
 #include "wide.h"
 
@@ -169,7 +170,7 @@
 template <int D, int BKIND>
 __global__ void __launch_bounds__(rows_threads<D>()) __attribute__((amdgpu_waves_per_eu((rows_nmw<D>() + 4) / 4, (rows_nmw<D>() + 4) / 4)))
 k_rows_wk(const float* __restrict__ X, int ldx, int N, int K, const char* __restrict__ wfrag, int wpitch,
-          float* __restrict__ C, int ldc) {
+          float* __restrict__ C, int ldc, PmNormSums nn) {
   constexpr int NMW = rows_nmw<D>(), WC = D / NMW, TN = WC / 32, HS = D + 8, NTHR = rows_threads<D>();
   extern __shared__ __attribute__((aligned(16))) char smem[];
   float* const sH = reinterpret_cast<float*>(smem);
@@ -291,26 +292,72 @@
   static_assert(NTHR >= 512, "row groups");
   const int col = tid % D, rg = tid / D;
   const __amdgpu_buffer_rsrc_t crs = __builtin_amdgcn_make_buffer_rsrc(C, 0, GCL_OOB, 0x00020000);
-  if (tid >= 512) return;
+  const bool sums = nn.h != nullptr;
+  float nm = 0.f, nrs = 1.f, nga = 1.f, nbe = 0.f, amax = 0.f;
+  double s0 = 0, s1 = 0, s2 = 0;
+  if (sums && tid < 512) { nm = nn.mean[col]; nrs = rsqrtf(nn.var[col] + nn.eps); nga = nn.gamma[col]; nbe = nn.beta[col]; }
+  if (tid < 512 && !sums) {
 #pragma unroll 8
-  for (int k = 0; k < RG; ++k) {
-    const int rr = rg * RG + k, row = m0 + rr;
-    __builtin_amdgcn_raw_buffer_store_b32(__float_as_uint(sH[rr * HS + col]), crs, row < N ? (int)(((int64_t)row * ldc + col) * 4) : GCL_OOB, 0, 0);
-  }
-}
-
-extern "C" int pm_rows_times_weight_longk(const float* X, int32_t ldx, int32_t N, int32_t K, const uint16_t* w_frag,
-                                          int32_t kind, int32_t w_pitch, int32_t Nout, float* C, int32_t ldc,
-                                          pm_stream_t stream) {
+    for (int k = 0; k < RG; ++k) {
+      const int rr = rg * RG + k, row = m0 + rr;
+      __builtin_amdgcn_raw_buffer_store_b32(__float_as_uint(sH[rr * HS + col]), crs, row < N ? (int)(((int64_t)row * ldc + col) * 4) : GCL_OOB, 0, 0);
+    }
+  }
+  if (tid < 512 && sums) {
+#pragma unroll 1
+    for (int k0 = 0; k0 < RG; k0 += 8) {
+      float hv[8];
+#pragma unroll
+      for (int u = 0; u < 8; ++u) hv[u] = nn.h[(int64_t)min(m0 + rg * RG + k0 + u, N - 1) * D + col];
+#pragma unroll
+      for (int u = 0; u < 8; ++u) {
+        const int rr = rg * RG + k0 + u, row = m0 + rr;
+        const float v = sH[rr * HS + col];
+        __builtin_amdgcn_raw_buffer_store_b32(__float_as_uint(v), crs, row < N ? (int)(((int64_t)row * ldc + col) * 4) : GCL_OOB, 0, 0);
+        if (row < N) {
+          amax = fmaxf(amax, fabsf(v));
+          pm_bn_bwd_acc(hv[u], v, nm, nrs, nga, nbe, nn.relu, s0, s1, s2);
+        }
+      }
+    }
+  }
+  if (!sums) return;
+  __syncthreads();
+  double* const sd = reinterpret_cast<double*>(smem);
+  unsigned* const sMax = reinterpret_cast<unsigned*>(sd + NG * 3 * D);
+  if (tid == 0) *sMax = 0u;
+  if (tid < 512) { sd[(rg * 3 + 0) * D + col] = s0; sd[(rg * 3 + 1) * D + col] = s1; sd[(rg * 3 + 2) * D + col] = s2; }
+  amax = pm_wave_max(amax);
+  __syncthreads();
+  if (lane == 0) atomicMax(sMax, __float_as_uint(amax));
+  double* const dst = nn.acc3 + (int64_t)(blockIdx.x % PM_BN_REPL) * 3 * D;
+  for (int i = tid; i < 3 * D; i += NTHR) {
+    double t = 0;
+#pragma unroll
+    for (int g = 0; g < NG; ++g) t += sd[g * 3 * D + i];
+    atomicAdd(&dst[i], t);
+  }
+  __syncthreads();
+  if (tid == 0 && nn.absmax_out) atomicMax(nn.absmax_out + (blockIdx.x % PM_ABSMAX_SLOTS), *sMax);
+}
+
+static int rows_times_weight_longk_impl(const float* X, int32_t ldx, int32_t N, int32_t K, const uint16_t* w_frag,
+                                        int32_t kind, int32_t w_pitch, int32_t Nout, float* C, int32_t ldc,
+                                        const PmNormSums* nn, pm_stream_t stream) {
   if (!X || !w_frag || !C || N <= 0 || K <= 0 || (K % CH) || (Nout != 128 && Nout != 256 && Nout != 512) || (kind != 0 && kind != 1) ||
       ldx < K || ldc < Nout || (ldx & 3) || ((uintptr_t)X % 16) || ((uintptr_t)w_frag % 16) ||
       (int64_t)N * ldx * 4 >= 0x7fffffffLL || (int64_t)N * ldc * 4 >= 0x7fffffffLL || (kind == 0 && w_pitch * 16 < K))
     return PM_E_INVALID;
+  if (nn && (!nn->h || !nn->mean || !nn->var || !nn->gamma || !nn->beta || !nn->acc3)) return PM_E_INVALID;
+  if (nn && (Nout == 512 || pm_det_on())) return PM_E_UNSUPPORTED;
   if (Nout == 512)
     return pm_wide_rows_times_weight_longk(X, ldx, N, K, w_frag, kind, w_pitch, C, ldc, (hipStream_t)stream);
   hipStream_t st = (hipStream_t)stream;
   const dim3 grid(pm_row_grid(N));
   const size_t lds = 2 * IMG;
+  PmNormSums nv_;
+  memset(&nv_, 0, sizeof(nv_));
+  if (nn) nv_ = *nn;
   const int pe = pm_prof_open(st, PM_PROF_ROWS_W, 2.0 * N * (double)K * Nout);
 #define LAUNCH(DD, KD)                                                                                                 \
   do {                                                                                                                 \
@@ -320,13 +367,24 @@
       once = true;                                                                                                     \
     }                                                                                                                  \
     hipLaunchKernelGGL((k_rows_wk<DD, KD>), grid, dim3(rows_threads<DD>()), lds, st, X, ldx, N, K, reinterpret_cast<const char*>(w_frag), \
-                       w_pitch, C, ldc);                                                                               \
+                       w_pitch, C, ldc, nv_);                                                                          \
   } while (0)
   if (Nout == 256) { if (kind == 0) LAUNCH(256, 0); else LAUNCH(256, 1); }
   else { if (kind == 0) LAUNCH(128, 0); else LAUNCH(128, 1); }
 #undef LAUNCH
   pm_prof_close(st, pe);
   return pm_check_launch();
+}
+extern "C" int pm_rows_times_weight_longk(const float* X, int32_t ldx, int32_t N, int32_t K, const uint16_t* w_frag,
+                                          int32_t kind, int32_t w_pitch, int32_t Nout, float* C, int32_t ldc,
+                                          pm_stream_t stream) {
+  return rows_times_weight_longk_impl(X, ldx, N, K, w_frag, kind, w_pitch, Nout, C, ldc, nullptr, stream);
+}
+extern "C" int pm_rows_times_weight_longk_norm(const float* X, int32_t ldx, int32_t N, int32_t K, const uint16_t* w_frag,
+                                               int32_t kind, int32_t w_pitch, int32_t Nout, float* C, int32_t ldc,
+                                               const PmNormSums* top_norm, pm_stream_t stream) {
+  if (!top_norm) return PM_E_INVALID;
+  return rows_times_weight_longk_impl(X, ldx, N, K, w_frag, kind, w_pitch, Nout, C, ldc, top_norm, stream);
 }
 
 
diff --git a/polyphemus_amd/csrc/norm.hip b/polyphemus_amd/csrc/norm.hip
--- a/polyphemus_amd/csrc/norm.hip
+++ b/polyphemus_amd/csrc/norm.hip
@@ -11,12 +11,7 @@
 __device__ static inline void bn_acc(float xv, float dyv, float m, float rstd, float ga, float be, int relu,
                                      double& a, double& b, double& c) {
   if (MODE == 0) { a += (double)xv; b += (double)xv * (double)xv; }
-  else {
-    const float xh = (xv - m) * rstd;
-    float du = dyv;
-    if (relu && !(xh * ga + be > 0.f)) du = 0.f;
-    a += (double)du; b += (double)du * (double)xh; c += (double)xh;
-  }
+  else pm_bn_bwd_acc(xv, dyv, m, rstd, ga, be, relu, a, b, c);
 }
 
 template <int MODE>
diff --git a/polyphemus_amd/csrc/pool.hip b/polyphemus_amd/csrc/pool.hip
--- a/polyphemus_amd/csrc/pool.hip
+++ b/polyphemus_amd/csrc/pool.hip
@@ -1,4 +1,5 @@
 #include "common.h"
+#include <string.h>
 
 __global__ void __launch_bounds__(256) k_gate_fwd(const float* __restrict__ x, const float* __restrict__ w,
                                                   const float* __restrict__ b, int N, int d, float* __restrict__ g) {
@@ -112,6 +113,7 @@
   if (threadIdx.x == 0) { atomicAdd(&sums[0], (double)s0); atomicAdd(&sums[1], (double)s1); }
   pm_turn_leave_block(gate);
 }
+template <bool SUMS>
 __global__ void __launch_bounds__(256) k_attnpool_bwd2(const float* __restrict__ x, const float* __restrict__ g,
                                                        const float* __restrict__ gm, const float* __restrict__ gv,
                                                        float eps, const float* __restrict__ bg,
@@ -121,11 +123,23 @@
                                                        int N, int d, float* __restrict__ dx, float* dW, float* db,
                                                        float* dbn_g, float* dbn_b, const float* __restrict__ xg,
                                                        float* __restrict__ dxg, const double* __restrict__ gsums,
-                                                       double gcount, unsigned* gate) {
+                                                       double gcount, unsigned* gate, PmNormSums nn) {
   extern __shared__ __attribute__((aligned(16))) float sW[];
   for (int i = threadIdx.x; i <= d; i += blockDim.x) sW[i] = 0.f;
+  double* const sD = reinterpret_cast<double*>(sW + d + 2);
+  unsigned* const sMax = reinterpret_cast<unsigned*>(sD + 12 * d);
+  if (SUMS && threadIdx.x == 0) *sMax = 0u;
   __syncthreads();
   const int lane = threadIdx.x & 63, wave = threadIdx.x >> 6;
+  float nm[4], nrs[4], nga[4], nbe[4], amax = 0.f;
+  double ns0[4] = {0, 0, 0, 0}, ns1[4] = {0, 0, 0, 0}, ns2[4] = {0, 0, 0, 0};
+  if (SUMS) {
+#pragma unroll
+    for (int j = 0; j < 4; ++j) {
+      const int col = lane * 4 < d ? lane * 4 + j : 0;
+      nm[j] = nn.mean[col]; nrs[j] = rsqrtf(nn.var[col] + nn.eps); nga[j] = nn.gamma[col]; nbe[j] = nn.beta[col];
+    }
+  }
   const float mean = gm[0], rstd = rsqrtf(gv[0] + eps), ga = bg[0];
   const float m0 = gsums ? (float)(gsums[0] / gcount) : (float)(sums[0] / N);
   const float m1 = gsums ? (float)(gsums[1] / gcount) : (float)(sums[1] / N);
@@ -149,9 +163,19 @@
       if (dxg) {
         *reinterpret_cast<float4*>(dx + (int64_t)n * d + c) = make_float4(a * dv.x, a * dv.y, a * dv.z, a * dv.w);
         *reinterpret_cast<float4*>(dxg + (int64_t)n * d + c) = make_float4(dg * wv.x, dg * wv.y, dg * wv.z, dg * wv.w);
-      } else
-      *reinterpret_cast<float4*>(dx + (int64_t)n * d + c) =
-          make_float4(a * dv.x + dg * wv.x, a * dv.y + dg * wv.y, a * dv.z + dg * wv.z, a * dv.w + dg * wv.w);
+      } else {
+        const float4 o = make_float4(__builtin_fmaf(dg, wv.x, a * dv.x), __builtin_fmaf(dg, wv.y, a * dv.y),
+                                     __builtin_fmaf(dg, wv.z, a * dv.z), __builtin_fmaf(dg, wv.w, a * dv.w));
+        *reinterpret_cast<float4*>(dx + (int64_t)n * d + c) = o;
+        if (SUMS && k == 0) {
+          const float4 hv = *reinterpret_cast<const float4*>(nn.h + (int64_t)n * d + c);
+          amax = fmaxf(fmaxf(amax, fmaxf(fabsf(o.x), fabsf(o.y))), fmaxf(fabsf(o.z), fabsf(o.w)));
+          pm_bn_bwd_acc(hv.x, o.x, nm[0], nrs[0], nga[0], nbe[0], nn.relu, ns0[0], ns1[0], ns2[0]);
+          pm_bn_bwd_acc(hv.y, o.y, nm[1], nrs[1], nga[1], nbe[1], nn.relu, ns0[1], ns1[1], ns2[1]);
+          pm_bn_bwd_acc(hv.z, o.z, nm[2], nrs[2], nga[2], nbe[2], nn.relu, ns0[2], ns1[2], ns2[2]);
+          pm_bn_bwd_acc(hv.w, o.w, nm[3], nrs[3], nga[3], nbe[3], nn.relu, ns0[3], ns1[3], ns2[3]);
+        }
+      }
       wacc[k].x += dg * xv.x; wacc[k].y += dg * xv.y; wacc[k].z += dg * xv.z; wacc[k].w += dg * xv.w;
     }
     bacc += dg;
@@ -169,18 +193,40 @@
     }
     if (gate) __syncthreads();
   }
+  if (SUMS) {
+    if (lane * 4 < d) {
+#pragma unroll
+      for (int j = 0; j < 4; ++j) {
+        double* slot = sD + (int64_t)wave * 3 * d + lane * 4 + j;
+        slot[0] = ns0[j]; slot[d] = ns1[j]; slot[2 * d] = ns2[j];
+      }
+    }
+    amax = pm_wave_max(amax);
+    if (lane == 0) atomicMax(sMax, __float_as_uint(amax));
+  }
   __syncthreads();
   pm_turn_enter_block(gate);
   for (int i = threadIdx.x; i < d; i += blockDim.x) atomicAdd(&dW[i], sW[i]);
   if (threadIdx.x == 0) atomicAdd(&db[0], sW[d]);
   pm_turn_leave_block(gate);
+  if (SUMS) {
+    double* dst = nn.acc3 + (int64_t)(blockIdx.x % PM_BN_REPL) * 3 * d;
+    for (int i = threadIdx.x; i < 3 * d; i += blockDim.x)
+      atomicAdd(&dst[i], (sD[i] + sD[3 * d + i]) + (sD[6 * d + i] + sD[9 * d + i]));
+    if (nn.absmax_out && threadIdx.x == 0) atomicMax(nn.absmax_out + (blockIdx.x % PM_ABSMAX_SLOTS), *sMax);
+  }
 }
 static int attnpool_bwd_impl(const float* x, const float* g, const float* g_mean, const float* g_var, float eps,
                              const float* bn_g, const float* alpha, const float* dout, const float* gate_w,
                              const int32_t* plan, int32_t N, int32_t E, int32_t G, int32_t d, float* dx, float* d_gate_w,
                              float* d_gate_b, float* d_bn_g, float* d_bn_b, float* scratch, const float* x_gate,
-                             float* dx_gate, int phase, const double* gsums, double gcount, pm_stream_t stream) {
+                             float* dx_gate, int phase, const double* gsums, double gcount, const PmNormSums* nn,
+                             pm_stream_t stream) {
   if ((x_gate == nullptr) != (dx_gate == nullptr)) return PM_E_INVALID;
+  if (nn && (!nn->h || !nn->mean || !nn->var || !nn->gamma || !nn->beta || !nn->acc3 || ((uintptr_t)nn->h & 15) || phase == 1 ||
+             x_gate))
+    return PM_E_INVALID;
+  if (nn && (d > 256 || pm_det_on())) return PM_E_UNSUPPORTED;
   if (!x || !g || !g_mean || !g_var || !alpha || !dout || !plan || !scratch || N <= 0 || G <= 0 || d <= 0 || (d & 3) ||
       d > 1024 || ((uintptr_t)scratch & 7))
     return PM_E_INVALID;
@@ -197,9 +243,16 @@
   if (phase != 1) {
     int nb = (int)pm_cdiv(N, 4);
     if (nb > 256) nb = 256;
-    hipLaunchKernelGGL(k_attnpool_bwd2, dim3(nb), dim3(256), sizeof(float) * (d + 1), st, x, g, g_mean, g_var, eps, bn_g,
-                       alpha, dout, gate_w, pv.node_bar, dgn, sums, N, d, dx, d_gate_w, d_gate_b, d_bn_g, d_bn_b,
-                       x_gate ? x_gate : x, dx_gate, gsums, gcount, pm_det_gate(st));
+    PmNormSums none;
+    memset(&none, 0, sizeof(none));
+    if (nn)
+      hipLaunchKernelGGL(k_attnpool_bwd2<true>, dim3(nb), dim3(256), sizeof(float) * (d + 2) + sizeof(double) * 12 * d + 8, st, x, g,
+                         g_mean, g_var, eps, bn_g, alpha, dout, gate_w, pv.node_bar, dgn, sums, N, d, dx, d_gate_w, d_gate_b, d_bn_g,
+                         d_bn_b, x, dx_gate, gsums, gcount, nullptr, *nn);
+    else
+      hipLaunchKernelGGL(k_attnpool_bwd2<false>, dim3(nb), dim3(256), sizeof(float) * (d + 1), st, x, g, g_mean, g_var, eps, bn_g,
+                         alpha, dout, gate_w, pv.node_bar, dgn, sums, N, d, dx, d_gate_w, d_gate_b, d_bn_g, d_bn_b,
+                         x_gate ? x_gate : x, dx_gate, gsums, gcount, pm_det_gate(st), none);
   }
   return pm_check_launch();
 }
@@ -209,13 +262,22 @@
                                float* d_gate_w, float* d_gate_b, float* d_bn_g, float* d_bn_b, float* scratch,
                                const float* x_gate, float* dx_gate, pm_stream_t stream) {
   return attnpool_bwd_impl(x, g, g_mean, g_var, eps, bn_g, alpha, dout, gate_w, plan, N, E, G, d, dx, d_gate_w, d_gate_b,
-                           d_bn_g, d_bn_b, scratch, x_gate, dx_gate, 0, nullptr, 0.0, stream);
+                           d_bn_g, d_bn_b, scratch, x_gate, dx_gate, 0, nullptr, 0.0, nullptr, stream);
+}
+extern "C" int pm_attnpool_bwd_norm(const float* x, const float* g, const float* g_mean, const float* g_var, float eps,
+                                    const float* bn_g, const float* alpha, const float* dout, const float* gate_w,
+                                    const int32_t* plan, int32_t N, int32_t E, int32_t G, int32_t d, float* dx,
+                                    float* d_gate_w, float* d_gate_b, float* d_bn_g, float* d_bn_b, float* scratch,
+                                    const PmNormSums* top_norm, pm_stream_t stream) {
+  if (!top_norm) return PM_E_INVALID;
+  return attnpool_bwd_impl(x, g, g_mean, g_var, eps, bn_g, alpha, dout, gate_w, plan, N, E, G, d, dx, d_gate_w, d_gate_b,
+                           d_bn_g, d_bn_b, scratch, nullptr, nullptr, 0, nullptr, 0.0, top_norm, stream);
 }
 extern "C" int pm_attnpool_bwd_sums(const float* x, const float* g, const float* g_mean, const float* g_var, float eps,
                                     const float* alpha, const float* dout, const int32_t* plan, int32_t N, int32_t E,
                                     int32_t G, int32_t d, float* scratch, pm_stream_t stream) {
   return attnpool_bwd_impl(x, g, g_mean, g_var, eps, nullptr, alpha, dout, nullptr, plan, N, E, G, d, nullptr, nullptr,
-                           nullptr, nullptr, nullptr, scratch, nullptr, nullptr, 1, nullptr, 0.0, stream);
+                           nullptr, nullptr, nullptr, scratch, nullptr, nullptr, 1, nullptr, 0.0, nullptr, stream);
 }
 extern "C" int pm_attnpool_bwd_from_sums(const float* x, const float* g, const float* g_mean, const float* g_var, float eps,
                                          const float* bn_g, const float* alpha, const float* dout, const float* gate_w,
@@ -225,7 +287,7 @@
                                          double count_global, pm_stream_t stream) {
   if (!sums_global || !(count_global > 0)) return PM_E_INVALID;
   return attnpool_bwd_impl(x, g, g_mean, g_var, eps, bn_g, alpha, dout, gate_w, plan, N, E, G, d, dx, d_gate_w, d_gate_b,
-                           d_bn_g, d_bn_b, scratch, x_gate, dx_gate, 2, sums_global, count_global, stream);
+                           d_bn_g, d_bn_b, scratch, x_gate, dx_gate, 2, sums_global, count_global, nullptr, stream);
 }
 
 __global__ void __launch_bounds__(256) k_bar_bcast_fwd(const float* __restrict__ bars, const int* __restrict__ node_bar,
diff --git a/polyphemus_amd/csrc/segreduce.hip b/polyphemus_amd/csrc/segreduce.hip
--- a/polyphemus_amd/csrc/segreduce.hip
+++ b/polyphemus_amd/csrc/segreduce.hip
@@ -171,7 +171,7 @@
                                                        const float* __restrict__ csc_invcnt, int N, int d,
                                                        uint32_t seed, uint32_t layer_uid, uint32_t thresh, float scale,
                                                        int compact, float* __restrict__ dx, float* __restrict__ dT,
-                                                       PmNormSums nn, int xcd_nodes, int pr, unsigned* gate) {
+                                                       PmNormSums nn, int xcd_nodes, int pr, unsigned* gate, int relu_x) {
   constexpr int EPT = NV == 1 ? SEG_EPT : 2;
   extern __shared__ __attribute__((aligned(16))) float sT[];
   const int nwv0 = blockDim.x >> 6;
@@ -332,6 +332,10 @@
 #pragma unroll
     for (int v = 0; v < NV; ++v) {
       if (!ok[v]) continue;
+      if (!FUSE && relu_x) {
+        acc[v].x = xv[v].x > 0.f ? acc[v].x : 0.f; acc[v].y = xv[v].y > 0.f ? acc[v].y : 0.f;
+        acc[v].z = xv[v].z > 0.f ? acc[v].z : 0.f; acc[v].w = xv[v].w > 0.f ? acc[v].w : 0.f;
+      }
       *reinterpret_cast<float4*>(dx + (int64_t)n * d + c[v]) = acc[v];
       if (FUSE) {
         if constexpr (NV == 1)
@@ -432,7 +436,7 @@
 static int segreduce_bwd_impl(const float* x, const float* T, const float* dA, const float* dres, const int32_t* plan,
                               int32_t N, int32_t E, int32_t G, int32_t d, float dropout_p, uint32_t seed,
                               uint32_t layer_uid, int32_t compact, float* dx, float* dT, const PmNormSums* nn,
-                              pm_stream_t stream) {
+                              int relu_x, pm_stream_t stream) {
   if (!x || !T || !dA || !plan || !dx || !dT || N <= 0 || d <= 0 || (d & 3) || d > 1024 || dropout_p < 0.f ||
       dropout_p >= 1.f)
     return PM_E_INVALID;
@@ -463,7 +467,7 @@
 #define LAUNCH(NV, DR, FU, RL)                                                                                       \
   do { seg_bwd_lds_attr<NV, DR, FU, RL>(lds);                                                                     \
   hipLaunchKernelGGL((k_segreduce_bwd<NV, DR, FU, RL>), grid, block, lds, st, x, T, dA, dres, pv.colptr, pv.csc_dst,  \
-                     pv.csc_reldist, pv.csc_eid, pv.csc_invcnt, N, d, seed, layer_uid, thresh, scale, compact, dx, dT, nv_, xcd_nodes, pr, gate); } while (0)
+                     pv.csc_reldist, pv.csc_eid, pv.csc_invcnt, N, d, seed, layer_uid, thresh, scale, compact, dx, dT, nv_, xcd_nodes, pr, gate, relu_x); } while (0)
   const bool rl = d <= 256 || (int64_t)E >= 16 * (int64_t)N;
 #define LAUNCH2(NV, DR) do { if (nn) { if (rl) LAUNCH(NV, DR, true, true); else LAUNCH(NV, DR, true, false); }       \
                              else { if (rl) LAUNCH(NV, DR, false, true); else LAUNCH(NV, DR, false, false); } } while (0)
@@ -480,12 +484,17 @@
 extern "C" int pm_segreduce_bwd(const float* x, const float* T, const float* dA, const float* dres, const int32_t* plan,
                                 int32_t N, int32_t E, int32_t G, int32_t d, float dropout_p, uint32_t seed,
                                 uint32_t layer_uid, int32_t compact, float* dx, float* dT, pm_stream_t stream) {
-  return segreduce_bwd_impl(x, T, dA, dres, plan, N, E, G, d, dropout_p, seed, layer_uid, compact, dx, dT, nullptr, stream);
+  return segreduce_bwd_impl(x, T, dA, dres, plan, N, E, G, d, dropout_p, seed, layer_uid, compact, dx, dT, nullptr, 0, stream);
 }
 extern "C" int pm_segreduce_bwd_norm(const float* x, const float* T, const float* dA, const float* dres,
                                      const int32_t* plan, int32_t N, int32_t E, int32_t G, int32_t d, float dropout_p,
                                      uint32_t seed, uint32_t layer_uid, int32_t compact, float* dx, float* dT,
                                      const PmNormSums* next_norm, pm_stream_t stream) {
   if (!next_norm) return PM_E_INVALID;
-  return segreduce_bwd_impl(x, T, dA, dres, plan, N, E, G, d, dropout_p, seed, layer_uid, compact, dx, dT, next_norm, stream);
-}
+  return segreduce_bwd_impl(x, T, dA, dres, plan, N, E, G, d, dropout_p, seed, layer_uid, compact, dx, dT, next_norm, 0, stream);
+}
+extern "C" int pm_segreduce_bwd_relu(const float* x, const float* T, const float* dA, const float* dres, const int32_t* plan,
+                                     int32_t N, int32_t E, int32_t G, int32_t d, float dropout_p, uint32_t seed,
+                                     uint32_t layer_uid, int32_t compact, float* dx, float* dT, pm_stream_t stream) {
+  return segreduce_bwd_impl(x, T, dA, dres, plan, N, E, G, d, dropout_p, seed, layer_uid, compact, dx, dT, nullptr, 1, stream);
+}
diff --git a/polyphemus_amd/csrc/vae_step.hip b/polyphemus_amd/csrc/vae_step.hip
--- a/polyphemus_amd/csrc/vae_step.hip
+++ b/polyphemus_amd/csrc/vae_step.hip
@@ -30,6 +30,7 @@
   bool unembed_dw;
   bool pad_skip;
   bool cnn_fused;
+  bool chain_folds;
   bool bar_route;
   int64_t offset_limit;
 };
@@ -54,6 +55,7 @@
   k.unembed_dw = flag("PM_UNEMBED_DW", true);
   k.senc_first = flag("PM_SENC_FIRST", true);
   k.cnn_fused = flag("PM_CNN_FUSED", true);
+  k.chain_folds = flag("PM_CHAIN_FOLDS", true);
   k.offset_limit = getenv("PM_GCL_OFFSET_LIMIT") ? atoll(getenv("PM_GCL_OFFSET_LIMIT")) : 0x7fffffffLL;
   return k;
 }
@@ -98,6 +100,8 @@
   enum Bagg { BAGG_SEG_DROPPED, BAGG_BAR, BAGG_SEG } bagg;
   bool bagg_sums;
   bool bagg_absmax;
+  bool top_sums_folded;
+  bool relu_x0_folded;
   bool frag;
   int classes;
 };
@@ -354,6 +358,10 @@
   r.bagg = dropping ? GcnRoute::BAGG_SEG_DROPPED : bar ? GcnRoute::BAGG_BAR : GcnRoute::BAGG_SEG;
   r.bagg_sums = d <= 512 && c.bn && !dropping;
   r.bagg_absmax = r.h2 && (d <= 256 || bar);
+  const bool decoder = &sv == &c.s->dg;
+  const bool folds = k.chain_folds && !pm_det_on() && in_dagg && r.bagg == GcnRoute::BAGG_SEG;
+  r.top_sums_folded = folds && (decoder ? rows_w_ok(c) : true);
+  r.relu_x0_folded = folds && !decoder;
   return r;
 }
 HeadRoute head_route(const Ctx& c) {
@@ -522,6 +530,15 @@
   }
   return sv.x[c.L];
 }
+PmNormSums gcn_top_norm(const Ctx& c, const PmGcn& g, const GcnSaved& sv) {
+  const int i = c.L - 1;
+  const PmBn& bn = g.norm[i];
+  PmNormSums nn;
+  nn.h = sv.h[i]; nn.mean = sv.mean[i]; nn.var = sv.var[i]; nn.gamma = c.P + bn.w; nn.beta = c.P + bn.b; nn.eps = 1e-5f; nn.relu = 1;
+  nn.acc3 = sv.pool + ((size_t)i * 5 + 2) * c.d * PM_BN_REPL;
+  nn.absmax_out = sv.rt.h2 ? sv.mdu + i * PM_ABSMAX_SLOTS : nullptr;
+  return nn;
+}
 float* gcn_backward(Ctx& c, float* dx, const PmGcn& g, GcnSaved& sv) {
   Arena& ar = c.s->ar;
   const int N = c.N, d = c.d, nb = c.compact ? 4 : 7;
@@ -548,7 +565,7 @@
     if (r.h2) { h2.absmax_in = sv.mdu + i * PM_ABSMAX_SLOTS; h2.scale_out = sv.sdh + i; h2.w_scale = kH2WScale; }
     switch (r.norm) {
       case GcnRoute::NORM_IN_DAGG:
-        if (!sums_ready)
+        if (!sums_ready && !r.top_sums_folded)
           RUN(pm_bn_bwd_sums_absmax(sv.h[i], dx, N, d, sv.mean[i], sv.var[i], 1e-5f, c.P + bn.w, c.P + bn.b, 1, acc3,
                                       (r.h2 && du_from_sums) ? sv.mdu + i * PM_ABSMAX_SLOTS : nullptr, c.st));
         break;
@@ -648,6 +665,8 @@
         if (carry)
           RUN(pm_segreduce_bwd_norm(sv.x[i], sv.T, dA, res, c.s->plan, N, c.E, c.Gn, d, sv.p, sv.seed, sv.uid0 + i, c.compact, out,
                                       dT, &nn, c.st));
+        else if (i == 0 && r.relu_x0_folded)
+          RUN(pm_segreduce_bwd_relu(sv.x[i], sv.T, dA, res, c.s->plan, N, c.E, c.Gn, d, sv.p, sv.seed, sv.uid0 + i, c.compact, out, dT, c.st));
         else
           RUN(pm_segreduce_bwd(sv.x[i], sv.T, dA, res, c.s->plan, N, c.E, c.Gn, d, sv.p, sv.seed, sv.uid0 + i, c.compact, out, dT, c.st));
         break;
@@ -1086,7 +1105,10 @@
   if (s.fix_structure) structure_decoder_backward(c, dzr);
   unembed_input_grad(c);
   float* dxL = s.ar.f((size_t)N * d);
-  if (s.head.dec_rows)
+  if (s.head.dec_rows && s.dg.rt.top_sums_folded) {
+    const PmNormSums nn = gcn_top_norm(c, Y.dec_gcn, s.dg);
+    RUN(pm_rows_times_weight_longk_norm(s.dH, S * d, N, S * d, s.wf_dec_t, 1, 0, d, dxL, d, &nn, c.st));
+  } else if (s.head.dec_rows)
     RUN(pm_rows_times_weight_longk(s.dH, S * d, N, S * d, s.wf_dec_t, 1, 0, d, dxL, d, c.st));
   else
     lin_bwd(c, s.dH, s.dg.x[c.L], Y.dec_chord, N, S * d, d, dxL);
@@ -1154,6 +1176,12 @@
   float* pscr = ar.f((size_t)3 * N + 8);
   const bool dropping = c.pdrop > 0.f;
   float* dxg = dropping ? ar.f((size_t)N * d) : nullptr;
+  if (s.eg.rt.top_sums_folded) {
+    const PmNormSums nn = gcn_top_norm(c, Y.enc_gcn, s.eg);
+    RUN(pm_attnpool_bwd_norm(s.eg.x[c.L], s.g, s.gm, s.gv, 1e-5f, c.P + Y.enc_gate_bn.w, s.alpha, dpooled, c.P + Y.enc_gate.w,
+                               s.plan, N, c.E, Gn, d, dxL, c.G + Y.enc_gate.w, c.G + Y.enc_gate.b, c.G + Y.enc_gate_bn.w,
+                               c.G + Y.enc_gate_bn.b, pscr, &nn, c.st));
+  } else
   RUN(pm_attnpool_bwd(s.eg.x[c.L], s.g, s.gm, s.gv, 1e-5f, c.P + Y.enc_gate_bn.w, s.alpha, dpooled, c.P + Y.enc_gate.w,
                         s.plan, N, c.E, Gn, d, dxL, c.G + Y.enc_gate.w, c.G + Y.enc_gate.b, c.G + Y.enc_gate_bn.w,
                         c.G + Y.enc_gate_bn.b, pscr, dropping ? s.xLg : nullptr, dxg, c.st));
@@ -1174,7 +1202,7 @@
   s.bk_dxL = nullptr;
   float* dx0 = gcn_backward(c, dxL, Y.enc_gcn, s.eg);
   drop(c, dx0, N, d, SITE_ENC_CHORD, s.seed_enc, dx0);
-  RUN(pm_relu_bwd(dx0, s.x0, (int64_t)N * d, dx0, c.st));
+  if (!s.eg.rt.relu_x0_folded) RUN(pm_relu_bwd(dx0, s.x0, (int64_t)N * d, dx0, c.st));
   branch_join(c, BR_ENC_HEAD_WGRAD);
   s.bk_dx0 = dx0; s.bk_dzcat = dzcat;
 }
```

New measurement: 132,800 (median of 6 runs). About the same (+0.7%).
